# pierluigiferrari/differential_equations_resnet

Hardware: AMD Instinct MI355X
Metric: CIFAR-10 images/sec (fwd+bwd) antisym-ResNet-32 @ batch 512; 1/2/4/8 GPUs (higher is better)
Workload: dtype bf16; 1 GPU; antisym-ResNet-32 (C=64, 30 Euler blocks) batch 512/GPU bf16; train step = fwd + bwd + Adam; global_batch=512, per_gpu_batch=512, channels=64, blocks=30, integrator=euler, parallelism=dp1, degraded_handoffs=0

## Files before the change

### differential_equations_resnet_amd/csrc/asr_api.hip

```cpp
#include <math.h>

#include <vector>

#include "asr_common.h"
#include "asr_internal.h"

namespace asr {
static bool mfma_supported(int C, int W) { return (C == 16 || C == 32 || C == 64) && W == 32; }

static int check_shape(int N, int H, int W, int C) {
  if (N < 1 || H < 1 || W < 1 || C < 1) return fail(ASR_E_ARG, "bad shape N=%d H=%d W=%d C=%d", N, H, W, C);
  if ((long)N * H * W * C > (1L << 40)) return fail(ASR_E_ARG, "shape too large");
  return ASR_OK;
}

static int check_bf16_conv(int C, int W) {
  if (!mfma_supported(C, W) && !convb_supported(W, C))
    return fail(ASR_E_UNSUPPORTED, "bf16 conv needs C in {16,32,64} and W == 8 or W %% 16 == 0 (C=%d W=%d)", C, W);
  return ASR_OK;
}

static int check_kernel_size(const char* fn, int kernel_size) {
  if (kernel_size < 1 || kernel_size > 15 || !(kernel_size & 1))
    return fail(ASR_E_ARG, "%s: kernel_size %d (odd, 1..15)", fn, kernel_size);
  return ASR_OK;
}

struct BwdWs {
  size_t dz, slabs, red, g, total;
};

static BwdWs bwd_ws_layout(int N, int H, int W, int C, int dtype, int stages = 1, int K = 3, int slab_rows = -1) {
  BwdWs b{};
  const long E = (long)K * K * C * C;
  const long P = (long)N * H * W * C;
  const int nsl = slab_rows >= 0 ? slab_rows : kMaxBlockSlabs * stages;
  WsCursor c;
  b.dz = c.take(dtype == ASR_F32 ? (size_t)P * 4 : 0);
  b.slabs = c.take((size_t)nsl * (E + C) * 4);
  b.red = c.take(reduce_ws_bytes(nsl, E + C));
  b.g = c.take(stages > 1 ? (size_t)P * (dtype == ASR_BF16 ? 2 : 4) : 0);
  b.total = c.off;
  return b;
}

struct StemWs {
  size_t dz, slabs, red, total;
};

static StemWs stem_ws_layout(long P, int Cin, int C, int K = 3) {
  StemWs w{};
  const long ES1 = (long)K * K * Cin * C + C;
  WsCursor c;
  w.dz = c.take((size_t)P * 4);
  w.slabs = c.take((size_t)kMaxBlockSlabs * ES1 * 4);
  w.red = c.take(reduce_ws_bytes(kMaxBlockSlabs, ES1));
  w.total = c.off;
  return w;
}

static int block_backward(int mode, const void* dy, const void* x, const uint8_t* mask, const void* w, float h,
                          float gamma, int N, int H, int W, int C, int dtype, void* dx, bool need_w, const void* extra,
                          bool skip_dy, float* slabs, float* dz_scratch, int* nsl, hipStream_t s, bool relu_dx = false,
                          int* relu_done = nullptr, const float* fold_slabs = nullptr, int fold_P = 0,
                          float* fold_grp = nullptr, int* fold_done = nullptr, bool accum_slabs = false) {
  *nsl = 0;
  if (relu_done) *relu_done = 0;
  if (fold_done) *fold_done = 0;
  if (dtype == ASR_BF16) {
    if (!dx && !need_w) return ASR_OK;
    if (!mfma_supported(C, W)) {
      if (extra || skip_dy || relu_dx || fold_slabs || accum_slabs || !convb_supported(W, C))
        return fail(ASR_E_UNSUPPORTED, "bf16 backward at C=%d W=%d: plain Euler blocks and convs only", C, W);
      return convb_backward(dy, mask, x, w, h, 2.f * gamma, N, H, W, C, dx, need_w, slabs, nsl, s,
                            mode == ASR_MODE_CONV);
    }
    const int cm = (mode == ASR_MODE_EULER) ? 2 : 3;
    return block_bwd_mfma(cm, dy, x, mask, w, h, 2.f * gamma, N, H, W, C, dx, slabs, nsl, extra, skip_dy ? 1 : 0, s,
                          relu_dx ? 1 : 0, relu_done, fold_slabs, fold_P, fold_grp, fold_done, accum_slabs ? 1 : 0);
  }
  if (accum_slabs) return fail(ASR_E_UNSUPPORTED, "slab accumulation: bf16 path only");
  const bool euler = mode == ASR_MODE_EULER;
  if (euler && conv32_fused_bwd_supported(W, C))
    return conv32_bwd_fused((const float*)dy, mask, h, (const float*)x, (const float*)w, 2.f * gamma,
                            (const float*)extra, skip_dy, N, H, W, C, (float*)dx, need_w, slabs, nsl, s);
  ASR_TRY(make_dz(euler ? F_EULER : F_CONV, dy, mask, nullptr, h, N, H, W, C, 0, dz_scratch, s));
  if (dx)
    ASR_TRY(conv_f32((euler && !skip_dy) ? B_EULER : B_CONV, dz_scratch, dx, nullptr, (const float*)w, nullptr, h,
                     2.f * gamma, (const float*)dy, N, H, W, C, C, 0, s, (const float*)extra));
  if (need_w) ASR_TRY(wgrad_f32(x, 0, dz_scratch, N, H, W, C, C, slabs, nsl, s));
  return ASR_OK;
}

int conv_backward_keep_slabs(const void* dy, const void* x, const uint8_t* mask, const void* w, float h, float gamma,
                             int N, int H, int W, int C, void* dx, void* ws, float* slabs, int* nsl, hipStream_t s) {
  const BwdWs L = bwd_ws_layout(N, H, W, C, ASR_F32);
  return block_backward(ASR_MODE_EULER, dy, x, mask, w, h, gamma, N, H, W, C, ASR_F32, dx, true, nullptr, false, slabs,
                        (float*)((unsigned char*)ws + L.dz), nsl, s);
}

static int rk2_forward_impl(const void* x, void* xmid, void* y, uint8_t* mask1, uint8_t* mask2, const void* w,
                            const float* bias, float h, int N, int H, int W, int C, int dtype, hipStream_t s) {
  if (dtype == ASR_BF16) {
    ASR_TRY(block_fwd_mfma(0, x, nullptr, xmid, mask1, w, bias, 0.5f * h, N, H, W, C, s));
    return block_fwd_mfma(0, xmid, x, y, mask2, w, bias, h, N, H, W, C, s);
  }
  ASR_TRY(conv_f32(F_EULER, x, xmid, mask1, (const float*)w, bias, 0.5f * h, 0.f, nullptr, N, H, W, C, C, 0, s));
  return conv_f32(F_EULER, xmid, y, mask2, (const float*)w, bias, h, 0.f, nullptr, N, H, W, C, C, 0, s,
                  (const float*)x);
}

static int rk2_backward_slabs(const void* dy, const void* x, const void* xmid, const uint8_t* mask1,
                              const uint8_t* mask2, const void* w, float h, float gamma, int N, int H, int W, int C,
                              int dtype, void* dx, void* g, bool need_w, float* slabs, float* dz_scratch, int* nsl,
                              hipStream_t s, const float* fold_slabs = nullptr, int fold_P = 0,
                              float* fold_grp = nullptr, int* fold_done = nullptr) {
  int n2 = 0, n1 = 0;
  const bool one_set = dtype == ASR_BF16;
  ASR_TRY(block_backward(ASR_MODE_EULER, dy, xmid, mask2, w, h, gamma, N, H, W, C, dtype, g, need_w, nullptr, true,
                         slabs, dz_scratch, &n2, s, false, nullptr, fold_slabs, fold_P, fold_grp, fold_done));
  ASR_TRY(block_backward(ASR_MODE_EULER, g, x, mask1, w, 0.5f * h, gamma, N, H, W, C, dtype, dx, need_w, dy, false,
                         one_set ? slabs : slabs + (long)n2 * (9L * C * C + C), dz_scratch, &n1, s, false, nullptr,
                         nullptr, 0, nullptr, nullptr, one_set));
  *nsl = one_set ? n2 : n1 + n2;
  return ASR_OK;
}

__global__ void k_adam(float* __restrict__ p, const float* __restrict__ g, float* __restrict__ m,
                       float* __restrict__ v, long n, float lr_t, float b1, float b2, float eps, float gscale) {
  for (long i = blockIdx.x * (long)blockDim.x + threadIdx.x; i < n; i += (long)gridDim.x * blockDim.x) {
    const float gi = g[i] * gscale;
    const float mi = b1 * m[i] + (1.f - b1) * gi;
    const float vi = b2 * v[i] + (1.f - b2) * gi * gi;
    m[i] = mi;
    v[i] = vi;
    p[i] -= lr_t * mi / (sqrtf(vi) + eps);
  }
}

__global__ __launch_bounds__(256) void k_relu_grad_bf16(bf16* __restrict__ d, const bf16* __restrict__ x, long n8) {
  for (long i = blockIdx.x * (long)blockDim.x + threadIdx.x; i < n8; i += (long)gridDim.x * blockDim.x) {
    bf16x8 dv = ((const bf16x8*)d)[i];
    const bf16x8 xv = ((const bf16x8*)x)[i];
#pragma unroll
    for (int e = 0; e < 8; ++e) dv[e] = (float)xv[e] > 0.f ? dv[e] : (bf16)0.f;
    ((bf16x8*)d)[i] = dv;
  }
}

int relu_grad_bf16(void* d, const void* x, long n, hipStream_t s) {
  if (n % 8) return fail(ASR_E_ARG, "relu_grad_bf16: n %% 8 != 0");
  const long n8 = n / 8;
  hipLaunchKernelGGL(k_relu_grad_bf16, dim3((unsigned)std::max<long>(1, std::min<long>((n8 + 255) / 256, 4096))),
                     dim3(256), 0, s, (bf16*)d, (const bf16*)x, n8);
  ASR_LAUNCH_CHECK("k_relu_grad_bf16");
  return ASR_OK;
}

__global__ __launch_bounds__(256) void k_segment_sq_norms(const float* __restrict__ x, const long* __restrict__ off,
                                                          float* __restrict__ out) {
  const long b = off[blockIdx.x], e = off[blockIdx.x + 1];
  float acc = 0.f;
  for (long i = b + threadIdx.x; i < e; i += blockDim.x) acc = fmaf(x[i], x[i], acc);
  for (int d = 32; d >= 1; d >>= 1) acc += __shfl_xor(acc, d, 64);
  __shared__ float part[4];
  if ((threadIdx.x & 63) == 0) part[threadIdx.x >> 6] = acc;
  __syncthreads();
  if (threadIdx.x == 0) out[blockIdx.x] = (part[0] + part[1]) + (part[2] + part[3]);
}

__global__ __launch_bounds__(256) void k_batch_metrics(const float* __restrict__ probs, const float* __restrict__ tgt,
                                                       const float* __restrict__ loss, int N, int K,
                                                       float* __restrict__ accum) {
  __shared__ int correct;
  __shared__ float lsum[4];
  if (threadIdx.x == 0) correct = 0;
  __syncthreads();
  float l = 0.f;
  for (int n = threadIdx.x; n < N; n += blockDim.x) {
    const float* p = probs + (long)n * K;
    const float* t = tgt + (long)n * K;
    int ap = 0, at = 0;
    float bp = p[0], bt = t[0], s = 0.f;
    for (int k = 0; k < K; ++k) {
      if (p[k] > bp) bp = p[k], ap = k;
      if (t[k] > bt) bt = t[k], at = k;
      s += p[k];
    }
    if (ap == at) atomicAdd(&correct, 1);
    if (!loss)
      for (int k = 0; k < K; ++k) {
        const float q = p[k] / s;
        l -= t[k] * (q > 1.f - 1e-7f ? -1e-7f : logf(fmaxf(q, 1e-7f)));
      }
  }
  for (int d = 32; d >= 1; d >>= 1) l += __shfl_xor(l, d, 64);
  if ((threadIdx.x & 63) == 0) lsum[threadIdx.x >> 6] = l;
  __syncthreads();
  if (threadIdx.x == 0) {
    accum[0] += loss ? *loss : ((lsum[0] + lsum[1]) + (lsum[2] + lsum[3])) / (float)N;
    accum[1] += (float)correct;
    accum[2] += (float)N;
    accum[3] += 1.f;
  }
}

template <typename Tin>
__global__ void k_normalize(const Tin* __restrict__ img, long n, float mean, float inv_std, int use_norm,
                            float* __restrict__ out) {
  for (long i = blockIdx.x * (long)blockDim.x + threadIdx.x; i < n; i += (long)gridDim.x * blockDim.x) {
    float v = (float)img[i];
    if (use_norm) v = (v - mean) * inv_std;
    out[i] = v;
  }
}

struct NetLayout {
  long ntheta, P, E, wstride;
  long off_c1k, off_c1b, off_blk, blk_stride, off_fck, off_fcb, nparams;
  bool sep_bwd;
  bool rk2;
  int stages;
  long grp_stride;
  size_t grp;
  size_t slabs_all;
  long slab_stride;
  size_t w_src, w_src_bwd, theta_dst, wbuf, wbuf_bwd, x0, acts, xmids, masks, dxa, dxb, dxg, bwdws, slabs2, slabs, red, probs,
      loss_per, dlogits, gap, total;
  long mask_bytes;
  int act_bytes;
  bool fast_stem;
  bool deep;
  size_t deep_slabs;
  bool inference;
  bool stack_bwd;
  bool stack_pair;
  int stack_grid;
  size_t theta_dst_tm, stack_slabs, stack_done;
  size_t theta_dst_pr;
  int f32_rows;
  size_t grow;
  BwdWs bw;
  StemWs stem;
  int k1, kb;
  bool stem_kxk;
  bool kxk;
  int kxk_rows;
};

static int net_k1(const asr_net_config* c) { return c->conv1_kernel_size ? c->conv1_kernel_size : 3; }
static int net_kb(const asr_net_config* c) { return c->kernel_size ? c->kernel_size : 3; }

static const char kNetKernelSizes[] =
    "kernel_size and conv1_kernel_size in {0 (= 3), 3, 5, 7}; kernel_size 5 / 7: ASR_PARAM_GENERAL or "
    "ASR_PARAM_REGULAR blocks, Euler integrator, float32 at any shape, bfloat16 at C in {16, 32, 64} and "
    "W in {8, 16, 32}; kernel_size 3 in bfloat16: C in {16, 32, 64} and W == 8 or W % 16 == 0 (RK2: W == 32)";

static int check_net_kernel_size(const char* field, int k) {
  if (k == 3 || k == 5 || k == 7) return ASR_OK;
  return fail((k < 1 || !(k & 1)) ? ASR_E_ARG : ASR_E_UNSUPPORTED, "%s %d: the network takes %s", field, k,
              kNetKernelSizes);
}

static int net_check(const asr_net_config* c) {
  if (!c) return fail(ASR_E_ARG, "null config");
  ASR_TRY(check_shape(c->N, c->H, c->W, c->C));
  if (c->L < 1 || c->Cin < 1 || c->num_classes < 1)
    return fail(ASR_E_ARG, "bad net config (L=%d Cin=%d K=%d C=%d)", c->L, c->Cin, c->num_classes, c->C);
  if (c->num_classes > 256 || c->C > 256)
    return fail(ASR_E_UNSUPPORTED, "the head takes C and num_classes <= 256 (C=%d K=%d)", c->C, c->num_classes);
  if (c->dtype != ASR_F32 && c->dtype != ASR_BF16) return fail(ASR_E_ARG, "bad dtype");
  if (param_is_antisymmetric(c->param_kind, c->antisymmetric) < 0) return ASR_E_ARG;
  if (c->param_kind == ASR_PARAM_3BY3 && !c->antisymmetric)
    return fail(ASR_E_ARG, "the 3by3 parametrisation is always antisymmetric");
  if (c->integrator != ASR_INTEGRATOR_EULER && c->integrator != ASR_INTEGRATOR_RK2)
    return fail(ASR_E_ARG, "bad integrator %d", c->integrator);
  if (c->variant & ~(ASR_VARIANT_NO_FOLD | ASR_VARIANT_STEM_FWD_VALU | ASR_VARIANT_STEM_WGRAD_VALU | ASR_VARIANT_PER_BLOCK_FWD |
                    ASR_VARIANT_PER_BLOCK_BWD | ASR_VARIANT_INFERENCE | ASR_VARIANT_TIMED | ASR_VARIANT_FULL_DXL |
                    ASR_VARIANT_FULL_SLABS | ASR_VARIANT_W_BF16))
    return fail(ASR_E_ARG, "bad variant bits 0x%x", c->variant);
  const int kb = net_kb(c);
  ASR_TRY(check_net_kernel_size("conv1_kernel_size", net_k1(c)));
  ASR_TRY(check_net_kernel_size("kernel_size", kb));
  if (kb != 3) {
    if (c->param_kind == ASR_PARAM_3BY3)
      return fail(ASR_E_ARG, "the 3by3 parametrisation has kernel_size 3 (kernel_size=%d): the network takes %s", kb,
                  kNetKernelSizes);
    if (c->integrator == ASR_INTEGRATOR_RK2)
      return fail(ASR_E_UNSUPPORTED, "RK2 blocks with kernel_size %d: the network takes %s", kb, kNetKernelSizes);
    if (c->dtype == ASR_BF16 && !convk_bf16_supported(kb, c->W, c->C))
      return fail(ASR_E_UNSUPPORTED, "bf16 network with kernel_size %d at C=%d W=%d: the network takes %s", kb, c->C,
                  c->W, kNetKernelSizes);
    return ASR_OK;
  }
  if (c->dtype == ASR_BF16 && !mfma_supported(c->C, c->W)) {
    if (!convb_supported(c->W, c->C))
      return fail(ASR_E_UNSUPPORTED, "bf16 network needs C in {16,32,64} and W == 8 or W %% 16 == 0 (C=%d W=%d)", c->C,
                  c->W);
    if (c->integrator == ASR_INTEGRATOR_RK2)
      return fail(ASR_E_UNSUPPORTED, "bf16 network with RK2 blocks needs W == 32 (C=%d W=%d)", c->C, c->W);
  }
  return ASR_OK;
}

static NetLayout net_layout(const asr_net_config* c) {
  NetLayout L{};
  const int C = c->C, K = c->num_classes;
  L.k1 = net_k1(c);
  L.kb = net_kb(c);
  L.kxk = L.kb != 3;
  L.ntheta = theta_count_k(C, L.kb, c->param_kind, c->antisymmetric);
  L.sep_bwd = param_is_antisymmetric(c->param_kind, c->antisymmetric) == 0;
  L.rk2 = c->integrator == ASR_INTEGRATOR_RK2;
  L.stages = L.rk2 ? 2 : 1;
  L.P = (long)c->N * c->H * c->W * C;
  L.E = (long)L.kb * L.kb * C * C;
  L.act_bytes = c->dtype == ASR_BF16 ? 2 : 4;
  L.wstride = c->dtype == ASR_BF16 ? (long)(C / 16) * ((L.kb * L.kb * C + 31) / 32) * 512 : L.E;
  L.off_c1k = 0;
  L.off_c1b = (long)L.k1 * L.k1 * c->Cin * C;
  L.off_blk = L.off_c1b + C;
  L.blk_stride = L.ntheta + C;
  L.off_fck = L.off_blk + (long)c->L * L.blk_stride;
  L.off_fcb = L.off_fck + (long)C * K;
  L.nparams = L.off_fcb + K;
  L.mask_bytes = asr_mask_bytes(c->N, c->H, c->W, C);
  L.fast_stem = L.k1 == 3 && stem_supported(c->Cin, c->H, c->W, C);
  L.stem_kxk = c->dtype == ASR_BF16 && L.k1 != 3 && stem_kxk_supported(L.k1, c->Cin, c->W, C);
  L.inference = (c->variant & ASR_VARIANT_INFERENCE) != 0;
  const bool tr = !L.inference;
  L.deep = !L.kxk && c->dtype == ASR_BF16 && !L.rk2 && deep16_supported(c->H, c->W, C);
  L.stack_bwd = !L.kxk && tr && c->dtype == ASR_BF16 && block_stack_bwd_supported(c->N, c->H, c->W, C);
  L.stack_grid = L.stack_bwd ? block_stack_bwd_grid(c->N) : 0;
  L.stack_pair = L.stack_bwd && !L.sep_bwd;
  WsCursor ws;
  L.w_src = ws.take((size_t)L.E * 4);
  L.w_src_bwd = ws.take(L.sep_bwd && tr ? (size_t)L.E * 4 : 0);
  L.theta_dst = ws.take((size_t)L.ntheta * 2 * 4);
  L.wbuf = ws.take((size_t)c->L * L.wstride * L.act_bytes);
  L.wbuf_bwd = ws.take(L.sep_bwd && tr ? (size_t)c->L * L.wstride * L.act_bytes : 0);
  L.x0 = ws.take(L.fast_stem ? 0 : (size_t)c->N * c->H * c->W * c->Cin * 4);
  L.acts = ws.take((size_t)(tr ? c->L + 1 : 3) * L.P * L.act_bytes);
  L.xmids = ws.take(L.rk2 ? (size_t)(tr ? c->L : 1) * L.P * L.act_bytes : 0);
  L.masks = ws.take(tr ? (size_t)L.stages * c->L * L.mask_bytes : 0);
  L.dxa = ws.take(tr ? (size_t)L.P * L.act_bytes : 0);
  L.dxb = ws.take(tr ? (size_t)L.P * L.act_bytes : 0);
  L.dxg = ws.take(L.rk2 && tr ? (size_t)L.P * L.act_bytes : 0);
  const bool f32 = c->dtype == ASR_F32;
  L.kxk_rows = !L.kxk ? 0 : f32 ? wgrad_f32_chunks(c->N, c->H) : wgradk_bf16_slab_rows(L.kb, c->N, c->H, c->W, C);
  L.f32_rows = f32 && !L.kxk ? f32_block_slab_rows(c->N, c->H, c->W, C) : 0;
  L.bw = bwd_ws_layout(c->N, c->H, c->W, C, c->dtype, L.stages, L.kb, L.kxk ? L.kxk_rows : f32 ? 0 : -1);
  L.stem = stem_ws_layout(L.P, c->Cin, C, L.k1);
  L.bwdws = ws.take(tr ? std::max(L.bw.total, L.stem.total) : 0);
  L.slabs2 = ws.take(tr && !f32 && !L.kxk ? (size_t)L.stages * kMaxBlockSlabs * (L.E + C) * 4 : 0);
  const int rows = L.kxk ? L.kxk_rows : f32 ? L.stages * L.f32_rows : L.stages * kMaxBlockSlabs;
  L.grp_stride = (long)reduce_groups(rows) * (L.E + C);
  L.grp = ws.take(tr ? (size_t)c->L * L.grp_stride * 4 : 0);
  L.slab_stride = (long)rows * (L.E + C);
  L.slabs_all = ws.take(tr && f32 && !L.kxk ? (size_t)c->L * L.slab_stride * 4 : 0);
  L.deep_slabs = ws.take(L.deep && tr ? deep16_slab_bytes(c->N, c->L) : 0);
  L.theta_dst_tm = ws.take(L.stack_bwd ? (size_t)L.ntheta * 2 * 4 : 0);
  L.theta_dst_pr = ws.take(L.stack_pair ? (size_t)L.ntheta * 2 * 4 : 0);
  L.stack_slabs = ws.take(L.stack_bwd ? (size_t)c->L * L.stack_grid * (L.E + C) * 4 : 0);
  L.stack_done = ws.take(L.stack_bwd ? (size_t)stack_done_words(c->L) * 4 : 0);
  L.grow = ws.take(L.stack_bwd && !L.rk2 ? (size_t)c->N * C * 2 : 0);
  L.probs = ws.take((size_t)c->N * K * 4);
  L.loss_per = ws.take(tr ? (size_t)c->N * 4 : 0);
  L.dlogits = ws.take(tr ? (size_t)c->N * K * 4 : 0);
  L.gap = ws.take(tr ? (size_t)c->N * C * 4 : 0);
  L.total = ws.off;
  return L;
}

constexpr int kMaxTimedDevices = 64;
struct TimedEvents {
  hipEvent_t ev[5];
  bool made;
  unsigned rec;
};
static TimedEvents g_tev[kMaxTimedDevices];

static TimedEvents* timed_events_here() {
  int dev = 0;
  if (hipGetDevice(&dev) != hipSuccess || dev < 0 || dev >= kMaxTimedDevices) return nullptr;
  return &g_tev[dev];
}

static int timed_event(const asr_net_config* c, int i, hipStream_t s) {
  if (!(c->variant & ASR_VARIANT_TIMED)) return ASR_OK;
  TimedEvents* t = timed_events_here();
  if (!t) return fail(ASR_E_HIP, "ASR_VARIANT_TIMED: no current device (or device id >= %d)", kMaxTimedDevices);
  if (!t->made) {
    for (auto& e : t->ev) ASR_TRY(hip_check(hipEventCreate(&e), "hipEventCreate"));
    t->made = true;
  }
  if (i == 0) t->rec = 0;
  ASR_TRY(hip_check(hipEventRecord(t->ev[i], s), "hipEventRecord"));
  t->rec |= 1u << i;
  return ASR_OK;
}

static unsigned char* net_xL(const asr_net_config* c, const NetLayout& L, unsigned char* ws, bool training,
                             bool stack_fwd) {
  const size_t a = (size_t)L.P * L.act_bytes;
  if (training) return ws + L.acts + (size_t)c->L * a;
  if (stack_fwd) return ws + L.acts + (size_t)(1 + (c->L - 1) % 2) * a;
  return ws + L.acts + (size_t)(c->L & 1) * a;
}

static int net_normalize(const asr_net_config* c, const NetLayout& L, const void* images, unsigned char* ws,
                         hipStream_t s) {
  const float inv_std = c->use_norm ? 1.f / c->divide_by_stddev : 1.f;
  const long nin = (long)c->N * c->H * c->W * c->Cin;
  float* x0 = (float*)(ws + L.x0);
  const unsigned gn = (unsigned)std::min<long>((nin + 255) / 256, 4096);
  if (c->input_u8)
    hipLaunchKernelGGL(k_normalize<uint8_t>, dim3(gn), dim3(256), 0, s, (const uint8_t*)images, nin, c->subtract_mean,
                       inv_std, c->use_norm, x0);
  else
    hipLaunchKernelGGL(k_normalize<float>, dim3(gn), dim3(256), 0, s, (const float*)images, nin, c->subtract_mean,
                       inv_std, c->use_norm, x0);
  ASR_LAUNCH_CHECK("k_normalize");
  return ASR_OK;
}

static int net_forward_impl(const asr_net_config* c, const NetLayout& L, const float* params, const void* images,
                            bool training, unsigned char* ws, hipStream_t s, unsigned char** xL_out = nullptr) {
  const int C = c->C, N = c->N, H = c->H, W = c->W;
  const bool bf = c->dtype == ASR_BF16;
  const float inv_std = c->use_norm ? 1.f / c->divide_by_stddev : 1.f;
  if (training && L.inference) return fail(ASR_E_ARG, "an ASR_VARIANT_INFERENCE workspace has no training buffers");
  const bool bal = !(c->variant & ASR_VARIANT_W_BF16);
  if (L.kxk) {
    const float* th = params + L.off_blk;
    const int32_t* src = (const int32_t*)(ws + L.w_src);
    const int32_t* src_bwd = (const int32_t*)(ws + L.w_src_bwd);
    if (bf) {
      ASR_TRY(asr_theta_to_w_k_bf16(th, L.blk_stride, c->L, C, L.kb, src, c->gamma, ws + L.wbuf, L.wstride, s));
      if (training && L.sep_bwd)
        ASR_TRY(asr_theta_to_w_k_bf16(th, L.blk_stride, c->L, C, L.kb, src_bwd, 0.f, ws + L.wbuf_bwd, L.wstride, s));
    } else {
      ASR_TRY(asr_theta_to_w_k(th, L.blk_stride, c->L, C, L.kb, src, c->gamma, (float*)(ws + L.wbuf), L.wstride, s));
      if (training && L.sep_bwd)
        ASR_TRY(asr_theta_to_w_k(th, L.blk_stride, c->L, C, L.kb, src_bwd, 0.f, (float*)(ws + L.wbuf_bwd), L.wstride,
                                 s));
    }
  } else if (bf)
    ASR_TRY(theta_to_w_bf16(params + L.off_blk, L.blk_stride, c->L, C, (const int32_t*)(ws + L.w_src), c->gamma,
                            ws + L.wbuf, L.wstride, bal, s,
                            c->param_kind != ASR_PARAM_REGULAR ? (const int32_t*)(ws + L.theta_dst) : nullptr,
                            L.ntheta));
  else
    ASR_TRY(asr_theta_to_w(params + L.off_blk, L.blk_stride, c->L, C, (const int32_t*)(ws + L.w_src), c->gamma,
                           ws + L.wbuf, L.wstride, c->dtype, s));
  if (training && L.sep_bwd && !L.kxk) {
    if (bf)
      ASR_TRY(theta_to_w_bf16(params + L.off_blk, L.blk_stride, c->L, C, (const int32_t*)(ws + L.w_src_bwd), 0.f,
                              ws + L.wbuf_bwd, L.wstride, bal, s));
    else
      ASR_TRY(asr_theta_to_w(params + L.off_blk, L.blk_stride, c->L, C, (const int32_t*)(ws + L.w_src_bwd), 0.f,
                             ws + L.wbuf_bwd, L.wstride, c->dtype, s));
  }
  unsigned char* acts = ws + L.acts;
  auto act = [&](int i) -> unsigned char* {
    const int slot = training ? i : (i & 1);
    return acts + (size_t)slot * L.P * L.act_bytes;
  };
  if (xL_out) *xL_out = net_xL(c, L, ws, training, false);
  if (L.fast_stem && bf && stem_fwd_mfma_supported(c->Cin, H, W, C) && !(c->variant & ASR_VARIANT_STEM_FWD_VALU)) {
    ASR_TRY(stem_fwd_mfma(images, c->input_u8, params + L.off_c1k, params + L.off_c1b, N, H, W, c->Cin, C,
                          c->subtract_mean, inv_std, c->use_norm, act(0), s));
  } else if (L.stem_kxk && !(c->variant & ASR_VARIANT_STEM_FWD_VALU)) {
    ASR_TRY(stem_fwd_kxk(L.k1, images, c->input_u8, params + L.off_c1k, params + L.off_c1b, N, H, W, c->Cin, C,
                         c->subtract_mean, inv_std, c->use_norm, act(0), s));
  } else if (L.fast_stem) {
    ASR_TRY(stem_forward(images, c->input_u8, params + L.off_c1k, params + L.off_c1b, N, H, W, c->Cin, C,
                         c->subtract_mean, inv_std, c->use_norm, act(0), bf ? 1 : 0, s));
  } else {
    float* x0 = (float*)(ws + L.x0);
    ASR_TRY(net_normalize(c, L, images, ws, s));
    ASR_TRY(conv_f32(F_RELU, x0, act(0), nullptr, params + L.off_c1k, params + L.off_c1b, 1.f, 0.f, nullptr, N, H,
                     W, c->Cin, C, bf ? 1 : 0, s, nullptr, L.k1));
  }
  ASR_TRY(timed_event(c, 0, s));
  if (L.deep) {
    ASR_TRY(deep16_forward(act(0), act(training ? 1 : c->L), L.P, training ? (uint8_t*)(ws + L.masks) : nullptr,
                           L.mask_bytes, ws + L.wbuf, params + L.off_blk + L.ntheta, L.blk_stride, c->h, N, c->L,
                           training, s));
    return timed_event(c, 1, s);
  }
  if (bf && training && L.rk2 && block_stack_fwd_supported(N, H, W, C) && !(c->variant & ASR_VARIANT_PER_BLOCK_FWD)) {
    uint8_t* m1 = (uint8_t*)(ws + L.masks);
    ASR_TRY(block_stack_fwd_rk2_mfma(act(0), act(1), ws + L.xmids, (long)L.P, m1, m1 + (size_t)c->L * L.mask_bytes,
                                     (long)L.mask_bytes, ws + L.wbuf, (long)L.wstride, params + L.off_blk + L.ntheta,
                                     L.blk_stride, c->h, N, H, W, C, c->L, s));
    return timed_event(c, 1, s);
  }
  if (bf && !L.rk2 && !L.kxk && (training || L.inference) && block_stack_fwd_supported(N, H, W, C) &&
      !(c->variant & ASR_VARIANT_PER_BLOCK_FWD)) {
    if (training) {
      ASR_TRY(block_stack_fwd_mfma(act(0), act(1), (long)L.P, (uint8_t*)(ws + L.masks), (long)L.mask_bytes,
                                   ws + L.wbuf, (long)L.wstride, params + L.off_blk + L.ntheta, L.blk_stride, c->h, N,
                                   H, W, C, c->L, s));
    } else {
      ASR_TRY(block_stack_fwd_mfma(acts, acts + (size_t)L.P * L.act_bytes, (long)L.P, nullptr, 0, ws + L.wbuf,
                                   (long)L.wstride, params + L.off_blk + L.ntheta, L.blk_stride, c->h, N, H, W, C,
                                   c->L, s, 2));
      if (xL_out) *xL_out = net_xL(c, L, ws, false, true);
    }
    return timed_event(c, 1, s);
  }
  for (int l = 0; l < c->L; ++l) {
    const float* bias = params + L.off_blk + (long)l * L.blk_stride + L.ntheta;
    const unsigned char* wl = ws + L.wbuf + (size_t)l * L.wstride * L.act_bytes;
    uint8_t* mask = training ? (uint8_t*)(ws + L.masks) + (size_t)l * L.mask_bytes : nullptr;
    if (L.rk2) {
      unsigned char* xm = ws + L.xmids + (training ? (size_t)l * L.P * L.act_bytes : 0);
      uint8_t* mask2 = training ? mask + (size_t)c->L * L.mask_bytes : nullptr;
      ASR_TRY(rk2_forward_impl(act(l), xm, act(l + 1), mask, mask2, wl, bias, c->h, N, H, W, C, c->dtype, s));
    } else if (L.kxk && bf) {
      ASR_TRY(convk_bf16(F_EULER, L.kb, act(l), act(l + 1), mask, wl, bias, c->h, 0.f, nullptr, N, H, W, C, s));
    } else if (L.kxk) {
      ASR_TRY(conv_f32_k(F_EULER, L.kb, act(l), act(l + 1), mask, (const float*)wl, bias, c->h, 0.f, nullptr, N, H, W,
                         C, s, nullptr));
    } else if (bf && !mfma_supported(C, W)) {
      ASR_TRY(convb_forward(act(l), act(l + 1), mask, wl, bias, c->h, N, H, W, C, s));
    } else if (bf) {
      ASR_TRY(block_fwd_mfma(0, act(l), nullptr, act(l + 1), mask, wl, bias, c->h, N, H, W, C, s));
    } else {
      ASR_TRY(conv_f32(F_EULER, act(l), act(l + 1), mask, (const float*)wl, bias, c->h, 0.f, nullptr, N, H, W, C, C,
                       0, s));
    }
  }
  return timed_event(c, 1, s);
}

int fused_stage_kind(int H, int W, int C, int dtype) {
  if (dtype == ASR_BF16 && deep16_supported(H, W, C)) return kFusedDeep16;
  return stage_img_supported(H, W, C, dtype) ? kFusedImg : kFusedNone;
}

int fused_stage_forward(int kind, int dtype, const void* x0, void* ys, long y_stride, uint8_t* masks, long mask_stride,
                        const void* w, long w_stride, const float* bias, long bias_stride, float h, int N, int H, int W,
                        int C, int L, bool store_all, hipStream_t s) {
  if (kind == kFusedDeep16)
    return deep16_forward(x0, ys, y_stride, masks, mask_stride, w, bias, bias_stride, h, N, L, store_all, s);
  if (kind != kFusedImg || !store_all)
    return fail(ASR_E_ARG, "fused_stage_forward: kind %d, store_all %d", kind, store_all);
  return stage_img_forward(dtype, x0, ys, y_stride, masks, mask_stride, w, w_stride, bias, bias_stride, h, N, H, W, C,
                           L, s);
}

int fused_stage_backward(const char* who, int kind, int dtype, void* d, void* e, int* in_e, void* dx0_copy, void* dys,
                         const void* xs, long x_stride, const uint8_t* masks, long mask_stride, const void* w,
                         long w_stride, float h, float two_gamma, int N, int H, int W, int C, int L, float* slabs,
                         long slab_stride, int slab_rows, float* grp, long grp_stride, const int32_t* theta_dst,
                         long n_theta, float* dparams, long dp_stride, hipStream_t s) {
  const long E = 9L * C * C, P = (long)N * H * W * C;
  int rows = 0;
  if (kind == kFusedDeep16) {
    ASR_TRY(deep16_backward(d, e, xs, x_stride, masks, mask_stride, w, h, two_gamma, N, L, slabs, &rows, in_e, s));
    if (dx0_copy)
      ASR_TRY(hip_check(hipMemcpyAsync(dx0_copy, *in_e ? e : d, (size_t)P * 2, hipMemcpyDeviceToDevice, s),
                        "hipMemcpyAsync"));
    if (!dparams) return ASR_OK;
    if (rows != slab_rows) return fail(ASR_E_WORKSPACE, "%s: deep16 slab rows %d != %d", who, rows, slab_rows);
    ASR_TRY(reduce_slabs_to_groups(slabs, L * rows, E + C, grp, s));
    return project_layers(grp, grp_stride, reduce_groups(rows), E, C, theta_dst, n_theta, L, dparams, dp_stride, s);
  }
  if (kind != kFusedImg) return fail(ASR_E_ARG, "%s: not a fused stage", who);
  *in_e = 1;
  ASR_TRY(stage_img_backward(dtype, d, dys, P, e, masks, mask_stride, w, w_stride, h, two_gamma, N, H, W, C, L, s));
  if (!dparams) return ASR_OK;
  ASR_TRY(wgrad_layers(dtype, xs, x_stride, dys, P, masks, mask_stride, h, N, H, W, C, L, slabs, slab_stride, &rows, s));
  if (rows > slab_rows) return fail(ASR_E_WORKSPACE, "%s: %d slab rows > the workspace's %d", who, rows, slab_rows);
  ASR_TRY(reduce_slab_layers(slabs, slab_stride, rows, E + C, grp, grp_stride, L, s));
  return project_layers(grp, grp_stride, reduce_groups(rows), E, C, theta_dst, n_theta, L, dparams, dp_stride, s);
}

}

using namespace asr;

extern "C" {

long asr_mask_bytes(int N, int H, int W, int C) {
  if (N < 1 || H < 1 || W < 1 || C < 1) return -1;
  return ((long)N * H * W * C + 31) / 32 * 4;
}

int asr_conv_forward(int mode, const void* x, void* y, uint8_t* mask, const void* w, const float* bias, float h,
                     int N, int H, int W, int C, int dtype, asr_stream_t stream) {
  ASR_TRY(check_shape(N, H, W, C));
  if (!x || !y || !w) return fail(ASR_E_ARG, "asr_conv_forward: null pointer");
  if (mode != ASR_MODE_EULER && mode != ASR_MODE_CONV) return fail(ASR_E_ARG, "asr_conv_forward: bad mode %d", mode);
  hipStream_t s = (hipStream_t)stream;
  if (dtype == ASR_BF16) {
    ASR_TRY(check_bf16_conv(C, W));
    if (!mfma_supported(C, W))
      return convb_forward(x, y, mask, w, bias, h, N, H, W, C, s, mode == ASR_MODE_CONV);
    if (mode == ASR_MODE_EULER && deep16_supported(H, W, C))
      return deep16_forward(x, y, 0, mask, 0, w, bias, 0, h, N, 1, true, s);
    return block_fwd_mfma(mode == ASR_MODE_EULER ? 0 : 1, x, nullptr, y, mask, w, bias, h, N, H, W, C, s);
  }
  if (dtype == ASR_F32)
    return conv_f32(mode == ASR_MODE_EULER ? F_EULER : F_CONV, x, y, mask, (const float*)w, bias, h, 0.f, nullptr, N,
                    H, W, C, C, 0, s);
  return fail(ASR_E_ARG, "asr_conv_forward: bad dtype %d", dtype);
}

static int stack_img_check_strides(const char* who, int dtype, long y_stride, long mask_stride, long w_stride,
                                   long bias_stride, long x_stride) {
  const bool bf = dtype == ASR_BF16;
  if (y_stride % 4) return fail(ASR_E_ARG, "%s: y_stride %% 4 != 0 on the image-resident path", who);
  if (mask_stride % 2) return fail(ASR_E_ARG, "%s: mask_stride %% 2 != 0 on the image-resident path", who);
  if (bf && w_stride % 8) return fail(ASR_E_ARG, "%s: w_stride %% 8 != 0 on the image-resident path", who);
  if (bias_stride % 4) return fail(ASR_E_ARG, "%s: bias_stride %% 4 != 0 on the image-resident path", who);
  if (x_stride % (bf ? 8 : 4))
    return fail(ASR_E_ARG, "%s: x_stride %% %d != 0 on the image-resident path", who, bf ? 8 : 4);
  return ASR_OK;
}

int asr_block_stack_forward(const void* x0, void* ys, long y_stride, uint8_t* masks, long mask_stride, const void* w,
                            long w_stride, const float* bias, long bias_stride, float h, int N, int H, int W, int C,
                            int L, int dtype, int store_all, asr_stream_t stream) {
  ASR_TRY(check_shape(N, H, W, C));
  if (!x0 || !ys || !w || L < 1) return fail(ASR_E_ARG, "asr_block_stack_forward: null pointer or L < 1");
  if (store_all && L > 1 && y_stride < (long)N * H * W * C)
    return fail(ASR_E_ARG, "asr_block_stack_forward: y_stride smaller than one activation");
  hipStream_t s = (hipStream_t)stream;
  const int fused = fused_stage_kind(H, W, C, dtype);
  if (fused == kFusedDeep16) {
    if (L > 1 && w_stride != (long)asr_wpack_elems(C))
      return fail(ASR_E_ARG, "asr_block_stack_forward: w_stride must be asr_wpack_elems(C) on the fused path");
    return fused_stage_forward(fused, dtype, x0, ys, y_stride, masks, mask_stride, w, w_stride, bias, bias_stride, h, N,
                               H, W, C, L, store_all != 0, s);
  }
  if (dtype == ASR_BF16) ASR_TRY(check_bf16_conv(C, W));
  if (dtype != ASR_F32 && dtype != ASR_BF16) return fail(ASR_E_ARG, "asr_block_stack_forward: bad dtype");
  const size_t es = dtype == ASR_BF16 ? 2 : 4;
  if (!store_all && L > 1) return fail(ASR_E_UNSUPPORTED, "asr_block_stack_forward: store_all=0 needs the fused path");
  if (fused == kFusedImg && store_all && bias && masks) {
    ASR_TRY(stack_img_check_strides("asr_block_stack_forward", dtype, y_stride, mask_stride, w_stride, bias_stride, 0));
    return fused_stage_forward(fused, dtype, x0, ys, y_stride, masks, mask_stride, w, w_stride, bias, bias_stride, h, N,
                               H, W, C, L, true, s);
  }
  if (dtype == ASR_BF16 && block_stack_fwd_supported(N, H, W, C))
    return block_stack_fwd_mfma(x0, ys, L > 1 ? y_stride : (long)N * H * W * C, masks, mask_stride, w, w_stride, bias,
                                bias_stride, h, N, H, W, C, L, s);
  for (int l = 0; l < L; ++l) {
    const void* xi = l == 0 ? x0 : (const unsigned char*)ys + (size_t)(l - 1) * y_stride * es;
    void* yo = (unsigned char*)ys + (size_t)l * y_stride * es;
    ASR_TRY(asr_conv_forward(ASR_MODE_EULER, xi, yo, masks ? masks + (size_t)l * mask_stride : nullptr,
                             (const unsigned char*)w + (size_t)l * w_stride * es, bias ? bias + l * bias_stride : nullptr,
                             h, N, H, W, C, dtype, stream));
  }
  return ASR_OK;
}

struct StackWs {
  size_t da, db, slabs, grp, blk, done, tdst, g, dys, total;
  int fused;
  bool stack64;
  int grid;
  int rows;
};
static StackWs stack_ws_layout(int N, int H, int W, int C, int L, int dtype, bool rk2 = false) {
  StackWs w{};
  const size_t act = (size_t)N * H * W * C * (dtype == ASR_BF16 ? 2 : 4);
  const long ES = 9L * C * C + C;
  w.fused = rk2 ? kFusedNone : fused_stage_kind(H, W, C, dtype);
  w.stack64 = dtype == ASR_BF16 && w.fused == kFusedNone && block_stack_bwd_supported(N, H, W, C);
  w.grid = w.stack64 ? block_stack_bwd_grid(N) : 0;
  WsCursor c;
  w.da = c.take(act);
  w.db = c.take(act);
  if (w.fused == kFusedImg) {
    w.rows = f32_block_slab_rows(N, H, W, C);
    w.dys = c.take(L * act);
    w.slabs = c.take((size_t)L * w.rows * ES * 4);
    w.grp = c.take((size_t)L * reduce_groups(w.rows) * ES * 4);
  } else if (w.fused == kFusedDeep16) {
    w.rows = (int)(deep16_slab_bytes(N, 1) / ((size_t)ES * 4));
    w.slabs = c.take(deep16_slab_bytes(N, L));
    w.grp = c.take((size_t)L * reduce_groups(kMaxBlockSlabs) * ES * 4);
  } else if (w.stack64) {
    w.slabs = c.take((size_t)L * w.grid * ES * 4);
    w.grp = c.take((size_t)L * reduce_groups(w.grid) * ES * 4);
    w.done = c.take((size_t)stack_done_words(L) * 4);
    w.tdst = c.take((size_t)2 * 9 * C * C * 4);
    if (rk2) w.g = c.take(act);
  } else {
    w.blk = c.take(bwd_ws_layout(N, H, W, C, dtype).total);
  }
  w.total = c.off;
  return w;
}

static int stack64_backward(const char* who, const StackWs& Lw, const void* dyL, const void* xs, const void* xmids,
                            long x_stride, const uint8_t* masks, const uint8_t* masks2, long mask_stride,
                            const void* w, long w_stride, const int32_t* theta_dst, long n_theta, float h, float gamma,
                            int N, int H, int W, int C, int L, void* dx0, float* dparams, unsigned char* base,
                            hipStream_t s) {
  if (n_theta > 9L * C * C) return fail(ASR_E_ARG, "%s: n_theta > 9*C*C", who);
  const size_t act = (size_t)N * H * W * C * 2;
  ASR_TRY(hip_check(hipMemcpyAsync(base + Lw.da, dyL, act, hipMemcpyDeviceToDevice, s), "hipMemcpyAsync"));
  float* slabs = (float*)(base + Lw.slabs);
  float* grp = (float*)(base + Lw.grp);
  const long ES = stack_slab_floats(C, 1), sst = (long)Lw.grid * ES, gst = (long)reduce_groups(Lw.grid) * ES;
  int lfold = L;
  ASR_TRY(block_stack_bwd_mfma(base + Lw.da, base + Lw.db, xs, x_stride, masks, mask_stride, w, w_stride, h,
                               2.f * gamma, N, H, W, C, L, 0, slabs, sst, grp, gst, (unsigned*)(base + Lw.done),
                               &lfold, s, xmids, masks2, xmids ? base + Lw.g : nullptr, nullptr, 1, 1));
  ASR_TRY(hip_check(hipMemcpyAsync(dx0, base + ((L & 1) ? Lw.db : Lw.da), act, hipMemcpyDeviceToDevice, s),
                    "hipMemcpyAsync"));
  if (!dparams) return ASR_OK;
  ASR_TRY(stack_bwd_reduce_rest(slabs, sst, Lw.grid, ES, grp, gst, L, lfold, (const unsigned*)(base + Lw.done), s));
  int32_t* tm = (int32_t*)(base + Lw.tdst);
  ASR_TRY(theta_dst_pair(theta_dst, n_theta, C, tm, s));
  return project_layers(grp, gst, reduce_groups(Lw.grid), ES - C, C, tm, n_theta, L, dparams, n_theta + C, s);
}

size_t asr_block_stack_backward_workspace_bytes(int N, int H, int W, int C, int L, int dtype) {
  if (check_shape(N, H, W, C) != ASR_OK || L < 1) return 0;
  return stack_ws_layout(N, H, W, C, L, dtype).total;
}

int asr_block_stack_backward(const void* dyL, const void* xs, long x_stride, const uint8_t* masks, long mask_stride,
                             const void* w, long w_stride, const int32_t* theta_dst, long n_theta, float h,
                             float gamma, int N, int H, int W, int C, int L, int dtype, void* dx0, float* dparams,
                             void* ws, size_t ws_bytes, asr_stream_t stream) {
  ASR_TRY(check_shape(N, H, W, C));
  if (!dyL || !xs || !masks || !w || !dx0 || L < 1) return fail(ASR_E_ARG, "asr_block_stack_backward: null pointer");
  if (dparams && !theta_dst) return fail(ASR_E_ARG, "asr_block_stack_backward: theta_dst needed for dparams");
  if (dtype != ASR_F32 && dtype != ASR_BF16) return fail(ASR_E_ARG, "asr_block_stack_backward: bad dtype");
  if (dtype == ASR_BF16) ASR_TRY(check_bf16_conv(C, W));
  const StackWs Lw = stack_ws_layout(N, H, W, C, L, dtype);
  if (Lw.fused == kFusedImg)
    ASR_TRY(stack_img_check_strides("asr_block_stack_backward", dtype, 0, 0, w_stride, 0, x_stride));
  if (!ws || ws_bytes < Lw.total) return fail(ASR_E_WORKSPACE, "asr_block_stack_backward: workspace too small");
  if (Lw.fused == kFusedDeep16 && w_stride != (long)asr_wpack_elems(C))
    return fail(ASR_E_ARG, "asr_block_stack_backward: w_stride must be asr_wpack_elems(C) on the fused path");
  hipStream_t s = (hipStream_t)stream;
  unsigned char* base = (unsigned char*)ws;
  const size_t es = dtype == ASR_BF16 ? 2 : 4, act = (size_t)N * H * W * C * es;
  if (Lw.fused != kFusedNone) {
    const bool deep = Lw.fused == kFusedDeep16;
    const long ES = 9L * C * C + C;
    if (deep) ASR_TRY(hip_check(hipMemcpyAsync(base + Lw.da, dyL, act, hipMemcpyDeviceToDevice, s), "hipMemcpyAsync"));
    int in_e = 0;
    return fused_stage_backward("asr_block_stack_backward", Lw.fused, dtype, deep ? base + Lw.da : (void*)dyL,
                                deep ? base + Lw.db : dx0, &in_e, deep ? dx0 : nullptr, base + Lw.dys, xs, x_stride,
                                masks, mask_stride, w, w_stride, h, 2.f * gamma, N, H, W, C, L,
                                (float*)(base + Lw.slabs), (long)Lw.rows * ES, Lw.rows, (float*)(base + Lw.grp),
                                (long)reduce_groups(Lw.rows) * ES, theta_dst, n_theta, dparams, n_theta + C, s);
  }
  if (Lw.stack64)
    return stack64_backward("asr_block_stack_backward", Lw, dyL, xs, nullptr, x_stride, masks, nullptr, mask_stride, w,
                            w_stride, theta_dst, n_theta, h, gamma, N, H, W, C, L, dx0, dparams, base, s);
  const void* dcur = dyL;
  for (int l = L - 1; l >= 0; --l) {
    void* dnext = l == 0 ? dx0 : base + ((l & 1) ? Lw.db : Lw.da);
    float* dp = dparams ? dparams + (long)l * (n_theta + C) : nullptr;
    ASR_TRY(asr_conv_backward(ASR_MODE_EULER, dcur, (const unsigned char*)xs + (size_t)l * x_stride * es,
                              masks + (size_t)l * mask_stride, (const unsigned char*)w + (size_t)l * w_stride * es,
                              theta_dst, n_theta, h, gamma, N, H, W, C, dtype, dnext, dp, dp ? dp + n_theta : nullptr,
                              nullptr, base + Lw.blk, ws_bytes - Lw.blk, stream));
    dcur = dnext;
  }
  return ASR_OK;
}

int asr_rk2_stack_forward(const void* x0, void* ys, void* xmids, long y_stride, uint8_t* masks1, uint8_t* masks2,
                          long mask_stride, const void* w, long w_stride, const float* bias, long bias_stride, float h,
                          int N, int H, int W, int C, int L, int dtype, asr_stream_t stream) {
  ASR_TRY(check_shape(N, H, W, C));
  if (!x0 || !ys || !xmids || !w || L < 1) return fail(ASR_E_ARG, "asr_rk2_stack_forward: null pointer or L < 1");
  if (dtype != ASR_BF16 || !block_stack_fwd_supported(N, H, W, C))
    return fail(ASR_E_UNSUPPORTED, "asr_rk2_stack_forward: bf16, C=64, W=32 only (C=%d W=%d)", C, W);
  if ((masks1 == nullptr) != (masks2 == nullptr)) return fail(ASR_E_ARG, "asr_rk2_stack_forward: masks1/masks2");
  return block_stack_fwd_rk2_mfma(x0, ys, xmids, y_stride, masks1, masks2, mask_stride, w, w_stride, bias,
                                  bias_stride, h, N, H, W, C, L, (hipStream_t)stream);
}

size_t asr_rk2_stack_backward_workspace_bytes(int N, int H, int W, int C, int L, int dtype) {
  if (check_shape(N, H, W, C) != ASR_OK || L < 1) return 0;
  const StackWs w = stack_ws_layout(N, H, W, C, L, dtype, true);
  return w.stack64 ? w.total : 0;
}

int asr_rk2_stack_backward(const void* dyL, const void* xs, const void* xmids, long x_stride, const uint8_t* masks1,
                           const uint8_t* masks2, long mask_stride, const void* w, long w_stride,
                           const int32_t* theta_dst, long n_theta, float h, float gamma, int N, int H, int W, int C,
                           int L, int dtype, void* dx0, float* dparams, void* ws, size_t ws_bytes,
                           asr_stream_t stream) {
  ASR_TRY(check_shape(N, H, W, C));
  if (!dyL || !xs || !xmids || !masks1 || !masks2 || !w || !dx0 || L < 1)
    return fail(ASR_E_ARG, "asr_rk2_stack_backward: null pointer");
  if (dparams && !theta_dst) return fail(ASR_E_ARG, "asr_rk2_stack_backward: theta_dst needed for dparams");
  const StackWs Lw = stack_ws_layout(N, H, W, C, L, dtype, true);
  if (!Lw.stack64) return fail(ASR_E_UNSUPPORTED, "asr_rk2_stack_backward: bf16, C=64, W=32 only (C=%d W=%d)", C, W);
  if (!ws || ws_bytes < Lw.total) return fail(ASR_E_WORKSPACE, "asr_rk2_stack_backward: workspace too small");
  return stack64_backward("asr_rk2_stack_backward", Lw, dyL, xs, xmids, x_stride, masks1, masks2, mask_stride, w,
                          w_stride, theta_dst, n_theta, h, gamma, N, H, W, C, L, dx0, dparams, (unsigned char*)ws,
                          (hipStream_t)stream);
}

size_t asr_conv_backward_workspace_bytes_k(int N, int H, int W, int C, int kernel_size) {
  if (check_shape(N, H, W, C) != ASR_OK || kernel_size < 1 || !(kernel_size & 1)) return 0;
  return bwd_ws_layout(N, H, W, C, ASR_F32, 1, kernel_size).total;
}

int asr_conv_forward_k(int mode, int kernel_size, const float* x, float* y, uint8_t* mask, const float* w,
                       const float* bias, float h, int N, int H, int W, int C, asr_stream_t stream) {
  ASR_TRY(check_shape(N, H, W, C));
  if (!x || !y || !w) return fail(ASR_E_ARG, "asr_conv_forward_k: null pointer");
  if (mode != ASR_MODE_EULER && mode != ASR_MODE_CONV) return fail(ASR_E_ARG, "asr_conv_forward_k: bad mode %d", mode);
  ASR_TRY(check_kernel_size("asr_conv_forward_k", kernel_size));
  return conv_f32_k(mode == ASR_MODE_EULER ? F_EULER : F_CONV, kernel_size, x, y, mask, w, bias, h, 0.f, nullptr, N, H, W,
                    C, (hipStream_t)stream, nullptr);
}

int asr_conv_backward_k(int mode, int kernel_size, const float* dy, const float* x, const uint8_t* mask,
                        const float* w, const int32_t* theta_dst, long n_theta, float h, float gamma, int N, int H,
                        int W, int C, float* dx, float* dtheta, float* dbias, float* dw, void* ws, size_t ws_bytes,
                        asr_stream_t stream) {
  ASR_TRY(check_shape(N, H, W, C));
  if (mode != ASR_MODE_EULER && mode != ASR_MODE_CONV) return fail(ASR_E_ARG, "asr_conv_backward_k: bad mode %d", mode);
  ASR_TRY(check_kernel_size("asr_conv_backward_k", kernel_size));
  if (!dy || !w || (mode == ASR_MODE_EULER && !mask)) return fail(ASR_E_ARG, "asr_conv_backward_k: null pointer");
  if ((dtheta || dbias || dw) && !x) return fail(ASR_E_ARG, "asr_conv_backward_k: x needed for weight gradients");
  if (dtheta && !theta_dst) return fail(ASR_E_ARG, "asr_conv_backward_k: theta_dst needed for dtheta");
  const BwdWs Lw = bwd_ws_layout(N, H, W, C, ASR_F32, 1, kernel_size);
  if (!ws || ws_bytes < Lw.total) return fail(ASR_E_WORKSPACE, "asr_conv_backward_k: workspace too small");
  hipStream_t s = (hipStream_t)stream;
  unsigned char* base = (unsigned char*)ws;
  float* dz = (float*)(base + Lw.dz);
  float* slabs = (float*)(base + Lw.slabs);
  const bool euler = mode == ASR_MODE_EULER;
  ASR_TRY(make_dz(euler ? F_EULER : F_CONV, dy, mask, nullptr, h, N, H, W, C, 0, dz, s));
  if (dx) ASR_TRY(conv_f32_k(euler ? B_EULER : B_CONV, kernel_size, dz, dx, nullptr, w, nullptr, h, 2.f * gamma, dy, N, H,
                             W, C, s, nullptr));
  if (dtheta || dbias || dw) {
    int nsl = 0;
    ASR_TRY(wgrad_f32(x, 0, dz, N, H, W, C, C, slabs, &nsl, s, kernel_size));
    ASR_TRY(reduce_and_project(slabs, nsl, (long)kernel_size * kernel_size * C * C, C, dtheta ? theta_dst : nullptr,
                               n_theta, dtheta, dbias, dw, (float*)(base + Lw.red), s));
  }
  return ASR_OK;
}

static int check_k_bf16(const char* fn, int kernel_size, int W, int C) {
  ASR_TRY(check_kernel_size(fn, kernel_size));
  if (!convk_bf16_supported(kernel_size, W, C))
    return fail(ASR_E_UNSUPPORTED,
                "%s: the bf16 k x k kernels take kernel_size in {5, 7}, C in {16, 32, 64}, W in {8, 16, 32} "
                "(kernel_size=%d C=%d W=%d)", fn, kernel_size, C, W);
  return ASR_OK;
}

struct BwdWsK {
  size_t slabs, red, total;
  int rows;
};
static BwdWsK bwd_ws_layout_k_bf16(int N, int H, int W, int C, int K) {
  BwdWsK b{};
  const long ES = (long)K * K * C * C + C;
  b.rows = wgradk_bf16_slab_rows(K, N, H, W, C);
  WsCursor c;
  b.slabs = c.take((size_t)b.rows * ES * 4);
  b.red = c.take(reduce_ws_bytes(b.rows, ES));
  b.total = c.off;
  return b;
}

int asr_conv_forward_k_bf16(int mode, int kernel_size, const void* x, void* y, uint8_t* mask, const void* w,
                            const float* bias, float h, int N, int H, int W, int C, asr_stream_t stream) {
  ASR_TRY(check_shape(N, H, W, C));
  if (!x || !y || !w) return fail(ASR_E_ARG, "asr_conv_forward_k_bf16: null pointer");
  if (mode != ASR_MODE_EULER && mode != ASR_MODE_CONV)
    return fail(ASR_E_ARG, "asr_conv_forward_k_bf16: bad mode %d", mode);
  ASR_TRY(check_k_bf16("asr_conv_forward_k_bf16", kernel_size, W, C));
  return convk_bf16(mode == ASR_MODE_EULER ? F_EULER : F_CONV, kernel_size, x, y, mask, w, bias, h, 0.f, nullptr, N, H,
                    W, C, (hipStream_t)stream);
}

size_t asr_conv_backward_workspace_bytes_k_bf16(int N, int H, int W, int C, int kernel_size) {
  if (check_shape(N, H, W, C) != ASR_OK || !convk_bf16_supported(kernel_size, W, C)) return 0;
  return bwd_ws_layout_k_bf16(N, H, W, C, kernel_size).total;
}

int asr_conv_backward_k_bf16(int mode, int kernel_size, const void* dy, const void* x, const uint8_t* mask,
                             const void* w, const int32_t* theta_dst, long n_theta, float h, float gamma, int N, int H,
                             int W, int C, void* dx, float* dtheta, float* dbias, float* dw, void* ws, size_t ws_bytes,
                             asr_stream_t stream) {
  ASR_TRY(check_shape(N, H, W, C));
  if (mode != ASR_MODE_EULER && mode != ASR_MODE_CONV)
    return fail(ASR_E_ARG, "asr_conv_backward_k_bf16: bad mode %d", mode);
  ASR_TRY(check_k_bf16("asr_conv_backward_k_bf16", kernel_size, W, C));
  if (!dy || !w || (mode == ASR_MODE_EULER && !mask)) return fail(ASR_E_ARG, "asr_conv_backward_k_bf16: null pointer");
  if ((dtheta || dbias || dw) && !x) return fail(ASR_E_ARG, "asr_conv_backward_k_bf16: x needed for weight gradients");
  if (dtheta && !theta_dst) return fail(ASR_E_ARG, "asr_conv_backward_k_bf16: theta_dst needed for dtheta");
  const BwdWsK Lw = bwd_ws_layout_k_bf16(N, H, W, C, kernel_size);
  if (!ws || ws_bytes < Lw.total) return fail(ASR_E_WORKSPACE, "asr_conv_backward_k_bf16: workspace too small");
  hipStream_t s = (hipStream_t)stream;
  unsigned char* base = (unsigned char*)ws;
  const bool euler = mode == ASR_MODE_EULER;
  if (dx) ASR_TRY(convk_bf16(euler ? B_EULER : B_CONV, kernel_size, dy, dx, nullptr, w, nullptr, h, 2.f * gamma,
                             euler ? mask : nullptr, N, H, W, C, s));
  if (dtheta || dbias || dw) {
    float* slabs = (float*)(base + Lw.slabs);
    int nsl = 0;
    ASR_TRY(wgradk_bf16(kernel_size, x, dy, euler ? mask : nullptr, euler ? h : 1.f, N, H, W, C, slabs, &nsl, s));
    ASR_TRY(reduce_and_project(slabs, nsl, (long)kernel_size * kernel_size * C * C, C, dtheta ? theta_dst : nullptr,
                               n_theta, dtheta, dbias, dw, (float*)(base + Lw.red), s));
  }
  return ASR_OK;
}

size_t asr_conv_backward_workspace_bytes(int N, int H, int W, int C, int dtype) {
  if (check_shape(N, H, W, C) != ASR_OK) return 0;
  return bwd_ws_layout(N, H, W, C, dtype).total;
}

int asr_conv_backward(int mode, const void* dy, const void* x, const uint8_t* mask, const void* w,
                      const int32_t* theta_dst, long n_theta, float h, float gamma, int N, int H, int W, int C,
                      int dtype, void* dx, float* dtheta, float* dbias, float* dw_hwio, void* ws, size_t ws_bytes,
                      asr_stream_t stream) {
  ASR_TRY(check_shape(N, H, W, C));
  if (mode != ASR_MODE_EULER && mode != ASR_MODE_CONV) return fail(ASR_E_ARG, "asr_conv_backward: bad mode %d", mode);
  if (!dy || !w || (mode == ASR_MODE_EULER && !mask)) return fail(ASR_E_ARG, "asr_conv_backward: null pointer");
  if ((dtheta || dbias || dw_hwio) && !x) return fail(ASR_E_ARG, "asr_conv_backward: x needed for weight gradients");
  if (dtheta && !theta_dst) return fail(ASR_E_ARG, "asr_conv_backward: theta_dst needed for dtheta");
  if (dtype != ASR_F32 && dtype != ASR_BF16) return fail(ASR_E_ARG, "asr_conv_backward: bad dtype");
  if (dtype == ASR_BF16) ASR_TRY(check_bf16_conv(C, W));
  const BwdWs L = bwd_ws_layout(N, H, W, C, dtype);
  if (!ws || ws_bytes < L.total) return fail(ASR_E_WORKSPACE, "asr_conv_backward: workspace too small");
  hipStream_t s = (hipStream_t)stream;
  unsigned char* base = (unsigned char*)ws;
  float* slabs = (float*)(base + L.slabs);
  const bool need_w = dtheta || dbias || dw_hwio;
  int nsl = 0;
  ASR_TRY(block_backward(mode, dy, x, mask, w, h, gamma, N, H, W, C, dtype, dx, need_w, nullptr, false, slabs,
                         (float*)(base + L.dz), &nsl, s));
  if (need_w)
    ASR_TRY(reduce_and_project(slabs, nsl, 9L * C * C, C, dtheta ? theta_dst : nullptr, n_theta, dtheta, dbias,
                               dw_hwio, (float*)(base + L.red), s));
  return ASR_OK;
}

static int check_block_args(const char* fn, int N, int H, int W, int C, int dtype) {
  ASR_TRY(check_shape(N, H, W, C));
  if (dtype != ASR_F32 && dtype != ASR_BF16) return fail(ASR_E_ARG, "%s: bad dtype %d", fn, dtype);
  if (dtype == ASR_BF16 && !mfma_supported(C, W))
    return fail(ASR_E_UNSUPPORTED, "%s: bf16 needs C in {16,32,64} and W == 32 (C=%d W=%d)", fn, C, W);
  return ASR_OK;
}

int asr_rk2_forward(const void* x, void* xmid, void* y, uint8_t* mask1, uint8_t* mask2, const void* w,
                    const float* bias, float h, int N, int H, int W, int C, int dtype, asr_stream_t stream) {
  ASR_TRY(check_block_args("asr_rk2_forward", N, H, W, C, dtype));
  if (!x || !xmid || !y || !w) return fail(ASR_E_ARG, "asr_rk2_forward: null pointer");
  if (x == xmid || x == y || xmid == y) return fail(ASR_E_ARG, "asr_rk2_forward: x, xmid and y must not alias");
  return rk2_forward_impl(x, xmid, y, mask1, mask2, w, bias, h, N, H, W, C, dtype, (hipStream_t)stream);
}

size_t asr_rk2_backward_workspace_bytes(int N, int H, int W, int C, int dtype) {
  if (check_shape(N, H, W, C) != ASR_OK) return 0;
  return bwd_ws_layout(N, H, W, C, dtype, 2).total;
}

int asr_rk2_backward(const void* dy, const void* x, const void* xmid, const uint8_t* mask1, const uint8_t* mask2,
                     const void* w, const int32_t* theta_dst, long n_theta, float h, float gamma, int N, int H, int W,
                     int C, int dtype, void* dx, float* dtheta, float* dbias, float* dw_hwio, void* ws,
                     size_t ws_bytes, asr_stream_t stream) {
  ASR_TRY(check_block_args("asr_rk2_backward", N, H, W, C, dtype));
  if (!dy || !x || !xmid || !mask1 || !mask2 || !w) return fail(ASR_E_ARG, "asr_rk2_backward: null pointer");
  if (dtheta && !theta_dst) return fail(ASR_E_ARG, "asr_rk2_backward: theta_dst needed for dtheta");
  const BwdWs L = bwd_ws_layout(N, H, W, C, dtype, 2);
  if (!ws || ws_bytes < L.total) return fail(ASR_E_WORKSPACE, "asr_rk2_backward: workspace too small");
  hipStream_t s = (hipStream_t)stream;
  unsigned char* base = (unsigned char*)ws;
  float* slabs = (float*)(base + L.slabs);
  const bool need_w = dtheta || dbias || dw_hwio;
  int nsl = 0;
  ASR_TRY(rk2_backward_slabs(dy, x, xmid, mask1, mask2, w, h, gamma, N, H, W, C, dtype, dx, base + L.g, need_w, slabs,
                             (float*)(base + L.dz), &nsl, s));
  if (need_w)
    ASR_TRY(reduce_and_project(slabs, nsl, 9L * C * C, C, dtheta ? theta_dst : nullptr, n_theta, dtheta, dbias,
                               dw_hwio, (float*)(base + L.red), s));
  return ASR_OK;
}

long asr_net_param_count(const asr_net_config* cfg) {
  if (net_check(cfg) != ASR_OK) return -1;
  return net_layout(cfg).nparams;
}

size_t asr_net_workspace_bytes(const asr_net_config* cfg) {
  if (net_check(cfg) != ASR_OK) return 0;
  return net_layout(cfg).total;
}

int asr_net_prepare(const asr_net_config* cfg, void* ws, size_t ws_bytes) {
  ASR_TRY(net_check(cfg));
  const NetLayout L = net_layout(cfg);
  if (!ws || ws_bytes < L.total) return fail(ASR_E_WORKSPACE, "asr_net_prepare: workspace too small");
  ASR_TRY(check_ws_device(ws, "asr_net_prepare"));
  std::vector<int32_t> w_src((size_t)L.E), theta_dst((size_t)L.ntheta * 2);
  ASR_TRY(param_map_k(cfg->C, L.kb, cfg->param_kind, cfg->antisymmetric, w_src.data(), theta_dst.data()));
  unsigned char* b = (unsigned char*)ws;
  if (L.sep_bwd && !L.inference) {
    std::vector<int32_t> w_bwd((size_t)L.E);
    ASR_TRY(param_map_transpose_k(cfg->C, L.kb, w_src.data(), w_bwd.data()));
    ASR_TRY(hip_check(hipMemcpy(b + L.w_src_bwd, w_bwd.data(), w_bwd.size() * 4, hipMemcpyHostToDevice), "hipMemcpy"));
  }
  ASR_TRY(hip_check(hipMemcpy(b + L.w_src, w_src.data(), w_src.size() * 4, hipMemcpyHostToDevice), "hipMemcpy"));
  ASR_TRY(hip_check(hipMemcpy(b + L.theta_dst, theta_dst.data(), theta_dst.size() * 4, hipMemcpyHostToDevice),
                    "hipMemcpy"));
  if (L.stack_pair) {
    std::vector<int32_t> pr(theta_dst.size());
    ASR_TRY(theta_dst_pair_host(theta_dst.data(), L.ntheta, cfg->C, pr.data()));
    ASR_TRY(hip_check(hipMemcpy(b + L.theta_dst_pr, pr.data(), pr.size() * 4, hipMemcpyHostToDevice), "hipMemcpy"));
  }
  if (L.stack_bwd) {
    const int C = cfg->C;
    std::vector<int32_t> tm(theta_dst);
    for (auto& v : tm) {
      if (v < 0) continue;
      const long e = v >> 1, m = e / C, o = e % C;
      const long et = (((m / 16) * (C / 16) + o / 16) * 64 + 16 * ((m % 16) / 4) + o % 16) * 4 + m % 4;
      v = (int32_t)((et << 1) | (v & 1));
    }
    ASR_TRY(hip_check(hipMemcpy(b + L.theta_dst_tm, tm.data(), tm.size() * 4, hipMemcpyHostToDevice), "hipMemcpy"));
  }
  return ASR_OK;
}

int asr_net_forward(const asr_net_config* cfg, const float* params, const void* images, float* probs, void* ws,
                    size_t ws_bytes, asr_stream_t stream) {
  ASR_TRY(net_check(cfg));
  const NetLayout L = net_layout(cfg);
  if (!params || !images || !probs) return fail(ASR_E_ARG, "asr_net_forward: null pointer");
  if (!ws || ws_bytes < L.total) return fail(ASR_E_WORKSPACE, "asr_net_forward: workspace too small");
  ASR_TRY(check_ws_device(ws, "asr_net_forward"));
  hipStream_t s = (hipStream_t)stream;
  unsigned char* b = (unsigned char*)ws;
  unsigned char* xL = nullptr;
  ASR_TRY(net_forward_impl(cfg, L, params, images, false, b, s, &xL));
  ASR_TRY(head(xL, cfg->dtype == ASR_BF16, params + L.off_fck, params + L.off_fcb, nullptr, cfg->N, cfg->H * cfg->W,
               cfg->C, cfg->num_classes, probs, nullptr, nullptr, nullptr, nullptr, s));
  return ASR_OK;
}

int asr_net_check_status(const asr_net_config* cfg, const void* ws, size_t ws_bytes, asr_stream_t stream) {
  ASR_TRY(net_check(cfg));
  const NetLayout L = net_layout(cfg);
  if (!ws || ws_bytes < L.total) return fail(ASR_E_WORKSPACE, "asr_net_check_status: workspace too small");
  ASR_TRY(check_ws_device(ws, "asr_net_check_status"));
  return hip_check(hipStreamSynchronize((hipStream_t)stream), "hipStreamSynchronize");
}

int asr_net_kernel_times(float* us) {
  if (!us) return fail(ASR_E_ARG, "asr_net_kernel_times: null output");
  const TimedEvents* t = timed_events_here();
  if (!t || !t->made || !(t->rec & 3u))
    return fail(ASR_E_ARG, "asr_net_kernel_times: no ASR_VARIANT_TIMED call recorded on the current device");
  for (int i = 0; i < 3; ++i) us[i] = -1.f;
  for (int i = 0; i < 3; ++i) {
    const int a = i == 0 ? 0 : i + 1, e = a + 1;
    if ((t->rec >> a & 1u) && (t->rec >> e & 1u)) {
      ASR_TRY(hip_check(hipEventSynchronize(t->ev[e]), "hipEventSynchronize"));
      float ms = 0.f;
      ASR_TRY(hip_check(hipEventElapsedTime(&ms, t->ev[a], t->ev[e]), "hipEventElapsedTime"));
      us[i] = ms * 1e3f;
    }
  }
  return ASR_OK;
}

int asr_net_forward_backward(const asr_net_config* cfg, const float* params, const void* images, const float* targets,
                             float* grads, float* loss, float* probs, void* ws, size_t ws_bytes,
                             asr_stream_t stream) {
  ASR_TRY(net_check(cfg));
  const NetLayout L = net_layout(cfg);
  if (!params || !images || !targets || !grads || !loss) return fail(ASR_E_ARG, "asr_net_forward_backward: null");
  if (!ws || ws_bytes < L.total) return fail(ASR_E_WORKSPACE, "asr_net_forward_backward: workspace too small");
  if (L.inference)
    return fail(ASR_E_ARG, "asr_net_forward_backward: an ASR_VARIANT_INFERENCE workspace has no training buffers");
  ASR_TRY(check_ws_device(ws, "asr_net_forward_backward"));
  hipStream_t s = (hipStream_t)stream;
  unsigned char* b = (unsigned char*)ws;
  const int C = cfg->C, N = cfg->N, H = cfg->H, W = cfg->W, K = cfg->num_classes;
  const bool bf = cfg->dtype == ASR_BF16;
  const bool stacked = L.stack_bwd && !(cfg->variant & ASR_VARIANT_PER_BLOCK_BWD);
  ASR_TRY(net_forward_impl(cfg, L, params, images, true, b, s));
  auto act = [&](int i) { return b + L.acts + (size_t)i * L.P * L.act_bytes; };
  unsigned char* dcur = b + L.dxa;
  unsigned char* dnext = b + L.dxb;
  float* probs_ws = probs ? probs : (float*)(b + L.probs);
  const bool grow = stacked && !L.rk2 && !(cfg->variant & ASR_VARIANT_FULL_DXL);
  ASR_TRY(head(act(cfg->L), bf, params + L.off_fck, params + L.off_fcb, targets, N, H * W, C, K, probs_ws,
               (float*)(b + L.loss_per), (float*)(b + L.dlogits), (float*)(b + L.gap), grow ? nullptr : dcur, s,
               grow ? b + L.grow : nullptr));
  ASR_TRY(head_param_grads((const float*)(b + L.gap), (const float*)(b + L.dlogits), N, C, K, grads + L.off_fck,
                           grads + L.off_fcb, (const float*)(b + L.loss_per), loss, s));
  const int32_t* theta_dst = (const int32_t*)(b + L.theta_dst);
  int nsl_blk = 0;
  int dz1_fused = 0;
  const float* pend_slabs = nullptr;
  int pend_P = 0;
  float* pend_grp = nullptr;
  const bool fold_on = !(cfg->variant & ASR_VARIANT_NO_FOLD);
  const bool stem_v1 = (cfg->variant & ASR_VARIANT_STEM_WGRAD_VALU) != 0;
  ASR_TRY(timed_event(cfg, 2, s));
  if (L.deep) {
    int rows = 0, in_b = 0;
    float* slabs = (float*)(b + L.deep_slabs);
    ASR_TRY(deep16_backward(dcur, dnext, act(0), L.P, (const uint8_t*)(b + L.masks), L.mask_bytes,
                            b + (L.sep_bwd ? L.wbuf_bwd : L.wbuf), cfg->h, L.sep_bwd ? 0.f : 2.f * cfg->gamma, N,
                            cfg->L, slabs, &rows, &in_b, s));
    ASR_TRY(timed_event(cfg, 3, s));
    if (in_b) std::swap(dcur, dnext);
    const int G = reduce_groups(rows);
    ASR_TRY(reduce_slabs_to_groups(slabs, cfg->L * rows, L.E + C, (float*)(b + L.grp), s));
    ASR_TRY(project_layers((float*)(b + L.grp), (long)G * (L.E + C), G, L.E, C, theta_dst, L.ntheta, cfg->L,
                           grads + L.off_blk, L.blk_stride, s));
    ASR_TRY(timed_event(cfg, 4, s));
  }
  if (stacked) {
    const int grid = L.stack_grid;
    const bool pair = L.stack_pair && !(cfg->variant & ASR_VARIANT_FULL_SLABS);
    const long ES = stack_slab_floats(C, pair ? 1 : 0), sst = (long)grid * ES;
    float* slabs = (float*)(b + L.stack_slabs);
    float* grp = (float*)(b + L.grp);
    const int ro0 = (L.fast_stem || L.stem_kxk) && !stem_v1 && !L.rk2;
    int lfold = cfg->L;
    const uint8_t* m1 = (const uint8_t*)(b + L.masks);
    ASR_TRY(block_stack_bwd_mfma(dcur, dnext, act(0), L.P, m1, L.mask_bytes, b + (L.sep_bwd ? L.wbuf_bwd : L.wbuf),
                                 L.wstride, cfg->h, L.sep_bwd ? 0.f : 2.f * cfg->gamma, N, H, W, C, cfg->L, ro0, slabs,
                                 sst, grp, L.grp_stride, (unsigned*)(b + L.stack_done), &lfold, s,
                                 L.rk2 ? b + L.xmids : nullptr, L.rk2 ? m1 + (size_t)cfg->L * L.mask_bytes : nullptr,
                                 L.rk2 ? b + L.dxg : nullptr, grow ? b + L.grow : nullptr, fold_on ? 1 : 0,
                                 pair ? 1 : 0));
    ASR_TRY(timed_event(cfg, 3, s));
    ASR_TRY(stack_bwd_reduce_rest(slabs, sst, grid, ES, grp, L.grp_stride, cfg->L, lfold,
                                  (const unsigned*)(b + L.stack_done), s));
    if (cfg->L & 1) std::swap(dcur, dnext);
    dz1_fused = ro0;
    ASR_TRY(project_layers(grp, L.grp_stride, reduce_groups(grid), ES - C, C,
                           (const int32_t*)(b + (pair ? L.theta_dst_pr : L.theta_dst_tm)), L.ntheta, cfg->L,
                           grads + L.off_blk, L.blk_stride, s));
    ASR_TRY(timed_event(cfg, 4, s));
  }
  if (L.kxk) {
    float* slabs_k = (float*)(b + L.bwdws + L.bw.slabs);
    float* dz_k = (float*)(b + L.bwdws + L.bw.dz);
    for (int l = cfg->L - 1; l >= 0; --l) {
      const unsigned char* wl = b + (L.sep_bwd ? L.wbuf_bwd : L.wbuf) + (size_t)l * L.wstride * L.act_bytes;
      const uint8_t* mask = (const uint8_t*)(b + L.masks) + (size_t)l * L.mask_bytes;
      const float two_gamma = L.sep_bwd ? 0.f : 2.f * cfg->gamma;
      int nsl = 0;
      if (bf) {
        ASR_TRY(convk_bf16(B_EULER, L.kb, dcur, dnext, nullptr, wl, nullptr, cfg->h, two_gamma, mask, N, H, W, C, s));
        ASR_TRY(wgradk_bf16(L.kb, act(l), dcur, mask, cfg->h, N, H, W, C, slabs_k, &nsl, s));
      } else {
        ASR_TRY(make_dz(F_EULER, dcur, mask, nullptr, cfg->h, N, H, W, C, 0, dz_k, s));
        ASR_TRY(conv_f32_k(B_EULER, L.kb, dz_k, dnext, nullptr, (const float*)wl, nullptr, cfg->h, two_gamma,
                           (const float*)dcur, N, H, W, C, s, nullptr));
        ASR_TRY(wgrad_f32(act(l), 0, dz_k, N, H, W, C, C, slabs_k, &nsl, s, L.kb));
      }
      if (nsl < 1 || nsl > L.kxk_rows)
        return fail(ASR_E_WORKSPACE, "k x k block %d wrote %d slab rows, the workspace holds %d", l, nsl, L.kxk_rows);
      ASR_TRY(reduce_slabs_to_groups(slabs_k, nsl, L.E + C, (float*)(b + L.grp) + (size_t)l * L.grp_stride, s));
      nsl_blk = nsl;
      std::swap(dcur, dnext);
    }
  }
  const bool blk_fuses = !bf || mfma_supported(C, W);
  for (int l = (L.deep || stacked || L.kxk) ? -1 : cfg->L - 1; l >= 0; --l) {
    const unsigned char* wl = b + (L.sep_bwd ? L.wbuf_bwd : L.wbuf) + (size_t)l * L.wstride * L.act_bytes;
    const uint8_t* mask = (const uint8_t*)(b + L.masks) + (size_t)l * L.mask_bytes;
    const float gam = L.sep_bwd ? 0.f : cfg->gamma;
    float* grp_l = (float*)(b + L.grp) + (size_t)l * L.grp_stride;
    float* slabs_l = !bf ? (float*)(b + L.slabs_all) + (size_t)l * L.slab_stride
                         : (float*)(b + ((l & 1) ? L.slabs2 : L.bwdws + L.bw.slabs));
    int nsl = 0, folded = 0;
    if (L.rk2) {
      const unsigned char* xm = b + L.xmids + (size_t)l * L.P * L.act_bytes;
      ASR_TRY(rk2_backward_slabs(dcur, act(l), xm, mask, mask + (size_t)cfg->L * L.mask_bytes, wl, cfg->h, gam, N, H,
                                 W, C, cfg->dtype, dnext, b + L.dxg, true, slabs_l, (float*)(b + L.bwdws + L.bw.dz),
                                 &nsl, s, fold_on ? pend_slabs : nullptr, fold_on ? pend_P : 0, pend_grp, &folded));
    } else {
      ASR_TRY(block_backward(ASR_MODE_EULER, dcur, act(l), mask, wl, cfg->h, gam, N, H, W, C, cfg->dtype, dnext, true,
                             nullptr, false, slabs_l, (float*)(b + L.bwdws + L.bw.dz), &nsl, s,
                             l == 0 && (L.fast_stem || L.stem_kxk) && bf && !stem_v1 && blk_fuses,
                             l == 0 ? &dz1_fused : nullptr, fold_on && blk_fuses ? pend_slabs : nullptr,
                             fold_on && blk_fuses ? pend_P : 0, pend_grp, &folded));
    }
    nsl_blk = nsl;
    std::swap(dcur, dnext);
    if (!bf) {
      if (nsl > L.stages * L.f32_rows)
        return fail(ASR_E_WORKSPACE, "fp32 block %d wrote %d slab rows, the workspace holds %d (sized on another device?)",
                    l, nsl, L.stages * L.f32_rows);
      continue;
    }
    if (pend_P > 0 && !folded) ASR_TRY(reduce_slabs_to_groups(pend_slabs, pend_P, L.E + C, pend_grp, s));
    pend_slabs = slabs_l;
    pend_P = nsl;
    pend_grp = grp_l;
  }
  if (pend_P > 0) ASR_TRY(reduce_slabs_to_groups(pend_slabs, pend_P, L.E + C, pend_grp, s));
  if (!bf && !L.deep && !stacked && !L.kxk && nsl_blk > 0)
    ASR_TRY(reduce_slab_layers((const float*)(b + L.slabs_all), L.slab_stride, nsl_blk, L.E + C,
                               (float*)(b + L.grp), L.grp_stride, cfg->L, s));
  if (!L.deep && !stacked) {
    ASR_TRY(timed_event(cfg, 3, s));
    ASR_TRY(project_layers((float*)(b + L.grp), L.grp_stride, reduce_groups(nsl_blk), L.E, C, theta_dst, L.ntheta,
                           cfg->L, grads + L.off_blk, L.blk_stride, s));
    ASR_TRY(timed_event(cfg, 4, s));
  }
  const long E1 = (long)L.k1 * L.k1 * cfg->Cin * C;
  float* dz = (float*)(b + L.bwdws + L.stem.dz);
  float* slabs = (float*)(b + L.bwdws + L.stem.slabs);
  float* red = (float*)(b + L.bwdws + L.stem.red);
  int nsl = 0;
  const float inv_std = cfg->use_norm ? 1.f / cfg->divide_by_stddev : 1.f;
  if (L.fast_stem && bf && !dz1_fused && !stem_v1 && stem_wgrad_mfma_supported(cfg->Cin, H, W, C) && L.P % 8 == 0) {
    ASR_TRY(relu_grad_bf16(dcur, act(0), L.P, s));
    dz1_fused = 1;
  }
  if (L.stem_kxk && !stem_v1) {
    if (!dz1_fused) ASR_TRY(relu_grad_bf16(dcur, act(0), L.P, s));
    ASR_TRY(stem_wgrad_kxk(L.k1, images, cfg->input_u8, dcur, N, H, W, cfg->Cin, C, cfg->subtract_mean, inv_std,
                           cfg->use_norm, slabs, &nsl, s));
  } else if (L.fast_stem && dz1_fused && stem_wgrad_mfma_supported(cfg->Cin, H, W, C)) {
    ASR_TRY(stem_wgrad_mfma(images, cfg->input_u8, dcur, N, H, W, cfg->Cin, C, cfg->subtract_mean, inv_std,
                            cfg->use_norm, slabs, &nsl, s));
  } else if (L.fast_stem) {
    ASR_TRY(stem_wgrad(images, cfg->input_u8, dcur, act(0), bf, N, H, W, cfg->Cin, C, cfg->subtract_mean, inv_std,
                       cfg->use_norm, slabs, &nsl, s));
  } else {
    if (L.stem_kxk && !(cfg->variant & ASR_VARIANT_STEM_FWD_VALU)) ASR_TRY(net_normalize(cfg, L, images, b, s));
    ASR_TRY(make_dz(F_RELU, dcur, nullptr, act(0), 1.f, N, H, W, C, bf ? 1 : 0, dz, s));
    ASR_TRY(wgrad_f32(b + L.x0, 0, dz, N, H, W, cfg->Cin, C, slabs, &nsl, s, L.k1));
  }
  ASR_TRY(reduce_and_project(slabs, nsl, E1, C, nullptr, 0, nullptr, grads + L.off_c1b, grads + L.off_c1k, red, s));
  return ASR_OK;
}

int asr_segment_sq_norms(const float* x, const long* offsets, int n_segments, float* out, asr_stream_t stream) {
  if (!x || !offsets || !out || n_segments < 0) return fail(ASR_E_ARG, "asr_segment_sq_norms: bad arguments");
  if (n_segments == 0) return ASR_OK;
  hipLaunchKernelGGL(k_segment_sq_norms, dim3(n_segments), dim3(256), 0, (hipStream_t)stream, x, offsets, out);
  ASR_LAUNCH_CHECK("k_segment_sq_norms");
  return ASR_OK;
}

int asr_batch_metrics(const float* probs, const float* targets, const float* loss, int N, int K, float* accum,
                      asr_stream_t stream) {
  if (!probs || !targets || !accum || N < 1 || K < 1) return fail(ASR_E_ARG, "asr_batch_metrics: bad args");
  hipLaunchKernelGGL(k_batch_metrics, dim3(1), dim3(256), 0, (hipStream_t)stream, probs, targets, loss, N, K, accum);
  ASR_LAUNCH_CHECK("k_batch_metrics");
  return ASR_OK;
}

int asr_adam_update(float* params, const float* grads, float* m, float* v, long n, float lr, float beta1, float beta2,
                    float eps, long step, float grad_scale, asr_stream_t stream) {
  if (!params || !grads || !m || !v || n < 0 || step < 1) return fail(ASR_E_ARG, "asr_adam_update: bad arguments");
  const double lr_t = (double)lr * sqrt(1.0 - pow((double)beta2, (double)step)) / (1.0 - pow((double)beta1, (double)step));
  const unsigned grid = (unsigned)std::max<long>(1, std::min<long>((n + 255) / 256, 4096));
  hipLaunchKernelGGL(k_adam, dim3(grid), dim3(256), 0, (hipStream_t)stream, params, grads, m, v, n, (float)lr_t,
                     beta1, beta2, eps, grad_scale);
  ASR_LAUNCH_CHECK("k_adam");
  return ASR_OK;
}

}
```

### differential_equations_resnet_amd/csrc/asr_blk_stem.h

```cpp
#pragma once
#include <type_traits>

#include "asr_blk_common.h"
#include "asr_common.h"
#include "asr_device.h"

namespace asr {
namespace blk {

template <int C, typename Tin>
__global__ __launch_bounds__(256) void k_stem_wgrad_mfma(const Tin* __restrict__ img, const bf16* __restrict__ dz1,
                                                         int N, int H, float mean, float inv_std,
                                                         float* __restrict__ slabs) {
  constexpr int W = 32, CIN = 3, TW = W + 2, BRS = 8, KC = 9 * CIN, NT = C / 16;
  constexpr int IMROW = TW * 4 * 16, DZROW = TW * (C / 8) * 16, DZT = BRS * DZROW;
  extern __shared__ __attribute__((aligned(16))) unsigned char lds[];
  const int IM = 0, DZ0 = H * IMROW, FT = DZ0 + 2 * DZT;
  float* ft = (float*)(lds + FT);
  const int tid = threadIdx.x, lane = tid & 63, wave = tid >> 6;
  const int g = lane >> 4, lx = lane & 15, tq = lx >> 2, tp = lx & 3;
  const int nbands = H / BRS;
  for (int i = tid; i < (H + 2) * TW * CIN; i += 256) ft[i] = 0.f;
  f32x4 acc[2][NT];
#pragma unroll
  for (int mt = 0; mt < 2; ++mt)
#pragma unroll
    for (int nt = 0; nt < NT; ++nt) acc[mt][nt] = f32x4{0.f, 0.f, 0.f, 0.f};
  const int n0 = blockIdx.x, items = ((N - n0 + (int)gridDim.x - 1) / (int)gridDim.x) * nbands;
  auto band_n = [&](int it) { return n0 + (it / nbands) * (int)gridDim.x; };
  auto dma_band = [&](int it, int buf) {
    dma_rows<C, W>(dz1, lds + DZ0 + buf * DZT, band_n(it), (it % nbands) * BRS, BRS, H, wave, 4, lane);
  };
  if (items > 0) dma_band(0, 0);
  for (int it = 0; it < items; ++it) {
    const int buf = it & 1, b = it % nbands;
    if (b == 0) {
      const int n = band_n(it);
      __syncthreads();
      const Tin* src = img + (long)n * H * W * CIN;
      for (int i = tid; i < H * W * CIN; i += 256) {
        const int ci = i % CIN, p = i / CIN;
        ft[((p / W + 1) * TW + p % W + 1) * CIN + ci] = (float)src[i] - mean;
      }
      __syncthreads();
      for (int p = tid; p < H * W; p += 256) {
        const int y = p / W, x = p % W;
#pragma unroll
        for (int q = 0; q < 4; ++q) {
          bf16x8 v;
#pragma unroll
          for (int j = 0; j < 8; ++j) {
            const int kap = 8 * q + j;
            float f = 0.f;
            if (kap < KC) {
              const int tap = kap / CIN, ci = kap % CIN;
              f = ft[((y + tap / 3) * TW + x + tap % 3) * CIN + ci];
            } else if (kap == KC) {
              f = 1.f;
            }
            v[j] = (bf16)f;
          }
          *(bf16x8*)(lds + IM + toff<32>(y, x + 1, q, TW)) = v;
        }
      }
    }
    barrier_vm(0);
    if (it + 1 < items) dma_band(it + 1, buf ^ 1);
    const unsigned char* dzt = lds + DZ0 + buf * DZT;
#pragma unroll
    for (int k = 0; k < BRS / 4; ++k) {
      const int r = wave + 4 * k, y = b * BRS + r;
      const int pb = 8 * g + tq;
      bf16x8 A[2], B[NT];
#pragma unroll
      for (int mt = 0; mt < 2; ++mt) {
        const int q = 2 * mt + (tp >> 1);
        A[mt] = tr_pair(lds + IM + toff<32>(y, pb + 1, q, TW) + 8 * (tp & 1),
                        lds + IM + toff<32>(y, pb + 5, q, TW) + 8 * (tp & 1));
      }
#pragma unroll
      for (int nt = 0; nt < NT; ++nt) {
        const int q = 2 * nt + (tp >> 1);
        B[nt] = tr_pair(dzt + toff<C>(r, pb + 1, q, TW) + 8 * (tp & 1), dzt + toff<C>(r, pb + 5, q, TW) + 8 * (tp & 1));
      }
#pragma unroll
      for (int mt = 0; mt < 2; ++mt)
#pragma unroll
        for (int nt = 0; nt < NT; ++nt)
          acc[mt][nt] = __builtin_amdgcn_mfma_f32_16x16x32_bf16(A[mt], B[nt], acc[mt][nt], 0, 0, 0);
    }
  }
  barrier_vm(0);
  float* red = (float*)lds;
#pragma unroll
  for (int mt = 0; mt < 2; ++mt)
#pragma unroll
    for (int nt = 0; nt < NT; ++nt)
#pragma unroll
      for (int e = 0; e < 4; ++e) red[(wave * 32 + 16 * mt + 4 * g + e) * C + 16 * nt + lx] = acc[mt][nt][e];
  __syncthreads();
  float* slab = slabs + (long)blockIdx.x * (KC * C + C);
  for (int i = tid; i < (KC + 1) * C; i += 256) {
    const float v = (red[i] + red[32 * C + i]) + (red[2 * 32 * C + i] + red[3 * 32 * C + i]);
    slab[i] = i < KC * C ? v * inv_std : v;
  }
}

template <int C, typename Tin>
__global__ __launch_bounds__(256) void k_stem_fwd_mfma(const Tin* __restrict__ img, const float* __restrict__ w1,
                                                       const float* __restrict__ b1, int N, int H, float mean,
                                                       float inv_std, bf16* __restrict__ out) {
  constexpr int W = 32, CIN = 3, TW = W + 2, KC = 9 * CIN, MT = C / 16;
  extern __shared__ __attribute__((aligned(16))) unsigned char lds[];
  float* ft = (float*)lds;
  const int tid = threadIdx.x, lane = tid & 63, wave = tid >> 6;
  const int g = lane >> 4, lx = lane & 15;
  for (int i = tid; i < (H + 2) * TW * CIN; i += 256) ft[i] = 0.f;
  bf16x8 Ah[MT], Al[MT];
#pragma unroll
  for (int mt = 0; mt < MT; ++mt)
#pragma unroll
    for (int j = 0; j < 8; ++j) {
      const int kap = 8 * g + j;
      const float wv = kap < KC ? w1[kap * C + 16 * mt + lx] * inv_std : 0.f;
      const bf16 hi = (bf16)wv;
      Ah[mt][j] = hi;
      Al[mt][j] = (bf16)(wv - (float)hi);
    }
  float bz[MT][4];
#pragma unroll
  for (int mt = 0; mt < MT; ++mt)
#pragma unroll
    for (int e = 0; e < 4; ++e) bz[mt][e] = b1 ? b1[16 * mt + 4 * g + e] : 0.f;
  int koff[8];
#pragma unroll
  for (int j = 0; j < 8; ++j) {
    const int kap = min(8 * g + j, KC - 1), tap = kap / CIN, ci = kap % CIN;
    koff[j] = ((tap / 3) * TW + tap % 3) * CIN + ci;
  }
  for (int n = blockIdx.x; n < N; n += gridDim.x) {
    __syncthreads();
    const Tin* src = img + (long)n * H * W * CIN;
    for (int i = tid; i < H * W * CIN; i += 256) {
      const int ci = i % CIN, p = i / CIN;
      ft[((p / W + 1) * TW + p % W + 1) * CIN + ci] = (float)src[i] - mean;
    }
    __syncthreads();
    for (int pt = wave; pt < H * W / 16; pt += 4) {
      const int y = pt / (W / 16), x0 = (pt % (W / 16)) * 16;
      const float* pb = ft + (y * TW + x0 + lx) * CIN;
      bf16x8 B;
#pragma unroll
      for (int j = 0; j < 8; ++j) B[j] = (bf16)((8 * g + j < KC) ? pb[koff[j]] : 0.f);
      f32x4 acc[MT];
#pragma unroll
      for (int mt = 0; mt < MT; ++mt) {
        acc[mt] = f32x4{bz[mt][0], bz[mt][1], bz[mt][2], bz[mt][3]};
        acc[mt] = __builtin_amdgcn_mfma_f32_16x16x32_bf16(Ah[mt], B, acc[mt], 0, 0, 0);
        acc[mt] = __builtin_amdgcn_mfma_f32_16x16x32_bf16(Al[mt], B, acc[mt], 0, 0, 0);
      }
      u32x2 ov[MT];
#pragma unroll
      for (int mt = 0; mt < MT; ++mt) {
        bf16x4 o4;
#pragma unroll
        for (int e = 0; e < 4; ++e) o4[e] = (bf16)fmaxf(acc[mt][e], 0.f);
        ov[mt] = *(const u32x2*)&o4;
      }
      bf16* orow = out + (((long)n * H + y) * W + x0 + lx) * C;
      if constexpr (MT == 1) {
        *(u32x2*)(orow + 4 * g) = ov[0];
      } else {
#pragma unroll
        for (int mp = 0; mp < MT / 2; ++mp) {
          const auto s0 = __builtin_amdgcn_permlane16_swap(ov[2 * mp][0], ov[2 * mp + 1][0], false, false);
          const auto s1 = __builtin_amdgcn_permlane16_swap(ov[2 * mp][1], ov[2 * mp + 1][1], false, false);
          *(u32x4*)(orow + 16 * (2 * mp + (g & 1)) + 8 * (g >> 1)) = u32x4{s0[0], s1[0], s0[1], s1[1]};
        }
      }
    }
  }
}

template <int W_, int K>
struct StemK {
  static constexpr int W = W_, CIN = 3, KC = K * K * CIN, TW = W + K - 1;
  static constexpr int KS = (KC + 31) / 32;
  static constexpr int BRF = 512 / W;
  static constexpr int BRW = 256 / W;
  static constexpr int MT = (KC + 1 + 15) / 16;
  static constexpr int MTW = (MT + 3) / 4;
};

template <int W, int K, int ROWS, typename Tin>
__device__ __forceinline__ void stemk_stage(const Tin* __restrict__ img, int n, int y0, int H, float mean,
                                            float* __restrict__ ft, int tid) {
  constexpr int CIN = 3, TW = W + K - 1, R = K / 2;
  for (int i = tid; i < ROWS * TW * CIN; i += 256) {
    const int ci = i % CIN, c = (i / CIN) % TW, r = i / (CIN * TW);
    const int gy = y0 + r - R, gx = c - R;
    float v = 0.f;
    if ((unsigned)gy < (unsigned)H && (unsigned)gx < (unsigned)W)
      v = (float)img[(((long)n * H + gy) * W + gx) * CIN + ci] - mean;
    ft[i] = v;
  }
}

template <int C, int W, int K, typename Tin>
__global__ __launch_bounds__(256) void k_stem_fwd_kxk(const Tin* __restrict__ img, const float* __restrict__ w1,
                                                      const float* __restrict__ b1, int N, int H, float mean,
                                                      float inv_std, bf16* __restrict__ out) {
  using G = StemK<W, K>;
  constexpr int CIN = 3, TW = G::TW, KC = G::KC, KS = G::KS, MT = C / 16, BR = G::BRF, ROWS = BR + K - 1;
  __shared__ float ft[ROWS * TW * CIN];
  const int tid = threadIdx.x, lane = tid & 63, wave = tid >> 6;
  const int g = lane >> 4, lx = lane & 15;
  bf16x8 Ah[MT][KS], Al[MT][KS];
#pragma unroll
  for (int mt = 0; mt < MT; ++mt)
#pragma unroll
    for (int ks = 0; ks < KS; ++ks)
#pragma unroll
      for (int j = 0; j < 8; ++j) {
        const int kap = 32 * ks + 8 * g + j;
        const float wv = kap < KC ? w1[kap * C + 16 * mt + lx] * inv_std : 0.f;
        const bf16 hi = (bf16)wv;
        Ah[mt][ks][j] = hi;
        Al[mt][ks][j] = (bf16)(wv - (float)hi);
      }
  float bz[MT][4];
#pragma unroll
  for (int mt = 0; mt < MT; ++mt)
#pragma unroll
    for (int e = 0; e < 4; ++e) bz[mt][e] = b1 ? b1[16 * mt + 4 * g + e] : 0.f;
  int koff[KS][8];
#pragma unroll
  for (int ks = 0; ks < KS; ++ks)
#pragma unroll
    for (int j = 0; j < 8; ++j) {
      const int kap = min(32 * ks + 8 * g + j, KC - 1), tap = kap / CIN, ci = kap % CIN;
      koff[ks][j] = ((tap / K) * TW + tap % K) * CIN + ci;
    }
  const int nb = (H + BR - 1) / BR;
  const long items = (long)N * nb;
  for (long item = blockIdx.x; item < items; item += gridDim.x) {
    const int n = (int)(item / nb), y0 = (int)(item % nb) * BR;
    __syncthreads();
    stemk_stage<W, K, ROWS>(img, n, y0, H, mean, ft, tid);
    __syncthreads();
    const int rows = min(BR, H - y0), ntiles = (rows * W + 15) / 16;
    for (int pt = wave; pt < ntiles; pt += 4) {
      const int p = 16 * pt + lx, yl = p / W, x = p % W;
      const float* pb = ft + (yl * TW + x) * CIN;
      bf16x8 B[KS];
#pragma unroll
      for (int ks = 0; ks < KS; ++ks)
#pragma unroll
        for (int j = 0; j < 8; ++j) B[ks][j] = (bf16)((32 * ks + 8 * g + j < KC) ? pb[koff[ks][j]] : 0.f);
      f32x4 acc[MT];
#pragma unroll
      for (int mt = 0; mt < MT; ++mt) {
        acc[mt] = f32x4{bz[mt][0], bz[mt][1], bz[mt][2], bz[mt][3]};
#pragma unroll
        for (int ks = 0; ks < KS; ++ks) {
          acc[mt] = __builtin_amdgcn_mfma_f32_16x16x32_bf16(Ah[mt][ks], B[ks], acc[mt], 0, 0, 0);
          acc[mt] = __builtin_amdgcn_mfma_f32_16x16x32_bf16(Al[mt][ks], B[ks], acc[mt], 0, 0, 0);
        }
      }
      u32x2 ov[MT];
#pragma unroll
      for (int mt = 0; mt < MT; ++mt) {
        bf16x4 o4;
#pragma unroll
        for (int e = 0; e < 4; ++e) o4[e] = (bf16)fmaxf(acc[mt][e], 0.f);
        ov[mt] = *(const u32x2*)&o4;
      }
      const bool live = y0 + yl < H;
      bf16* orow = out + (((long)n * H + y0 + yl) * W + x) * C;
      if constexpr (MT == 1) {
        if (live) *(u32x2*)(orow + 4 * g) = ov[0];
      } else {
#pragma unroll
        for (int mp = 0; mp < MT / 2; ++mp) {
          const auto s0 = __builtin_amdgcn_permlane16_swap(ov[2 * mp][0], ov[2 * mp + 1][0], false, false);
          const auto s1 = __builtin_amdgcn_permlane16_swap(ov[2 * mp][1], ov[2 * mp + 1][1], false, false);
          if (live) *(u32x4*)(orow + 16 * (2 * mp + (g & 1)) + 8 * (g >> 1)) = u32x4{s0[0], s1[0], s0[1], s1[1]};
        }
      }
    }
  }
}

template <int C, int W, int K, typename Tin>
__global__ __launch_bounds__(256) void k_stem_wgrad_kxk(const Tin* __restrict__ img, const bf16* __restrict__ dz1,
                                                        int N, int H, float mean, float inv_std,
                                                        float* __restrict__ slabs) {
  using G = StemK<W, K>;
  constexpr int CIN = 3, TW = G::TW, KC = G::KC, MT = G::MT, MTW = G::MTW, NT = C / 16, BR = G::BRW;
  constexpr int ROWS = BR + K - 1, PS = C + 8, C8 = C / 8, NPX = BR * W;
  __shared__ float ft[ROWS * TW * CIN];
  __shared__ __attribute__((aligned(16))) bf16 dzt[NPX * PS];
  const int tid = threadIdx.x, lane = tid & 63, wave = tid >> 6;
  const int g = lane >> 4, lx = lane & 15, q = lx >> 2, pq = lx & 3;
  int koff[MTW], kind[MTW];
#pragma unroll
  for (int i = 0; i < MTW; ++i) {
    const int mt = wave + 4 * i, kap = 16 * mt + lx;
    const int kc = min(kap, KC - 1), tap = kc / CIN, ci = kc % CIN;
    koff[i] = ((tap / K) * TW + tap % K) * CIN + ci;
    kind[i] = (mt < MT && kap < KC) ? 0 : (mt < MT && kap == KC) ? 1 : 2;
  }
  f32x4 acc[MTW][NT];
#pragma unroll
  for (int i = 0; i < MTW; ++i)
#pragma unroll
    for (int nt = 0; nt < NT; ++nt) acc[i][nt] = f32x4{0.f, 0.f, 0.f, 0.f};
  typedef short s16x8 __attribute__((ext_vector_type(8)));
  const int nb = (H + BR - 1) / BR;
  const long items = (long)N * nb;
  const long i0 = (long)blockIdx.x * items / gridDim.x, i1 = (long)(blockIdx.x + 1) * items / gridDim.x;
  for (long item = i0; item < i1; ++item) {
    const int n = (int)(item / nb), y0 = (int)(item % nb) * BR;
    __syncthreads();
    stemk_stage<W, K, ROWS>(img, n, y0, H, mean, ft, tid);
    const bf16* src = dz1 + ((long)n * H + y0) * W * C;
    for (int i = tid; i < NPX * C8; i += 256) {
      const int P = i / C8, c8 = i % C8;
      uint4 v = make_uint4(0u, 0u, 0u, 0u);
      if (y0 + P / W < H) v = *(const uint4*)(src + 8L * i);
      *(uint4*)(dzt + P * PS + 8 * c8) = v;
    }
    __syncthreads();
    const int rows = min(BR, H - y0), nch = (rows * W + 31) / 32;
    for (int ch = 0; ch < nch; ++ch) {
      const int k1 = 32 * ch + 4 * g + q;
      bf16x8 B[NT];
#pragma unroll
      for (int nt = 0; nt < NT; ++nt) {
        const s16x4 a = __builtin_amdgcn_ds_read_tr16_b64_v4i16((ASR_LDS s16x4*)(dzt + k1 * PS + 16 * nt + 4 * pq));
        const s16x4 b =
            __builtin_amdgcn_ds_read_tr16_b64_v4i16((ASR_LDS s16x4*)(dzt + (k1 + 16) * PS + 16 * nt + 4 * pq));
        const s16x8 c = {a[0], a[1], a[2], a[3], b[0], b[1], b[2], b[3]};
        B[nt] = __builtin_bit_cast(bf16x8, c);
      }
      const int pa = 32 * ch + 4 * g, pb = pa + 16;
      const float* fa = ft + ((pa / W) * TW + pa % W) * CIN;
      const float* fb = ft + ((pb / W) * TW + pb % W) * CIN;
#pragma unroll
      for (int i = 0; i < MTW; ++i) {
        if (wave + 4 * i < MT) {
          bf16x8 A;
#pragma unroll
          for (int j = 0; j < 4; ++j) {
            A[j] = (bf16)(kind[i] == 0 ? fa[CIN * j + koff[i]] : kind[i] == 1 ? 1.f : 0.f);
            A[4 + j] = (bf16)(kind[i] == 0 ? fb[CIN * j + koff[i]] : kind[i] == 1 ? 1.f : 0.f);
          }
#pragma unroll
          for (int nt = 0; nt < NT; ++nt)
            acc[i][nt] = __builtin_amdgcn_mfma_f32_16x16x32_bf16(A, B[nt], acc[i][nt], 0, 0, 0);
        }
      }
    }
  }
  mfma_bf16_settle();
  float* slab = slabs + (long)blockIdx.x * (KC * C + C);
#pragma unroll
  for (int i = 0; i < MTW; ++i)
#pragma unroll
    for (int nt = 0; nt < NT; ++nt)
#pragma unroll
      for (int e = 0; e < 4; ++e) {
        const int m = 16 * (wave + 4 * i) + 4 * g + e;
        if (m <= KC) slab[m * C + 16 * nt + lx] = m < KC ? acc[i][nt][e] * inv_std : acc[i][nt][e];
      }
}

}
}
```

### differential_equations_resnet_amd/csrc/asr_block_mfma.hip

```cpp
#include <stdlib.h>

#include "asr_common.h"
#include "asr_internal.h"
#include "asr_blk_common.h"
#include "asr_blk_fwd.h"
#include "asr_blk_bwd.h"
#include "asr_blk_stack.h"
#include "asr_blk_stem.h"

namespace asr {

constexpr int kBwdBR = 4;
constexpr int kFwdBR = 4;

#if ASR_BLK_TRACE
}
extern "C" int asr_debug_blk_trace(void* trace, size_t tbytes, void* clock, size_t cbytes) {
  if (hipMemcpyFromSymbol(trace, HIP_SYMBOL(asr::blk::g_btrace), tbytes) != hipSuccess) return -1;
  return hipMemcpyFromSymbol(clock, HIP_SYMBOL(asr::blk::g_bclock), cbytes) == hipSuccess ? 0 : -1;
}
extern "C" int asr_debug_blk_switch(void* dst, size_t bytes) {
  if (bytes > sizeof(asr::blk::g_bswitch)) bytes = sizeof(asr::blk::g_bswitch);
  return hipMemcpyFromSymbol(dst, HIP_SYMBOL(asr::blk::g_bswitch), bytes) == hipSuccess ? 0 : -1;
}
namespace asr {
#endif

static int persistent_grid(long items) {
  const int cus = launch_cus();
  return (int)std::max<long>(1, std::min<long>({items, (long)cus, (long)kMaxBlockSlabs}));
}

template <int C, int W, int BR, int NW>
static int launch_fwd_v(int mode, const void* x, const void* resid, void* y, uint8_t* mask, const void* w,
                        const float* bias, float h, int N, int H, hipStream_t s) {
  static_assert(NW % blk::Geo<C>::OSPLIT == 0, "waves must cover the o-split");
  const long items = (long)N * ((H + BR - 1) / BR);
  if (items > 0x7fffffffL) return fail(ASR_E_UNSUPPORTED, "bf16 block: too many row bands (%ld)", items);
  const int cus = launch_cus();
  const int grid = (int)std::max<long>(1, std::min<long>(items, (long)cus * (8 / NW)));
  const size_t lds = 2 * (size_t)(BR + 2) * (W + 2) * C * 2;
  if constexpr (C == 64 && W == 32 && BR == 4 && NW == 4) {
    if (!resid || mode == blk::FWD_EULER) {
      const int grid3 = (int)std::max<long>(1, std::min<long>(items, (long)cus * kFwd3Wgs));
      if (mode == blk::FWD_EULER && resid)
        hipLaunchKernelGGL((blk::k_fwd3<C, W, BR, blk::FWD_EULER, 3, true>), dim3(grid3), dim3(256), lds, s,
                           (const bf16*)x, (const bf16*)resid, (bf16*)y, mask, (const bf16*)w, bias, h, N, H);
      else if (mode == blk::FWD_EULER)
        hipLaunchKernelGGL((blk::k_fwd3<C, W, BR, blk::FWD_EULER, 3>), dim3(grid3), dim3(256), lds, s, (const bf16*)x,
                           nullptr, (bf16*)y, mask, (const bf16*)w, bias, h, N, H);
      else
        hipLaunchKernelGGL((blk::k_fwd3<C, W, BR, blk::FWD_CONV, 3>), dim3(grid3), dim3(256), lds, s, (const bf16*)x,
                           nullptr, (bf16*)y, mask, (const bf16*)w, bias, h, N, H);
      ASR_LAUNCH_CHECK("k_fwd3");
      return ASR_OK;
    }
  }
  if constexpr (C >= 32) {
    if (mode == blk::FWD_EULER && resid) {
      hipLaunchKernelGGL((blk::k_fwd_pipe<C, W, BR, blk::FWD_EULER, NW, true>), dim3(grid), dim3(64 * NW), lds, s,
                         (const bf16*)x, (const bf16*)resid, (bf16*)y, mask, (const bf16*)w, bias, h, N, H);
    } else if (mode == blk::FWD_EULER) {
      hipLaunchKernelGGL((blk::k_fwd_pipe<C, W, BR, blk::FWD_EULER, NW>), dim3(grid), dim3(64 * NW), lds, s,
                         (const bf16*)x, nullptr, (bf16*)y, mask, (const bf16*)w, bias, h, N, H);
    } else {
      hipLaunchKernelGGL((blk::k_fwd_pipe<C, W, BR, blk::FWD_CONV, NW>), dim3(grid), dim3(64 * NW), lds, s,
                         (const bf16*)x, nullptr, (bf16*)y, mask, (const bf16*)w, bias, h, N, H);
    }
  } else {
    if (mode == blk::FWD_EULER)
      hipLaunchKernelGGL((blk::k_fwd<C, W, BR, blk::FWD_EULER, NW>), dim3(grid), dim3(64 * NW), lds, s,
                         (const bf16*)x, (const bf16*)resid, (bf16*)y, mask, (const bf16*)w, bias, h, N, H);
    else
      hipLaunchKernelGGL((blk::k_fwd<C, W, BR, blk::FWD_CONV, NW>), dim3(grid), dim3(64 * NW), lds, s,
                         (const bf16*)x, (const bf16*)resid, (bf16*)y, mask, (const bf16*)w, bias, h, N, H);
  }
  ASR_LAUNCH_CHECK("k_fwd");
  return ASR_OK;
}

template <int C, int W>
static int launch_fwd(int mode, const void* x, const void* resid, void* y, uint8_t* mask, const void* w,
                      const float* bias, float h, int N, int H, hipStream_t s) {
  return launch_fwd_v<C, W, 4, 4>(mode, x, resid, y, mask, w, bias, h, N, H, s);
}

template <int C, int W>
static int launch_bwd(int mode, const void* dy, const void* x, const uint8_t* mask, const void* w, float h,
                      float two_gamma, int N, int H, void* dx, float* slabs, int* nslabs, const void* extra,
                      int skip_dy, int relu_dx, int* relu_done, const float* fold_slabs, int fold_P, float* fold_grp,
                      int* fold_done, int accum, hipStream_t s) {
  const long items = (long)N * ((H + kBwdBR - 1) / kBwdBR);
  if (items > 0x7fffffffL) return fail(ASR_E_UNSUPPORTED, "bf16 block: too many row bands (%ld)", items);
  const int grid = persistent_grid(items);
  *nslabs = grid;
  using L = blk::BwdLds<C, W, kBwdBR>;
  const size_t red = (size_t)(12288 + 4 * 64) * 4;
  const size_t lds = std::max((size_t)(extra ? L::TOTAL_XT : L::TOTAL), red);
#define ASR_LAUNCH_BWD(M, XT)                                                                                    \
  hipLaunchKernelGGL((blk::k_bwd<C, W, kBwdBR, M, XT>), dim3(grid), dim3(512), lds, s, (const bf16*)dy, (const bf16*)x, \
                     mask, (const bf16*)w, h, two_gamma, N, H, (bf16*)dx, slabs, (const bf16*)extra, skip_dy, accum)
  const bool xt = extra != nullptr || skip_dy != 0 || accum != 0;
  if constexpr (C == 64) {
    const bool xt2 = extra && accum && !skip_dy && mode == blk::BWD_EULER && !relu_dx;
    if (xt2 || (!extra && !accum && (mode == blk::BWD_EULER || !skip_dy))) {
      using L2 = blk::Bwd2Lds<C, W, kBwdBR>;
      const size_t lds2 = std::max((size_t)L2::TOTAL, red);
      const long fchunks = (long)((fold_P + 31) / 32) * ((9 * C * C + C) / 4);
      if ((fchunks + grid - 1) / grid > 512) fold_P = 0;
#define ASR_LAUNCH_BWD3(M, RO, XT)                                                                            \
  hipLaunchKernelGGL((blk::k_bwd3<C, W, kBwdBR, M, RO, XT>), dim3(grid), dim3(768), lds2, s, (const bf16*)dy,    \
                     (const bf16*)x, mask, (const bf16*)w, h, two_gamma, N, H, (bf16*)dx, slabs, fold_slabs, fold_P, \
                     fold_grp, skip_dy, (const bf16*)extra)
      if (xt2) ASR_LAUNCH_BWD3(blk::BWD_EULER, false, true);
      else if (mode == blk::BWD_EULER && relu_dx) {
        ASR_LAUNCH_BWD3(blk::BWD_EULER, true, false);
        if (relu_done) *relu_done = 1;
      } else if (mode == blk::BWD_EULER) ASR_LAUNCH_BWD3(blk::BWD_EULER, false, false);
      else ASR_LAUNCH_BWD3(blk::BWD_CONV, false, false);
#undef ASR_LAUNCH_BWD3
      ASR_LAUNCH_CHECK("k_bwd3");
      if (fold_done) *fold_done = fold_P > 0;
      return ASR_OK;
    }
  }
  if (mode == blk::BWD_EULER) {
    if (xt) ASR_LAUNCH_BWD(blk::BWD_EULER, true);
    else ASR_LAUNCH_BWD(blk::BWD_EULER, false);
  } else {
    if (xt) ASR_LAUNCH_BWD(blk::BWD_CONV, true);
    else ASR_LAUNCH_BWD(blk::BWD_CONV, false);
  }
#undef ASR_LAUNCH_BWD
  ASR_LAUNCH_CHECK("k_bwd");
  return ASR_OK;
}

static size_t stem_wgrad_mfma_lds(int H, int C) {
  return (size_t)H * 34 * 64 + 2 * 8 * 34 * (C / 8) * 16 + (size_t)(H + 2) * 34 * 3 * 4;
}

bool stem_wgrad_mfma_supported(int Cin, int H, int W, int C) {
  return Cin == 3 && W == 32 && (C == 64 || C == 16) && H % 8 == 0 && H >= 8 &&
         stem_wgrad_mfma_lds(H, C) <= 160 * 1024;
}

int stem_wgrad_mfma(const void* img, int input_u8, const void* dz1, int N, int H, int W, int Cin, int C, float mean,
                    float inv_std, int use_norm, float* slabs, int* nslabs, hipStream_t s) {
  if (!stem_wgrad_mfma_supported(Cin, H, W, C)) return fail(ASR_E_UNSUPPORTED, "stem wgrad (MFMA): unsupported shape");
  const int cus = launch_cus();
  const int grid = std::max(1, std::min(N, std::min(cus, kMaxBlockSlabs)));
  *nslabs = grid;
  const size_t lds = std::max(stem_wgrad_mfma_lds(H, C), (size_t)4 * 32 * C * 4);
  const float m = use_norm ? mean : 0.f, is = use_norm ? inv_std : 1.f;
#define ASR_STEMW(CC, TI)                                                                                   \
  hipLaunchKernelGGL((blk::k_stem_wgrad_mfma<CC, TI>), dim3(grid), dim3(256), lds, s, (const TI*)img, \
                     (const bf16*)dz1, N, H, m, is, slabs)
  if (C == 64) {
    if (input_u8) ASR_STEMW(64, uint8_t);
    else ASR_STEMW(64, float);
  } else {
    if (input_u8) ASR_STEMW(16, uint8_t);
    else ASR_STEMW(16, float);
  }
#undef ASR_STEMW
  ASR_LAUNCH_CHECK("k_stem_wgrad_mfma");
  return ASR_OK;
}

bool stem_fwd_mfma_supported(int Cin, int H, int W, int C) {
  const size_t lds = (size_t)(H + 2) * 34 * 3 * 4;
  return Cin == 3 && W == 32 && (C == 64 || C == 16) && H >= 1 && lds <= 160 * 1024;
}

int stem_fwd_mfma(const void* img, int input_u8, const float* w1, const float* b1, int N, int H, int W, int Cin, int C,
                  float mean, float inv_std, int use_norm, void* out, hipStream_t s) {
  if (!stem_fwd_mfma_supported(Cin, H, W, C)) return fail(ASR_E_UNSUPPORTED, "stem fwd (MFMA): unsupported shape");
  const int cus = launch_cus();
  const int grid = std::max(1, std::min(N, 4 * cus));
  const size_t lds = (size_t)(H + 2) * 34 * 3 * 4;
  const float m = use_norm ? mean : 0.f, is = use_norm ? inv_std : 1.f;
#define ASR_STEMF(CC, TI)                                                                                     \
  hipLaunchKernelGGL((blk::k_stem_fwd_mfma<CC, TI>), dim3(grid), dim3(256), lds, s, (const TI*)img, w1, b1, N, H, m, \
                     is, (bf16*)out)
  if (C == 64) {
    if (input_u8) ASR_STEMF(64, uint8_t);
    else ASR_STEMF(64, float);
  } else {
    if (input_u8) ASR_STEMF(16, uint8_t);
    else ASR_STEMF(16, float);
  }
#undef ASR_STEMF
  ASR_LAUNCH_CHECK("k_stem_fwd_mfma");
  return ASR_OK;
}

bool stem_kxk_supported(int K, int Cin, int W, int C) {
  return (K == 5 || K == 7) && Cin == 3 && (W == 32 || W == 16 || W == 8) && (C == 16 || C == 32 || C == 64);
}

#define ASR_STEMK_CASES(K_)                                                                                     \
  ASR_STEMK(K_, 16, 8) ASR_STEMK(K_, 16, 16) ASR_STEMK(K_, 16, 32) ASR_STEMK(K_, 32, 8) ASR_STEMK(K_, 32, 16)   \
  ASR_STEMK(K_, 32, 32) ASR_STEMK(K_, 64, 8) ASR_STEMK(K_, 64, 16) ASR_STEMK(K_, 64, 32)

template <int C, int W, int K, typename TI>
static int launch_stem_fwd_kxk(const void* img, const float* w1, const float* b1, int N, int H, float m, float is,
                               void* out, hipStream_t s) {
  const long items = (long)N * ((H + blk::StemK<W, K>::BRF - 1) / blk::StemK<W, K>::BRF);
  const int grid = (int)std::max<long>(1, std::min<long>(items, 2L * launch_cus()));
  hipLaunchKernelGGL((blk::k_stem_fwd_kxk<C, W, K, TI>), dim3(grid), dim3(256), 0, s, (const TI*)img, w1, b1, N, H, m,
                     is, (bf16*)out);
  ASR_LAUNCH_CHECK("k_stem_fwd_kxk");
  return ASR_OK;
}

int stem_fwd_kxk(int K, const void* img, int input_u8, const float* w1, const float* b1, int N, int H, int W, int Cin,
                 int C, float mean, float inv_std, int use_norm, void* out, hipStream_t s) {
  if (!stem_kxk_supported(K, Cin, W, C) || N < 1 || H < 1)
    return fail(ASR_E_UNSUPPORTED, "stem fwd (MFMA, K=%d): unsupported shape", K);
  const float m = use_norm ? mean : 0.f, is = use_norm ? inv_std : 1.f;
#define ASR_STEMK(K_, C_, W_)                                                                                  \
  if (K == K_ && C == C_ && W == W_)                                                                           \
    return input_u8 ? launch_stem_fwd_kxk<C_, W_, K_, uint8_t>(img, w1, b1, N, H, m, is, out, s)               \
                    : launch_stem_fwd_kxk<C_, W_, K_, float>(img, w1, b1, N, H, m, is, out, s);
  ASR_STEMK_CASES(5)
  ASR_STEMK_CASES(7)
#undef ASR_STEMK
  return fail(ASR_E_UNSUPPORTED, "stem fwd (MFMA, K=%d): unsupported shape", K);
}

template <int C, int W, int K, typename TI>
static int launch_stem_wgrad_kxk(const void* img, const void* dz1, int N, int H, float m, float is, float* slabs,
                                 int* nslabs, hipStream_t s) {
  const long items = (long)N * ((H + blk::StemK<W, K>::BRW - 1) / blk::StemK<W, K>::BRW);
  const int grid = persistent_grid(items);
  *nslabs = grid;
  hipLaunchKernelGGL((blk::k_stem_wgrad_kxk<C, W, K, TI>), dim3(grid), dim3(256), 0, s, (const TI*)img,
                     (const bf16*)dz1, N, H, m, is, slabs);
  ASR_LAUNCH_CHECK("k_stem_wgrad_kxk");
  return ASR_OK;
}

int stem_wgrad_kxk(int K, const void* img, int input_u8, const void* dz1, int N, int H, int W, int Cin, int C,
                   float mean, float inv_std, int use_norm, float* slabs, int* nslabs, hipStream_t s) {
  *nslabs = 0;
  if (!stem_kxk_supported(K, Cin, W, C) || N < 1 || H < 1)
    return fail(ASR_E_UNSUPPORTED, "stem wgrad (MFMA, K=%d): unsupported shape", K);
  const float m = use_norm ? mean : 0.f, is = use_norm ? inv_std : 1.f;
#define ASR_STEMK(K_, C_, W_)                                                                                  \
  if (K == K_ && C == C_ && W == W_)                                                                           \
    return input_u8 ? launch_stem_wgrad_kxk<C_, W_, K_, uint8_t>(img, dz1, N, H, m, is, slabs, nslabs, s)      \
                    : launch_stem_wgrad_kxk<C_, W_, K_, float>(img, dz1, N, H, m, is, slabs, nslabs, s);
  ASR_STEMK_CASES(5)
  ASR_STEMK_CASES(7)
#undef ASR_STEMK
  return fail(ASR_E_UNSUPPORTED, "stem wgrad (MFMA, K=%d): unsupported shape", K);
}
#undef ASR_STEMK_CASES

int block_fwd_mfma(int mode, const void* x, const void* resid, void* y, uint8_t* mask, const void* w,
                   const float* bias, float h, int N, int H, int W, int C, hipStream_t s) {
  if (W != 32) return fail(ASR_E_UNSUPPORTED, "bf16 block: W=%d not supported (W must be 32)", W);
  switch (C) {
    case 16: return launch_fwd<16, 32>(mode, x, resid, y, mask, w, bias, h, N, H, s);
    case 32: return launch_fwd<32, 32>(mode, x, resid, y, mask, w, bias, h, N, H, s);
    case 64: return launch_fwd<64, 32>(mode, x, resid, y, mask, w, bias, h, N, H, s);
  }
  return fail(ASR_E_UNSUPPORTED, "bf16 block: C=%d not supported (16, 32, 64)", C);
}

bool block_stack_fwd_supported(int N, int H, int W, int C) {
  return C == 64 && W == 32 && N >= 1 && (H + kFwdBR - 1) / kFwdBR >= 4;
}

static int stack_fwd_grid(int N) { return std::max(1, std::min(N, 2 * launch_cus())); }
static size_t stack_fwd_lds(int W, int C) { return 3 * (size_t)(kFwdBR + 2) * (W + 2) * C * 2; }

int block_stack_fwd_mfma(const void* x0, void* ys, long y_stride, uint8_t* masks, long mask_stride, const void* w,
                         long w_stride, const float* bias, long bias_stride, float h, int N, int H, int W, int C, int L,
                         hipStream_t s, int slots) {
  if (!block_stack_fwd_supported(N, H, W, C) || L < 1)
    return fail(ASR_E_UNSUPPORTED, "stack forward: needs C=64, W=32, >= 4 row bands per image (C=%d W=%d H=%d)", C, W, H);
  if (y_stride < (long)N * H * W * C) return fail(ASR_E_ARG, "stack forward: y_stride smaller than one activation");
  if (slots != 0 && slots != 2) return fail(ASR_E_ARG, "stack forward: slots must be 0 or 2");
  const int grid = stack_fwd_grid(N);
  const size_t lds = stack_fwd_lds(W, C);
  hipLaunchKernelGGL((blk::k_fwd3_stack<64, 32, kFwdBR>), dim3(grid), dim3(256), lds, s, (const bf16*)x0,
                     (bf16*)ys, y_stride, masks, mask_stride, (const bf16*)w, w_stride, bias, bias_stride, h, N, H, L,
                     slots);
  ASR_LAUNCH_CHECK("k_fwd3_stack");
  return ASR_OK;
}

static int g_stack_grid_override = 0;

static size_t stack_bwd_lds() { return (size_t)blk::Bwd2Lds<64, 32, kBwdBR>::TOTAL + 16; }

static int stack_bwd_resident_per_cu() {
  static int dev_cached = -1, per = 0;
  int dev = 0;
  if (hipGetDevice(&dev) != hipSuccess) return 0;
  if (dev != dev_cached) {
    int a = 0, b = 0, c = 0, d = 0;
    if (hipOccupancyMaxActiveBlocksPerMultiprocessor(&a, blk::k_bwd3_stack<64, 32, kBwdBR, false, false>, 768,
                                                     stack_bwd_lds()) != hipSuccess ||
        hipOccupancyMaxActiveBlocksPerMultiprocessor(&b, blk::k_bwd3_stack<64, 32, kBwdBR, true, false>, 768,
                                                     stack_bwd_lds()) != hipSuccess ||
        hipOccupancyMaxActiveBlocksPerMultiprocessor(&c, blk::k_bwd3_stack<64, 32, kBwdBR, false, true>, 768,
                                                     stack_bwd_lds()) != hipSuccess ||
        hipOccupancyMaxActiveBlocksPerMultiprocessor(&d, blk::k_bwd3_stack<64, 32, kBwdBR, true, true>, 768,
                                                     stack_bwd_lds()) != hipSuccess)
      return 0;
    per = std::min(std::min(a, b), std::min(c, d));
    dev_cached = dev;
  }
  return per;
}

bool block_stack_bwd_supported(int N, int H, int W, int C) {
  return C == 64 && W == 32 && N >= 1 && (H + kBwdBR - 1) / kBwdBR >= 4 && stack_bwd_resident_per_cu() >= 1;
}

int block_stack_bwd_grid(int N) {
  const int cus = launch_cus();
  const int cap = g_stack_grid_override > 0 ? g_stack_grid_override : cus;
  return std::max(1, std::min(N, std::min(cap, kMaxBlockSlabs)));
}

int stack_done_words(int L) { return 2 * L + 4; }

long stack_slab_floats(int C, int pair) { return pair ? (long)PairSlabLayout::ES : 9L * C * C + C; }

int block_stack_bwd_mfma(void* dbuf0, void* dbuf1, const void* xs, long x_stride, const uint8_t* masks,
                         long mask_stride, const void* w, long w_stride, float h, float two_gamma, int N, int H, int W,
                         int C, int L, int ro0, float* slabs, long slab_stride, float* grp, long grp_stride,
                         unsigned* done, int* lfold_out, hipStream_t s, const void* xm, const uint8_t* masks2,
                         void* gbuf, const void* gtop, int fold, int pair) {
  if (!block_stack_bwd_supported(N, H, W, C) || L < 1)
    return fail(ASR_E_UNSUPPORTED, "stack backward: needs C=64, W=32, >= 4 row bands per image (C=%d W=%d H=%d)", C, W, H);
  const int grid = block_stack_bwd_grid(N);
  const long ES = stack_slab_floats(C, pair);
  if (slab_stride < (long)grid * ES) return fail(ASR_E_ARG, "stack backward: slab_stride too small");
  const long fchunks = (long)((grid + 31) / 32) * (ES / 4);
  const int lfold = fold && (fchunks + grid - 1) / grid <= 512 ? 2 : L;
  if (lfold_out) *lfold_out = lfold;
  ASR_TRY(hip_check(hipMemsetAsync(done, 0, (size_t)stack_done_words(L) * 4, s), "hipMemsetAsync"));
  unsigned* skipf = done + L + 4;
  const size_t lds = stack_bwd_lds();
#define ASR_STACK_BWD(RK, PR)                                                                                   \
  hipLaunchKernelGGL((blk::k_bwd3_stack<64, 32, kBwdBR, RK, PR>), dim3(grid), dim3(768), lds, s, (bf16*)dbuf0,         \
                     (bf16*)dbuf1, (const bf16*)xs, x_stride, masks, mask_stride, (const bf16*)w, w_stride, h,         \
                     two_gamma, N, H, L, RK ? 0 : ro0, slabs, slab_stride, grp, grp_stride, done, skipf, lfold,        \
                     RK ? (const bf16*)xm : nullptr, RK ? masks2 : nullptr, RK ? (bf16*)gbuf : nullptr,                \
                     RK ? nullptr : (const bf16*)gtop)
  if (xm) {
    if (!masks2 || !gbuf) return fail(ASR_E_ARG, "stack backward (RK2): masks2 and the g buffer are required");
    if (pair) ASR_STACK_BWD(true, true);
    else ASR_STACK_BWD(true, false);
  } else {
    if (pair) ASR_STACK_BWD(false, true);
    else ASR_STACK_BWD(false, false);
  }
#undef ASR_STACK_BWD
  ASR_LAUNCH_CHECK("k_bwd3_stack");
  return ASR_OK;
}

__global__ __launch_bounds__(256) void k_reduce_slabs_flagged(const float* __restrict__ slabs, long slab_stride, long ES,
                                                              int P, float* __restrict__ grp, long grp_stride, int L,
                                                              int lfold, const unsigned* __restrict__ flags) {
  const long e = blockIdx.x * (long)blockDim.x + threadIdx.x;
  const int g = blockIdx.y;
  const int p0 = 32 * g, p1 = min(P, p0 + 32);
  for (int l = 0; l < L; ++l) {
    if (l >= lfold && flags[l] == 0u) continue;
    if (e >= ES) continue;
    const float* in = slabs + (long)l * slab_stride;
    float acc0 = 0.f, acc1 = 0.f, acc2 = 0.f, acc3 = 0.f;
    int p = p0;
    for (; p + 3 < p1; p += 4) {
      acc0 += in[(long)p * ES + e];
      acc1 += in[(long)(p + 1) * ES + e];
      acc2 += in[(long)(p + 2) * ES + e];
      acc3 += in[(long)(p + 3) * ES + e];
    }
    for (; p < p1; ++p) acc0 += in[(long)p * ES + e];
    grp[(long)l * grp_stride + (long)g * ES + e] = (acc0 + acc1) + (acc2 + acc3);
  }
}

int stack_bwd_reduce_rest(const float* slabs, long slab_stride, int grid, long ES, float* grp, long grp_stride, int L,
                          int lfold, const unsigned* done, hipStream_t s) {
  const int G = (grid + 31) / 32;
  hipLaunchKernelGGL(k_reduce_slabs_flagged, dim3((unsigned)((ES + 255) / 256), G), dim3(256), 0, s, slabs,
                     slab_stride, ES, grid, grp, grp_stride, L, lfold, done + L + 4);
  ASR_LAUNCH_CHECK("k_reduce_slabs_flagged");
  return ASR_OK;
}

int block_stack_fwd_rk2_mfma(const void* x0, void* ys, void* xm, long y_stride, uint8_t* masks, uint8_t* masks2,
                             long mask_stride, const void* w, long w_stride, const float* bias, long bias_stride,
                             float h, int N, int H, int W, int C, int L, hipStream_t s) {
  if (!block_stack_fwd_supported(N, H, W, C) || L < 1 || !xm)
    return fail(ASR_E_UNSUPPORTED, "RK2 stack forward: needs C=64, W=32, >= 4 row bands per image");
  if (y_stride < (long)N * H * W * C) return fail(ASR_E_ARG, "RK2 stack forward: y_stride smaller than one activation");
  const int grid = stack_fwd_grid(N);
  const size_t lds = stack_fwd_lds(W, C);
  hipLaunchKernelGGL((blk::k_fwd3_stack<64, 32, kFwdBR, true>), dim3(grid), dim3(256), lds, s, (const bf16*)x0,
                     (bf16*)ys, y_stride, masks, mask_stride, (const bf16*)w, w_stride, bias, bias_stride, h, N, H, L, 0,
                     (bf16*)xm, masks2);
  ASR_LAUNCH_CHECK("k_fwd3_stack<RK2>");
  return ASR_OK;
}

int block_bwd_mfma(int mode, const void* dy, const void* x, const uint8_t* mask, const void* w, float h,
                   float two_gamma, int N, int H, int W, int C, void* dx, float* slabs, int* nslabs, const void* extra,
                   int skip_dy, hipStream_t s, int relu_dx, int* relu_done, const float* fold_slabs, int fold_P,
                   float* fold_grp, int* fold_done, int accum) {
  if (relu_done) *relu_done = 0;
  if (fold_done) *fold_done = 0;
  if (fold_P > kMaxBlockSlabs) fold_P = 0;
  if (W != 32) return fail(ASR_E_UNSUPPORTED, "bf16 block: W=%d not supported (W must be 32)", W);
  switch (C) {
    case 16:
      return launch_bwd<16, 32>(mode, dy, x, mask, w, h, two_gamma, N, H, dx, slabs, nslabs, extra, skip_dy, relu_dx,
                                relu_done, fold_slabs, fold_P, fold_grp, fold_done, accum, s);
    case 32:
      return launch_bwd<32, 32>(mode, dy, x, mask, w, h, two_gamma, N, H, dx, slabs, nslabs, extra, skip_dy, relu_dx,
                                relu_done, fold_slabs, fold_P, fold_grp, fold_done, accum, s);
    case 64:
      return launch_bwd<64, 32>(mode, dy, x, mask, w, h, two_gamma, N, H, dx, slabs, nslabs, extra, skip_dy, relu_dx,
                                relu_done, fold_slabs, fold_P, fold_grp, fold_done, accum, s);
  }
  return fail(ASR_E_UNSUPPORTED, "bf16 block: C=%d not supported (16, 32, 64)", C);
}

}

extern "C" int asr_debug_stack_backward(int grid) {
  if (grid < 0 || grid > asr::kMaxBlockSlabs)
    return asr::fail(ASR_E_ARG, "asr_debug_stack_backward: grid must be in 0..%d", asr::kMaxBlockSlabs);
  asr::g_stack_grid_override = grid;
  return ASR_OK;
}

extern "C" int asr_stack_status(int reset) {
  unsigned* d = nullptr;
  if (hipMalloc(&d, sizeof(unsigned)) != hipSuccess) return asr::fail(ASR_E_HIP, "asr_stack_status: hipMalloc failed");
  int rs = reset ? 1 : 0;
  void* args[] = {&rs, &d};
  hipError_t e = hipLaunchKernel((const void*)asr::blk::k_stack_status_take, dim3(1), dim3(1), args, 0, (hipStream_t)0);
  unsigned n = 0;
  if (e == hipSuccess) e = hipMemcpy(&n, d, sizeof(n), hipMemcpyDeviceToHost);
  (void)hipFree(d);
  if (e != hipSuccess) return asr::fail(ASR_E_HIP, "asr_stack_status: %s", hipGetErrorString(e));
  return (int)std::min<unsigned>(n, 0x7fffffffu);
}

#if ASR_STAMP_BUILD
extern "C" int asr_debug_stamps(void* host, size_t bytes) {
  if (bytes > sizeof(asr::blk::g_stamps)) bytes = sizeof(asr::blk::g_stamps);
  return hipMemcpyFromSymbol(host, HIP_SYMBOL(asr::blk::g_stamps), bytes) == hipSuccess ? 0 : -4;
}
#endif
```

### differential_equations_resnet_amd/csrc/asr_internal.h

```cpp
#pragma once
#include "asr_common.h"

namespace asr {

enum { F_EULER = 0, F_CONV = 1, F_RELU = 2, B_EULER = 3, B_CONV = 4 };

constexpr int kMaxBlockSlabs = 512;
constexpr int kMaxStemSlabs = kMaxBlockSlabs;

int cu_count();
inline int launch_cus() { const int cus = cu_count(); return cus > 0 ? cus : 256; }
int check_ws_device(const void* ws, const char* who);
long theta_count(int C, int kind, int antisymmetric);
int param_map(int C, int kind, int antisymmetric, int32_t* w_src, int32_t* theta_dst);
int param_is_antisymmetric(int kind, int antisymmetric);
int param_map_transpose(int C, const int32_t* w_src, int32_t* w_bwd);
long theta_count_k(int C, int k, int kind, int antisymmetric);
int param_map_k(int C, int k, int kind, int antisymmetric, int32_t* w_src, int32_t* theta_dst);
int param_map_transpose_k(int C, int k, const int32_t* w_src, int32_t* w_bwd);
constexpr int kMaxPackJobs = 16;
int theta_to_w_bf16_jobs(const PackJob* jobs, int njobs, hipStream_t s);
int theta_to_w_bf16(const float* theta, long theta_stride, int L, int C, const int32_t* w_src, float gamma, void* w,
                    long w_stride, bool balance, hipStream_t s, const int32_t* theta_dst = nullptr,
                    long n_theta = 0);
int reduce_and_project(const float* slabs, int P, long E, int Cb, const int32_t* theta_dst, long n_theta,
                       float* dtheta, float* dbias, float* dw_out, float* ws, hipStream_t s);
size_t reduce_ws_bytes(int P, long ES);
int reduce_groups(int P);
int reduce_slabs_to_groups(const float* slabs, int P, long ES, float* grp, hipStream_t s);
int reduce_slab_layers(const float* slabs, long slab_stride, int P, long ES, float* grp, long grp_stride, int L,
                       hipStream_t s);
int project_layers(float* grp, long grp_stride, int G, long E, int Cb, const int32_t* theta_dst, long n_theta,
                   int L, float* out, long out_stride, hipStream_t s);
int theta_dst_pair(const int32_t* in, long n_theta, int C, int32_t* out, hipStream_t s);
int theta_dst_pair_host(const int32_t* in, long n_theta, int C, int32_t* out);

int block_fwd_mfma(int mode, const void* x, const void* resid, void* y, uint8_t* mask, const void* w,
                   const float* bias, float h, int N, int H, int W, int C, hipStream_t s);
int block_bwd_mfma(int mode, const void* dy, const void* x, const uint8_t* mask, const void* w, float h,
                   float two_gamma, int N, int H, int W, int C, void* dx, float* slabs, int* nslabs, const void* extra,
                   int skip_dy, hipStream_t s, int relu_dx = 0, int* relu_done = nullptr,
                   const float* fold_slabs = nullptr, int fold_P = 0, float* fold_grp = nullptr,
                   int* fold_done = nullptr, int accum = 0);
int stem_wgrad_mfma(const void* img, int input_u8, const void* dz1, int N, int H, int W, int Cin, int C, float mean,
                    float inv_std, int use_norm, float* slabs, int* nslabs, hipStream_t s);
bool stem_wgrad_mfma_supported(int Cin, int H, int W, int C);
int stem_fwd_mfma(const void* img, int input_u8, const float* w1, const float* b1, int N, int H, int W, int Cin, int C,
                  float mean, float inv_std, int use_norm, void* out, hipStream_t s);
bool stem_fwd_mfma_supported(int Cin, int H, int W, int C);
bool stem_kxk_supported(int K, int Cin, int W, int C);
int stem_fwd_kxk(int K, const void* img, int input_u8, const float* w1, const float* b1, int N, int H, int W, int Cin,
                 int C, float mean, float inv_std, int use_norm, void* out, hipStream_t s);
int stem_wgrad_kxk(int K, const void* img, int input_u8, const void* dz1, int N, int H, int W, int Cin, int C,
                   float mean, float inv_std, int use_norm, float* slabs, int* nslabs, hipStream_t s);
bool block_stack_fwd_supported(int N, int H, int W, int C);
int block_stack_fwd_mfma(const void* x0, void* ys, long y_stride, uint8_t* masks, long mask_stride, const void* w,
                         long w_stride, const float* bias, long bias_stride, float h, int N, int H, int W, int C, int L,
                         hipStream_t s, int slots = 0);
int block_stack_fwd_rk2_mfma(const void* x0, void* ys, void* xm, long y_stride, uint8_t* masks, uint8_t* masks2,
                             long mask_stride, const void* w, long w_stride, const float* bias, long bias_stride,
                             float h, int N, int H, int W, int C, int L, hipStream_t s);
bool block_stack_bwd_supported(int N, int H, int W, int C);
int block_stack_bwd_grid(int N);
int stack_done_words(int L);
long stack_slab_floats(int C, int pair);
int block_stack_bwd_mfma(void* dbuf0, void* dbuf1, const void* xs, long x_stride, const uint8_t* masks,
                         long mask_stride, const void* w, long w_stride, float h, float two_gamma, int N, int H, int W,
                         int C, int L, int ro0, float* slabs, long slab_stride, float* grp, long grp_stride,
                         unsigned* done, int* lfold_out, hipStream_t s, const void* xm = nullptr,
                         const uint8_t* masks2 = nullptr, void* gbuf = nullptr, const void* gtop = nullptr,
                         int fold = 1, int pair = 0);
int stack_bwd_reduce_rest(const float* slabs, long slab_stride, int grid, long ES, float* grp, long grp_stride, int L,
                          int lfold, const unsigned* done, hipStream_t s);

int conv_f32(int fmode, const void* xin, void* out, uint8_t* mask, const float* w, const float* bias, float h,
             float two_gamma, const float* dy, int N, int H, int W, int Ci, int Co, int out_bf16, hipStream_t s,
             const float* extra = nullptr, int K = 3);
int conv_f32_k(int fmode, int K, const void* xin, void* out, uint8_t* mask, const float* w, const float* bias, float h,
               float two_gamma, const float* dy, int N, int H, int W, int C, hipStream_t s, const float* extra);
int make_dz(int fmode, const void* dy, const uint8_t* mask, const void* relu_src, float h, int N, int H, int W, int C,
            int src_bf16, float* dz, hipStream_t s);
int wgrad_f32(const void* x, int x_bf16, const float* dz, int N, int H, int W, int Ci, int Co, float* slabs,
              int* nslabs, hipStream_t s, int K = 3);
int wgrad_f32_chunks(int N, int H);
int f32_block_slab_rows(int N, int H, int W, int C);
bool conv32_fused_bwd_supported(int W, int C);
int conv32_bwd_fused(const float* dy, const uint8_t* mask, float h, const float* x, const float* w, float two_gamma,
                     const float* extra, bool skip_dy, int N, int H, int W, int C, float* dx, bool need_w,
                     float* slabs, int* nslabs, hipStream_t s);
bool convb_supported(int W, int C);
int bf16_block_slab_rows(int N, int H, int W, int C);
int convb_forward(const void* x, void* y, uint8_t* mask, const void* w, const float* bias, float h, int N, int H, int W,
                  int C, hipStream_t s, bool conv_only = false);
int convb_backward(const void* dy, const uint8_t* mask, const void* x, const void* w, float h, float two_gamma, int N,
                   int H, int W, int C, void* dx, bool need_w, float* slabs, int* nslabs, hipStream_t s,
                   bool conv_only = false);
int convert_bf16_f32(const void* src, void* dst, long n, int to_f32, hipStream_t s);
bool stage_img_supported(int H, int W, int C, int dtype);
int stage_img_forward(int dtype, const void* x0, void* ys, long y_stride, uint8_t* masks, long mask_stride,
                      const void* w, long w_stride, const float* bias, long bias_stride, float h, int N, int H, int W,
                      int C, int L, hipStream_t s);
int stage_img_backward(int dtype, const void* dyL, void* dys, long d_stride, void* dx0, const uint8_t* masks,
                       long mask_stride, const void* w, long w_stride, float h, float two_gamma, int N, int H, int W,
                       int C, int L, hipStream_t s);
int wgrad_layers(int dtype, const void* x0, long x_stride, const void* dys, long d_stride, const uint8_t* masks,
                 long mask_stride, float h, int N, int H, int W, int C, int L, float* slabs, long slab_stride,
                 int* nslabs, hipStream_t s);

bool convk_bf16_supported(int K, int W, int C);
int convk_bf16(int fmode, int K, const void* xin, void* out, uint8_t* mask, const void* w, const float* bias, float h,
               float two_gamma, const uint8_t* dmask, int N, int H, int W, int C, hipStream_t s);
int wgradk_bf16_slab_rows(int K, int N, int H, int W, int C);
int wgradk_bf16(int K, const void* x, const void* dy, const uint8_t* mask, float h, int N, int H, int W, int C,
                float* slabs, int* nslabs, hipStream_t s);

bool deep16_supported(int H, int W, int C);
int deep16_forward(const void* x0, void* y0, long y_stride, uint8_t* mask0, long mask_stride, const void* wpack,
                   const float* bias, long bias_stride, float h, int N, int L, bool store_all, hipStream_t s);
size_t deep16_slab_bytes(int N, int L);
int deep16_backward(void* dbufA, void* dbufB, const void* xs, long x_stride, const uint8_t* masks, long mask_stride,
                    const void* wpack, float h, float two_gamma, int N, int L, float* slabs, int* slab_rows,
                    int* dx0_in_b, hipStream_t s);

bool stem_supported(int Cin, int H, int W, int C);
int stem_forward(const void* img, int input_u8, const float* w1, const float* b1, int N, int H, int W, int Cin, int C,
                 float mean, float inv_std, int use_norm, void* out, int out_bf16, hipStream_t s);
int stem_wgrad(const void* img, int input_u8, const void* dx1, const void* x1, int act_bf16, int N, int H, int W,
               int Cin, int C, float mean, float inv_std, int use_norm, float* slabs, int* nslabs, hipStream_t s);
int head(const void* xL, int act_bf16, const float* fck, const float* fcb, const float* targets, int N, int HW, int C,
         int K, float* probs, float* loss_per, float* dlogits, float* gap, void* dxL, hipStream_t s,
         void* growL = nullptr);
int head_param_grads(const float* gap, const float* dlogits, int N, int C, int K, float* dfck, float* dfcb,
                     const float* loss_per, float* loss_out, hipStream_t s);

int augment_batch(const void* src, long n_src, const asr_aug_plan* plan, const asr_aug_item* items, int N, void* dst,
                  hipStream_t s);

int conv_backward_keep_slabs(const void* dy, const void* x, const uint8_t* mask, const void* w, float h, float gamma,
                             int N, int H, int W, int C, void* dx, void* ws, float* slabs, int* nsl, hipStream_t s);
int relu_grad_bf16(void* d, const void* x, long n, hipStream_t s);
constexpr int kFusedNone = 0;
constexpr int kFusedDeep16 = 1;
constexpr int kFusedImg = 2;
int fused_stage_kind(int H, int W, int C, int dtype);
int fused_stage_forward(int kind, int dtype, const void* x0, void* ys, long y_stride, uint8_t* masks, long mask_stride,
                        const void* w, long w_stride, const float* bias, long bias_stride, float h, int N, int H, int W,
                        int C, int L, bool store_all, hipStream_t s);
int fused_stage_backward(const char* who, int kind, int dtype, void* d, void* e, int* in_e, void* dx0_copy, void* dys,
                         const void* xs, long x_stride, const uint8_t* masks, long mask_stride, const void* w,
                         long w_stride, float h, float two_gamma, int N, int H, int W, int C, int L, float* slabs,
                         long slab_stride, int slab_rows, float* grp, long grp_stride, const int32_t* theta_dst,
                         long n_theta, float* dparams, long dp_stride, hipStream_t s);

}
```

### differential_equations_resnet_amd/csrc/asr_stem_head.hip

```cpp
#include <math.h>

#include "asr_common.h"
#include "asr_internal.h"


namespace asr {

template <int CIN>
__device__ __forceinline__ void zero_tile(float* tile, int H, int W) {
  for (int i = threadIdx.x; i < (H + 2) * (W + 2) * CIN; i += blockDim.x) tile[i] = 0.f;
}

template <int CIN, typename Tin>
__device__ __forceinline__ void stage_image(const Tin* __restrict__ img, float* tile, int H, int W, float mean,
                                            float inv_std, int use_norm) {
  constexpr int EPV = 16 / sizeof(Tin);
  constexpr int KV = 4;
  const int TW = W + 2, nel = H * W * CIN;
  const bool vec_ok = ((uintptr_t)img % 16 == 0);
  const int nvec = vec_ok ? nel / EPV : 0;
  for (int v0 = threadIdx.x; v0 < nvec; v0 += KV * blockDim.x) {
    uint4 r[KV];
#pragma unroll
    for (int k = 0; k < KV; ++k) {
      const int vi = v0 + k * blockDim.x;
      r[k] = vi < nvec ? *(const uint4*)(img + (long)vi * EPV) : make_uint4(0, 0, 0, 0);
    }
#pragma unroll
    for (int k = 0; k < KV; ++k) {
      const int vi = v0 + k * blockDim.x;
      if (vi >= nvec) continue;
      const Tin* e = (const Tin*)&r[k];
#pragma unroll
      for (int j = 0; j < EPV; ++j) {
        const int o = vi * EPV + j, c = o % CIN, pix = o / CIN;
        float v = (float)e[j];
        if (use_norm) v = (v - mean) * inv_std;
        tile[((pix / W + 1) * TW + pix % W + 1) * CIN + c] = v;
      }
    }
  }
  for (int o = nvec * EPV + threadIdx.x; o < nel; o += blockDim.x) {
    const int c = o % CIN, pix = o / CIN;
    float v = (float)img[o];
    if (use_norm) v = (v - mean) * inv_std;
    tile[((pix / W + 1) * TW + pix % W + 1) * CIN + c] = v;
  }
}

typedef float f32x2 __attribute__((ext_vector_type(2)));

template <int CIN, typename Tin, typename Tout, int VEC>
__global__ __launch_bounds__(256) void k_stem_fwd(const Tin* __restrict__ img, const float* __restrict__ w1,
                                                  const float* __restrict__ b1, int N, int H, int W, int C,
                                                  float mean, float inv_std, int use_norm, Tout* __restrict__ out) {
  extern __shared__ __attribute__((aligned(16))) float sm[];
  float* tile = sm;
  constexpr int VP = (VEC + 1) / 2;
  const int NG = C / VEC, PLN = max(1, 256 / NG);
  const int cg = threadIdx.x % NG, pl = threadIdx.x / NG;
  const bool active = threadIdx.x < PLN * NG;
  f32x2 wr[9 * CIN][VP], bz[VP];
#pragma unroll
  for (int k = 0; k < 9 * CIN; ++k)
#pragma unroll
    for (int v = 0; v < VP; ++v)
      wr[k][v] = f32x2{active ? w1[k * C + cg * VEC + 2 * v] : 0.f,
                       (active && 2 * v + 1 < VEC) ? w1[k * C + cg * VEC + 2 * v + 1] : 0.f};
#pragma unroll
  for (int v = 0; v < VP; ++v)
    bz[v] = f32x2{(active && b1) ? b1[cg * VEC + 2 * v] : 0.f,
                  (active && b1 && 2 * v + 1 < VEC) ? b1[cg * VEC + 2 * v + 1] : 0.f};
  const int TW = W + 2;
  zero_tile<CIN>(tile, H, W);
  for (int n = blockIdx.x; n < N; n += gridDim.x) {
    __syncthreads();
    stage_image<CIN>(img + (long)n * H * W * CIN, tile, H, W, mean, inv_std, use_norm);
    __syncthreads();
    if (!active) continue;
    for (int p = pl; p < H * W; p += PLN) {
      const int x = p % W, y = p / W;
      f32x2 acc[VP];
#pragma unroll
      for (int v = 0; v < VP; ++v) acc[v] = bz[v];
#pragma unroll
      for (int tap = 0; tap < 9; ++tap) {
        const float* tp = tile + ((y + tap / 3) * TW + x + tap % 3) * CIN;
#pragma unroll
        for (int ci = 0; ci < CIN; ++ci) {
          const float xv = tp[ci];
#pragma unroll
          for (int v = 0; v < VP; ++v) acc[v] = __builtin_elementwise_fma(f32x2{xv, xv}, wr[tap * CIN + ci][v], acc[v]);
        }
      }
      Tout* o = out + ((long)n * H * W + p) * C + cg * VEC;
      if constexpr (VEC == 4 && sizeof(Tout) == 2) {
        bf16x4 r;
#pragma unroll
        for (int v = 0; v < 4; ++v) r[v] = (bf16)fmaxf(acc[v / 2][v % 2], 0.f);
        *(bf16x4*)o = r;
      } else {
#pragma unroll
        for (int v = 0; v < VEC; ++v) o[v] = from_f32<Tout>(fmaxf(acc[v / 2][v % 2], 0.f));
      }
    }
  }
}

template <int CIN, typename Tin, typename T>
__global__ __launch_bounds__(256) void k_stem_wgrad(const Tin* __restrict__ img, const T* __restrict__ dx1,
                                                    const T* __restrict__ x1, int N, int H, int W, int C, float mean,
                                                    float inv_std, int use_norm, float* __restrict__ slabs) {
  extern __shared__ __attribute__((aligned(16))) float sm[];
  constexpr int KC = 9 * CIN;
  const int tid = threadIdx.x, lane = tid & 63, wave = tid >> 6;
  const int NG = C / 4;
  int NGP = 1;
  while (NGP < NG) NGP <<= 1;
  const int PL = 256 / NGP;
  const int cg = tid % NGP, pl = tid / NGP;
  const int HWa = cg < NG ? H * W : 0;
  f32x2 acc[KC + 1][2];
#pragma unroll
  for (int k = 0; k <= KC; ++k) acc[k][0] = acc[k][1] = f32x2{0.f, 0.f};
  float* tile = sm;
  const int TW = W + 2;
  zero_tile<CIN>(tile, H, W);
  for (int n = blockIdx.x; n < N; n += gridDim.x) {
    __syncthreads();
    stage_image<CIN>(img + (long)n * H * W * CIN, tile, H, W, mean, inv_std, use_norm);
    __syncthreads();
    const T* d = dx1 + (long)n * H * W * C + cg * 4;
    const T* a = x1 + (long)n * H * W * C + cg * 4;
    constexpr int U = 4;
    for (int p0 = pl; p0 < HWa; p0 += U * PL) {
      f32x2 gv[U][2];
#pragma unroll
      for (int u = 0; u < U; ++u) {
        const int p = p0 + u * PL;
        const int pc = p < H * W ? p : 0;
        float dv[4], av[4];
        if constexpr (sizeof(T) == 2) {
          const bf16x4 d4 = *(const bf16x4*)(d + (long)pc * C), a4 = *(const bf16x4*)(a + (long)pc * C);
#pragma unroll
          for (int v = 0; v < 4; ++v) dv[v] = (float)d4[v], av[v] = (float)a4[v];
        } else {
          const float4 d4 = *(const float4*)(d + (long)pc * C), a4 = *(const float4*)(a + (long)pc * C);
          dv[0] = d4.x, dv[1] = d4.y, dv[2] = d4.z, dv[3] = d4.w;
          av[0] = a4.x, av[1] = a4.y, av[2] = a4.z, av[3] = a4.w;
        }
        float g4[4];
#pragma unroll
        for (int v = 0; v < 4; ++v) g4[v] = (p < H * W && av[v] > 0.f) ? dv[v] : 0.f;
        gv[u][0] = f32x2{g4[0], g4[1]};
        gv[u][1] = f32x2{g4[2], g4[3]};
      }
#pragma unroll
      for (int u = 0; u < U; ++u) {
        const int p = p0 + u * PL;
        const int pc = p < H * W ? p : 0;
        const int x = pc % W, y = pc / W;
#pragma unroll
        for (int tap = 0; tap < 9; ++tap) {
          const float* tp = tile + ((y + tap / 3) * TW + x + tap % 3) * CIN;
#pragma unroll
          for (int ci = 0; ci < CIN; ++ci) {
            const float xv = tp[ci];
#pragma unroll
            for (int h = 0; h < 2; ++h)
              acc[tap * CIN + ci][h] = __builtin_elementwise_fma(f32x2{xv, xv}, gv[u][h], acc[tap * CIN + ci][h]);
          }
        }
#pragma unroll
        for (int h = 0; h < 2; ++h) acc[KC][h] += gv[u][h];
      }
    }
  }
#pragma unroll
  for (int k = 0; k <= KC; ++k)
#pragma unroll
    for (int h = 0; h < 2; ++h)
#pragma unroll
      for (int e = 0; e < 2; ++e) {
        float v = acc[k][h][e];
        for (int off = NGP; off < 64; off <<= 1) v += __shfl_xor(v, off);
        acc[k][h][e] = v;
      }
  __syncthreads();
  float* red = sm;
  if (lane < NG)
#pragma unroll
    for (int k = 0; k <= KC; ++k)
#pragma unroll
      for (int v = 0; v < 4; ++v) red[((long)wave * (KC + 1) + k) * C + cg * 4 + v] = acc[k][v / 2][v % 2];
  __syncthreads();
  float* slab = slabs + (long)blockIdx.x * (KC * C + C);
  for (int i = tid; i < (KC + 1) * C; i += blockDim.x) {
    const long st = (long)(KC + 1) * C;
    slab[i] = (red[i] + red[st + i]) + (red[2 * st + i] + red[3 * st + i]);
  }
}

template <typename T, int VEC>
__global__ __launch_bounds__(256) void k_head(const T* __restrict__ xL, const float* __restrict__ fck,
                                              const float* __restrict__ fcb, const float* __restrict__ targets,
                                              int HW, int C, int K, float inv_n, float* __restrict__ probs,
                                              float* __restrict__ loss_per, float* __restrict__ dlogits,
                                              float* __restrict__ gap, T* __restrict__ dxL, T* __restrict__ growL) {
  __shared__ float red[256 * VEC];
  __shared__ float gs[256];
  __shared__ float lg[256];
  __shared__ float dl[256];
  const int n = blockIdx.x, tid = threadIdx.x;
  const int NQ = C / VEC;
  const int PL = max(1, 256 / NQ);
  const int q = tid % NQ, pl = tid / NQ;
  float s[VEC];
#pragma unroll
  for (int v = 0; v < VEC; ++v) s[v] = 0.f;
  if (pl < PL && tid < PL * NQ) {
    const T* base = xL + (long)n * HW * C + q * VEC;
#pragma unroll 8
    for (int p = pl; p < HW; p += PL) {
      if constexpr (VEC == 8 && sizeof(T) == 2) {
        const bf16x8 v8 = *(const bf16x8*)(base + (long)p * C);
#pragma unroll
        for (int v = 0; v < 8; ++v) s[v] += (float)v8[v];
      } else if constexpr (VEC == 4 && sizeof(T) == 4) {
        const float4 v4 = *(const float4*)(base + (long)p * C);
        s[0] += v4.x;
        s[1] += v4.y;
        s[2] += v4.z;
        s[3] += v4.w;
      } else {
#pragma unroll
        for (int v = 0; v < VEC; ++v) s[v] += to_f32(base[(long)p * C + v]);
      }
    }
  }
#pragma unroll
  for (int v = 0; v < VEC; ++v) red[tid * VEC + v] = s[v];
  __syncthreads();
  if (tid < C) {
    const int qq = tid / VEC, v = tid % VEC;
    float t = 0.f;
    for (int p = 0; p < PL; ++p) t += red[(p * NQ + qq) * VEC + v];
    t /= (float)HW;
    gs[tid] = t;
    if (gap) gap[(long)n * C + tid] = t;
  }
  __syncthreads();
  if (tid < K) {
    float a = fcb ? fcb[tid] : 0.f;
    for (int c = 0; c < C; ++c) a = fmaf(gs[c], fck[(long)c * K + tid], a);
    lg[tid] = a;
  }
  __syncthreads();
  if (tid == 0) {
    float m = -INFINITY;
    for (int k = 0; k < K; ++k) m = fmaxf(m, lg[k]);
    float S = 0.f;
    for (int k = 0; k < K; ++k) {
      const float e = expf(lg[k] - m);
      lg[k] = e;
      S += e;
    }
    float s2 = 0.f;
    for (int k = 0; k < K; ++k) {
      lg[k] /= S;
      s2 += lg[k];
      if (probs) probs[(long)n * K + k] = lg[k];
    }
    if (targets) {
      const float eps = 1e-7f;
      float loss = 0.f, sdq_p = 0.f;
      for (int k = 0; k < K; ++k) {
        const float qv = lg[k] / s2;
        const float qc = fminf(fmaxf(qv, eps), 1.f - eps);
        const float t = targets[(long)n * K + k];
        loss -= t * (qv > 1.f - eps ? -eps : logf(qc));
        const float dq = (qv >= eps && qv <= 1.f - eps) ? -t / qc * inv_n : 0.f;
        dl[k] = dq;
        sdq_p += dq * lg[k];
      }
      if (loss_per) loss_per[n] = loss;
      float sp_dp = 0.f;
      for (int k = 0; k < K; ++k) {
        const float dp = dl[k] / s2 - sdq_p / (s2 * s2);
        dl[k] = dp;
        sp_dp += lg[k] * dp;
      }
      for (int k = 0; k < K; ++k) {
        const float d = lg[k] * (dl[k] - sp_dp);
        dl[k] = d;
        if (dlogits) dlogits[(long)n * K + k] = d;
      }
    }
  }
  __syncthreads();
  if (targets && growL) {
    if (tid < C) {
      float a = 0.f;
      for (int k = 0; k < K; ++k) a = fmaf(dl[k], fck[(long)tid * K + k], a);
      growL[(long)n * C + tid] = from_f32<T>(a / (float)HW);
    }
  } else if (targets && dxL) {
    if (tid < C) {
      float a = 0.f;
      for (int k = 0; k < K; ++k) a = fmaf(dl[k], fck[(long)tid * K + k], a);
      gs[tid] = a / (float)HW;
    }
    __syncthreads();
    T* o = dxL + (long)n * HW * C;
    for (long i = tid; i < (long)HW * NQ; i += 256) {
      const int qq = (int)(i % NQ);
      T* dst = o + i * VEC;
      if constexpr (VEC == 8 && sizeof(T) == 2) {
        bf16x8 r;
#pragma unroll
        for (int v = 0; v < 8; ++v) r[v] = (bf16)gs[qq * 8 + v];
        *(bf16x8*)dst = r;
      } else {
#pragma unroll
        for (int v = 0; v < VEC; ++v) dst[v] = from_f32<T>(gs[qq * VEC + v]);
      }
    }
  }
}

__global__ __launch_bounds__(256) void k_head_param_grads(const float* __restrict__ gap,
                                                          const float* __restrict__ dlogits, int N, int C, int K,
                                                          float* __restrict__ dfck, float* __restrict__ dfcb,
                                                          const float* __restrict__ loss_per,
                                                          float* __restrict__ loss_out) {
  __shared__ float red[256];
  const int tid = threadIdx.x, c = blockIdx.x;
  const int NL = max(1, 256 / K);
  const int k = tid % K, nl = tid / K;
  float a = 0.f;
  if (nl < NL && tid < NL * K) {
    for (int n = nl; n < N; n += NL) {
      const float d = dlogits[(long)n * K + k];
      a = (c < C) ? fmaf(gap[(long)n * C + c], d, a) : a + d;
    }
  }
  red[tid] = a;
  __syncthreads();
  if (tid < K) {
    float s = 0.f;
    for (int g = 0; g < NL; ++g) s += red[g * K + tid];
    if (c < C)
      dfck[(long)c * K + tid] = s;
    else
      dfcb[tid] = s;
  }
  if (c == C) {
    __syncthreads();
    float l = 0.f;
    for (int n = tid; n < N; n += 256) l += loss_per[n];
    red[tid] = l;
    __syncthreads();
    for (int w = 128; w > 0; w >>= 1) {
      if (tid < w) red[tid] += red[tid + w];
      __syncthreads();
    }
    if (tid == 0) *loss_out = red[0] / (float)N;
  }
}

bool stem_supported(int Cin, int H, int W, int C) {
  const size_t lds = (size_t)(H + 2) * (W + 2) * Cin * 4;
  const size_t red = (size_t)4 * (9 * Cin + 1) * C * 4;
  return (Cin == 1 || Cin == 3) && C % 4 == 0 && C <= 64 && lds <= 64 * 1024 && red <= 64 * 1024;
}

static int stem_grid(int N) { return std::max(1, std::min(N, kMaxStemSlabs)); }

template <int CIN, typename Tin, typename Tout>
static void launch_stem_fwd(const void* img, const float* w1, const float* b1, int N, int H, int W, int C, float mean,
                            float inv_std, int use_norm, void* out, hipStream_t s) {
  const size_t lds = (size_t)(H + 2) * (W + 2) * CIN * 4;
  if (C % 4 == 0)
    hipLaunchKernelGGL((k_stem_fwd<CIN, Tin, Tout, 4>), dim3(stem_grid(N)), dim3(256), lds, s, (const Tin*)img, w1,
                       b1, N, H, W, C, mean, inv_std, use_norm, (Tout*)out);
  else
    hipLaunchKernelGGL((k_stem_fwd<CIN, Tin, Tout, 1>), dim3(stem_grid(N)), dim3(256), lds, s, (const Tin*)img, w1,
                       b1, N, H, W, C, mean, inv_std, use_norm, (Tout*)out);
}

int stem_forward(const void* img, int input_u8, const float* w1, const float* b1, int N, int H, int W, int Cin, int C,
                 float mean, float inv_std, int use_norm, void* out, int out_bf16, hipStream_t s) {
  if (!stem_supported(Cin, H, W, C)) return fail(ASR_E_UNSUPPORTED, "stem: unsupported shape");
#define ASR_STEM_F(CI, TI, TO) launch_stem_fwd<CI, TI, TO>(img, w1, b1, N, H, W, C, mean, inv_std, use_norm, out, s)
  if (Cin == 3) {
    if (input_u8) { if (out_bf16) ASR_STEM_F(3, uint8_t, bf16); else ASR_STEM_F(3, uint8_t, float); }
    else { if (out_bf16) ASR_STEM_F(3, float, bf16); else ASR_STEM_F(3, float, float); }
  } else {
    if (input_u8) { if (out_bf16) ASR_STEM_F(1, uint8_t, bf16); else ASR_STEM_F(1, uint8_t, float); }
    else { if (out_bf16) ASR_STEM_F(1, float, bf16); else ASR_STEM_F(1, float, float); }
  }
#undef ASR_STEM_F
  ASR_LAUNCH_CHECK("k_stem_fwd");
  return ASR_OK;
}

int stem_wgrad(const void* img, int input_u8, const void* dx1, const void* x1, int act_bf16, int N, int H, int W,
               int Cin, int C, float mean, float inv_std, int use_norm, float* slabs, int* nslabs, hipStream_t s) {
  if (!stem_supported(Cin, H, W, C)) return fail(ASR_E_UNSUPPORTED, "stem: unsupported shape");
  const int grid = stem_grid(N);
  *nslabs = grid;
  const size_t lds = std::max((size_t)(H + 2) * (W + 2) * Cin * 4, (size_t)4 * (9 * Cin + 1) * C * 4);
#define ASR_STEM_W(CI, TI, T)                                                                                   \
  hipLaunchKernelGGL((k_stem_wgrad<CI, TI, T>), dim3(grid), dim3(256), lds, s, (const TI*)img, (const T*)dx1, \
                     (const T*)x1, N, H, W, C, mean, inv_std, use_norm, slabs)
  if (Cin == 3) {
    if (input_u8) { if (act_bf16) ASR_STEM_W(3, uint8_t, bf16); else ASR_STEM_W(3, uint8_t, float); }
    else { if (act_bf16) ASR_STEM_W(3, float, bf16); else ASR_STEM_W(3, float, float); }
  } else {
    if (input_u8) { if (act_bf16) ASR_STEM_W(1, uint8_t, bf16); else ASR_STEM_W(1, uint8_t, float); }
    else { if (act_bf16) ASR_STEM_W(1, float, bf16); else ASR_STEM_W(1, float, float); }
  }
#undef ASR_STEM_W
  ASR_LAUNCH_CHECK("k_stem_wgrad");
  return ASR_OK;
}

int head(const void* xL, int act_bf16, const float* fck, const float* fcb, const float* targets, int N, int HW, int C,
         int K, float* probs, float* loss_per, float* dlogits, float* gap, void* dxL, hipStream_t s, void* growL) {
  if (C > 256 || K > 256) return fail(ASR_E_UNSUPPORTED, "head: C and num_classes must be <= 256");
  const float inv_n = 1.f / (float)N;
  if (act_bf16) {
    if (C % 8 == 0)
      hipLaunchKernelGGL((k_head<bf16, 8>), dim3(N), dim3(256), 0, s, (const bf16*)xL, fck, fcb, targets, HW, C, K,
                         inv_n, probs, loss_per, dlogits, gap, (bf16*)dxL, (bf16*)growL);
    else
      hipLaunchKernelGGL((k_head<bf16, 1>), dim3(N), dim3(256), 0, s, (const bf16*)xL, fck, fcb, targets, HW, C, K,
                         inv_n, probs, loss_per, dlogits, gap, (bf16*)dxL, (bf16*)growL);
  } else {
    if (C % 4 == 0)
      hipLaunchKernelGGL((k_head<float, 4>), dim3(N), dim3(256), 0, s, (const float*)xL, fck, fcb, targets, HW, C,
                         K, inv_n, probs, loss_per, dlogits, gap, (float*)dxL, (float*)growL);
    else
      hipLaunchKernelGGL((k_head<float, 1>), dim3(N), dim3(256), 0, s, (const float*)xL, fck, fcb, targets, HW, C,
                         K, inv_n, probs, loss_per, dlogits, gap, (float*)dxL, (float*)growL);
  }
  ASR_LAUNCH_CHECK("k_head");
  return ASR_OK;
}

int head_param_grads(const float* gap, const float* dlogits, int N, int C, int K, float* dfck, float* dfcb,
                     const float* loss_per, float* loss_out, hipStream_t s) {
  hipLaunchKernelGGL(k_head_param_grads, dim3(C + 1), dim3(256), 0, s, gap, dlogits, N, C, K, dfck, dfcb, loss_per,
                     loss_out);
  ASR_LAUNCH_CHECK("k_head_param_grads");
  return ASR_OK;
}

}
```

### differential_equations_resnet_amd/csrc/asr_theta.hip

```cpp
#include <stdarg.h>
#include <stdio.h>

#include <algorithm>
#include <type_traits>
#include <vector>

#include "asr_common.h"
#include "asr_internal.h"

namespace asr {

static thread_local char g_err[512] = "";

void set_error(const char* fmt, ...) {
  va_list ap;
  va_start(ap, fmt);
  vsnprintf(g_err, sizeof(g_err), fmt, ap);
  va_end(ap);
}

int fail(int code, const char* fmt, ...) {
  va_list ap;
  va_start(ap, fmt);
  vsnprintf(g_err, sizeof(g_err), fmt, ap);
// ... 480 lines not shown
  return (acc0 + acc1) + (acc2 + acc3);
}

__global__ void k_reduce_slabs(const float* __restrict__ in, long E, int P, int per, float* __restrict__ out) {
  const long e = blockIdx.x * (long)blockDim.x + threadIdx.x;
  const int g = blockIdx.y;
  if (e >= E) return;
  const int p0 = g * per, p1 = min(P, p0 + per);
  out[(long)g * E + e] = sum_slab_rows(in, E, e, p0, p1);
}

__global__ void k_project(const float* __restrict__ red_groups, int G, long E, const int32_t* __restrict__ theta_dst,
                          long n_theta, float* __restrict__ dtheta, float* __restrict__ dw_out, int Cb,
                          float* __restrict__ dbias) {
  const long t = blockIdx.x * (long)blockDim.x + threadIdx.x;
  const long ES = E + Cb;
  auto red_at = [&](long e) {
    float a[4] = {0.f, 0.f, 0.f, 0.f};
    int g = 0;
    for (; g + 3 < G; g += 4) {
#pragma unroll
      for (int q = 0; q < 4; ++q) a[q] += red_groups[(long)(g + q) * ES + e];
    }
    for (; g < G; ++g) a[0] += red_groups[(long)g * ES + e];
    return (a[0] + a[1]) + (a[2] + a[3]);
  };
  if (dtheta && t < n_theta) {
    float acc = 0.f;
#pragma unroll
    for (int q = 0; q < 2; ++q) {
      const int32_t v = theta_dst[2 * t + q];
      if (v >= 0) {
        const float d = red_at(v >> 1);
        acc += (v & 1) ? -d : d;
      }
    }
    dtheta[t] = acc;
  }
  if (dw_out && t < E) dw_out[t] = red_at(t);
  if (dbias && t < Cb) dbias[t] = red_at(E + t);
}

}

using namespace asr;

extern "C" {

const char* asr_last_error(void) { return g_err; }
int asr_abi_version(void) { return 11; }

int asr_device_cu_count(void) { return cu_count(); }

long asr_theta_count(int C, int kind, int antisymmetric) { return theta_count(C, kind, antisymmetric); }
long asr_theta_count_k(int C, int kernel_size, int kind, int antisymmetric) {
  return theta_count_k(C, kernel_size, kind, antisymmetric);
}
int asr_param_map_k(int C, int kernel_size, int kind, int antisymmetric, int32_t* w_src, int32_t* theta_dst) {
  return param_map_k(C, kernel_size, kind, antisymmetric, w_src, theta_dst);
}
int asr_param_map_transpose_k(int C, int kernel_size, const int32_t* w_src, int32_t* w_src_bwd) {
  return param_map_transpose_k(C, kernel_size, w_src, w_src_bwd);
}

int asr_param_map(int C, int kind, int antisymmetric, int32_t* w_src, int32_t* theta_dst) {
  return param_map(C, kind, antisymmetric, w_src, theta_dst);
}

int asr_param_is_antisymmetric(int kind, int antisymmetric) { return param_is_antisymmetric(kind, antisymmetric); }

int asr_param_map_transpose(int C, const int32_t* w_src, int32_t* w_src_bwd) {
  return param_map_transpose(C, w_src, w_src_bwd);
}

int asr_param_map_pair(int C, const int32_t* theta_dst, long n_theta, int32_t* theta_dst_pair) {
  if (C != 64 || !theta_dst || !theta_dst_pair || n_theta < 0)
    return fail(ASR_E_ARG, "asr_param_map_pair: C=64 and non-null maps required");
  return theta_dst_pair_host(theta_dst, n_theta, C, theta_dst_pair);
}

long asr_wpack_elems(int C) {
  if (C % 16 != 0) return -1;
  return (long)(C / 16) * ((9 * C + 31) / 32) * 64 * 8;
}

int asr_theta_to_w_k(const float* theta, long theta_stride, int L, int C, int kernel_size, const int32_t* w_src,
                     float gamma, float* w_out, long w_stride, asr_stream_t stream) {
  if (!theta || !w_src || !w_out || L < 1 || C < 1 || L > 65535 || kernel_size < 1)
    return fail(ASR_E_ARG, "asr_theta_to_w_k: bad arguments");
  const long E = (long)kernel_size * kernel_size * C * C;
  if (w_stride < E) return fail(ASR_E_ARG, "asr_theta_to_w_k: w_stride too small");
  dim3 grid((unsigned)std::min<long>((E + 255) / 256, 1024), L);
  hipLaunchKernelGGL(k_theta_to_w_hwio, grid, dim3(256), 0, (hipStream_t)stream, theta, theta_stride, E, w_src, gamma,
                     w_out, w_stride);
  ASR_LAUNCH_CHECK("k_theta_to_w_hwio");
  return ASR_OK;
}

long asr_wpack_elems_k(int C, int kernel_size) {
  if ((kernel_size != 5 && kernel_size != 7) || (C != 16 && C != 32 && C != 64)) return -1;
  return (long)(C / 16) * ((kernel_size * kernel_size * C + 31) / 32) * 64 * 8;
}

int asr_theta_to_w_k_bf16(const float* theta, long theta_stride, int L, int C, int kernel_size, const int32_t* w_src,
                          float gamma, void* w_pack, long w_stride, asr_stream_t stream) {
  if (!theta || !w_src || !w_pack || L < 1 || C < 1 || L > 65535 || kernel_size < 1 || kernel_size > 15 ||
      !(kernel_size & 1))
    return fail(ASR_E_ARG, "asr_theta_to_w_k_bf16: bad arguments");
  const long n = asr_wpack_elems_k(C, kernel_size);
  if (n < 0)
    return fail(ASR_E_UNSUPPORTED,
                "asr_theta_to_w_k_bf16: the bf16 k x k kernels take kernel_size in {5, 7}, C in {16, 32, 64}, "
                "W in {8, 16, 32} (kernel_size=%d C=%d)", kernel_size, C);
  if (w_stride < n) return fail(ASR_E_ARG, "asr_theta_to_w_k_bf16: w_stride too small");
  const int frags = (int)(n / 512);
  hipLaunchKernelGGL(k_theta_to_w_pack_k, dim3((frags + 3) / 4, L), dim3(256), 0, (hipStream_t)stream, theta,
                     theta_stride, C, kernel_size * kernel_size, w_src, gamma, (bf16*)w_pack, w_stride);
  ASR_LAUNCH_CHECK("k_theta_to_w_pack_k");
  return ASR_OK;
}

int asr_theta_to_w(const float* theta, long theta_stride, int L, int C, const int32_t* w_src, float gamma,
                   void* w_out, long w_stride, int dtype, asr_stream_t stream) {
  if (!theta || !w_src || !w_out || L < 1 || C < 1 || L > 65535)
    return fail(ASR_E_ARG, "asr_theta_to_w: bad arguments");
  hipStream_t s = (hipStream_t)stream;
  if (dtype == ASR_F32) {
    const long E = 9L * C * C;
    if (w_stride < E) return fail(ASR_E_ARG, "asr_theta_to_w: w_stride too small");
    dim3 grid((unsigned)std::min<long>((E + 255) / 256, 1024), L);
    hipLaunchKernelGGL(k_theta_to_w_hwio, grid, dim3(256), 0, s, theta, theta_stride, E, w_src, gamma,
                       (float*)w_out, w_stride);
    ASR_LAUNCH_CHECK("k_theta_to_w_hwio");
  } else if (dtype == ASR_BF16) {
    if (C % 16 != 0) return fail(ASR_E_UNSUPPORTED, "asr_theta_to_w: bf16 pack needs C %% 16 == 0 (C=%d)", C);
    if (w_stride < asr_wpack_elems(C)) return fail(ASR_E_ARG, "asr_theta_to_w: w_stride too small");
    return theta_to_w_bf16(theta, theta_stride, L, C, w_src, gamma, w_out, w_stride, true, s);
  } else {
    return fail(ASR_E_ARG, "asr_theta_to_w: bad dtype %d", dtype);
  }
  return ASR_OK;
}

}

namespace asr {

int theta_to_w_bf16(const float* theta, long theta_stride, int L, int C, const int32_t* w_src, float gamma, void* w,
                    long w_stride, bool balance, hipStream_t s, const int32_t* theta_dst, long n_theta) {
  const long n = asr_wpack_elems(C);
  if (!theta || !w_src || !w || L < 1 || L > 65535 || n < 0 || w_stride < n)
    return fail(ASR_E_ARG, "theta_to_w_bf16: bad arguments");
  if (balance && (C == 16 || C == 32 || C == 64)) {
    const PackJob job{theta, theta_stride, L, C, w_src, gamma, w, w_stride, theta_dst, n_theta};
    ASR_TRY(theta_to_w_bf16_jobs(&job, 1, s));
  } else {
    const int frags = (C / 16) * ((9 * C + 31) / 32);
    hipLaunchKernelGGL(k_theta_to_w_pack, dim3((frags + 3) / 4, L), dim3(256), 0, s, theta, theta_stride, C, w_src,
                       gamma, (bf16*)w, w_stride);
    ASR_LAUNCH_CHECK("k_theta_to_w_pack");
  }
  return ASR_OK;
}

int reduce_and_project(const float* slabs, int P, long E, int Cb, const int32_t* theta_dst, long n_theta,
                       float* dtheta, float* dbias, float* dw_out, float* ws, hipStream_t s) {
  const long ES = E + Cb;
  const int per = 32;
  const int G = (P + per - 1) / per;
  float* grp = ws;
  float* fin = ws + (long)G * ES;
  dim3 g1((unsigned)((ES + 255) / 256), G);
  hipLaunchKernelGGL(k_reduce_slabs, g1, dim3(256), 0, s, slabs, ES, P, per, grp);
  ASR_LAUNCH_CHECK("k_reduce_slabs");
  (void)fin;
  const long n = std::max(std::max(dtheta ? n_theta : 0L, dw_out ? E : 0L), (long)Cb);
  hipLaunchKernelGGL(k_project, dim3((unsigned)((n + 255) / 256)), dim3(256), 0, s, grp, G, E, theta_dst,
                     dtheta ? n_theta : 0L, dtheta, dw_out, Cb, dbias);
  ASR_LAUNCH_CHECK("k_project");
  return ASR_OK;
}

size_t reduce_ws_bytes(int P, long ES) { return (size_t)((P + 31) / 32 + 1) * ES * sizeof(float); }

int reduce_groups(int P) { return (P + 31) / 32; }

__global__ void k_reduce_slabs_layers(const float* __restrict__ in, long slab_stride, long E, int P, int per,
                                      float* __restrict__ out, long out_stride) {
  const long e = blockIdx.x * (long)blockDim.x + threadIdx.x;
  const int g = blockIdx.y;
  if (e >= E) return;
  const float* src = in + blockIdx.z * slab_stride;
  const int p0 = g * per, p1 = min(P, p0 + per);
  out[blockIdx.z * out_stride + (long)g * E + e] = sum_slab_rows(src, E, e, p0, p1);
}

int reduce_slab_layers(const float* slabs, long slab_stride, int P, long ES, float* grp, long grp_stride, int L,
                       hipStream_t s) {
  if (L < 1 || P < 1) return ASR_OK;
  dim3 g1((unsigned)((ES + 255) / 256), reduce_groups(P), L);
  hipLaunchKernelGGL(k_reduce_slabs_layers, g1, dim3(256), 0, s, slabs, slab_stride, ES, P, 32, grp, grp_stride);
  ASR_LAUNCH_CHECK("k_reduce_slabs_layers");
  return ASR_OK;
}

int reduce_slabs_to_groups(const float* slabs, int P, long ES, float* grp, hipStream_t s) {
  const int G = reduce_groups(P);
  dim3 g1((unsigned)((ES + 255) / 256), G);
  hipLaunchKernelGGL(k_reduce_slabs, g1, dim3(256), 0, s, slabs, ES, P, 32, grp);
  ASR_LAUNCH_CHECK("k_reduce_slabs");
  return ASR_OK;
}

__global__ void k_project_layers(const float* __restrict__ grp, long grp_stride, int G, long E, int Cb,
                                 const int32_t* __restrict__ theta_dst, long n_theta, float* __restrict__ out,
                                 long out_stride) {
  const int l = blockIdx.y;
  const float* rg = grp + (long)l * grp_stride;
  const long ES = E + Cb;
  const long t = blockIdx.x * (long)blockDim.x + threadIdx.x;
  auto red_at = [&](long e) {
    float a[4] = {0.f, 0.f, 0.f, 0.f};
    int g = 0;
    for (; g + 3 < G; g += 4) {
#pragma unroll
      for (int q = 0; q < 4; ++q) a[q] += rg[(long)(g + q) * ES + e];
    }
    for (; g < G; ++g) a[0] += rg[(long)g * ES + e];
    return (a[0] + a[1]) + (a[2] + a[3]);
  };
  float* o = out + (long)l * out_stride;
  if (t < n_theta) {
    const int32_t v0 = theta_dst[2 * t], v1 = theta_dst[2 * t + 1];
    float acc = 0.f;
    if (v0 >= 0) acc += (v0 & 1) ? -red_at(v0 >> 1) : red_at(v0 >> 1);
    if (v1 >= 0) acc += (v1 & 1) ? -red_at(v1 >> 1) : red_at(v1 >> 1);
    o[t] = acc;
  } else if (t < n_theta + Cb) {
    o[t] = red_at(E + (t - n_theta));
  }
}

__global__ void k_sum_groups(float* __restrict__ grp, long grp_stride, int G, long ES) {
  const long e = blockIdx.x * (long)blockDim.x + threadIdx.x;
  if (e >= ES) return;
  float* rg = grp + (long)blockIdx.y * grp_stride;
  float a[4] = {0.f, 0.f, 0.f, 0.f};
  int g = 0;
  for (; g + 3 < G; g += 4) {
#pragma unroll
    for (int q = 0; q < 4; ++q) a[q] += rg[(long)(g + q) * ES + e];
  }
  for (; g < G; ++g) a[0] += rg[(long)g * ES + e];
  rg[e] = (a[0] + a[1]) + (a[2] + a[3]);
}

__global__ void k_theta_dst_pair(const int32_t* __restrict__ in, long n_theta, int C, int32_t* __restrict__ out) {
  const long j = blockIdx.x * (long)blockDim.x + threadIdx.x;
  if (j >= n_theta) return;
  int32_t o[2] = {-1, -1};
  const int32_t v = in[2 * j];
  if (v >= 0) pair_encode(v >> 1, v & 1, C, o);
  out[2 * j] = o[0];
  out[2 * j + 1] = o[1];
}

int theta_dst_pair(const int32_t* in, long n_theta, int C, int32_t* out, hipStream_t s) {
  if (C != 64) return fail(ASR_E_UNSUPPORTED, "pair-local slabs: C=64 only");
  hipLaunchKernelGGL(k_theta_dst_pair, dim3((unsigned)((n_theta + 255) / 256)), dim3(256), 0, s, in, n_theta, C, out);
  ASR_LAUNCH_CHECK("k_theta_dst_pair");
  return ASR_OK;
}

int theta_dst_pair_host(const int32_t* in, long n_theta, int C, int32_t* out) {
  for (long j = 0; j < n_theta; ++j) {
    const int32_t v0 = in[2 * j], v1 = in[2 * j + 1];
    if (v0 < 0 || v1 < 0) return fail(ASR_E_ARG, "theta %ld: not an antisymmetric pair", j);
    const long e0 = v0 >> 1, e1 = v1 >> 1;
    const int t = (int)(e0 / ((long)C * C)), i = (int)((e0 / C) % C), o = (int)(e0 % C);
    const long mirror = ((long)(8 - t) * C + o) * C + i;
    if (e1 != mirror || ((v0 ^ v1) & 1) == 0) return fail(ASR_E_ARG, "theta %ld: not an antisymmetric pair", j);
    int32_t o2[2] = {-1, -1};
    if (pair_encode(e0, v0 & 1, C, o2) == 0) return fail(ASR_E_ARG, "theta %ld: no pair-local slab entry", j);
    out[2 * j] = o2[0];
    out[2 * j + 1] = o2[1];
  }
  return ASR_OK;
}

int project_layers(float* grp, long grp_stride, int G, long E, int Cb, const int32_t* theta_dst, long n_theta,
                   int L, float* out, long out_stride, hipStream_t s) {
  const long n = n_theta + Cb;
  if (G > 1) {
    hipLaunchKernelGGL(k_sum_groups, dim3((unsigned)((E + Cb + 255) / 256), L), dim3(256), 0, s, grp, grp_stride, G,
                       E + Cb);
    ASR_LAUNCH_CHECK("k_sum_groups");
  }
  hipLaunchKernelGGL(k_project_layers, dim3((unsigned)((n + 255) / 256), L), dim3(256), 0, s, grp, grp_stride, 1, E,
                     Cb, theta_dst, n_theta, out, out_stride);
  ASR_LAUNCH_CHECK("k_project_layers");
  return ASR_OK;
}

}
```

Before: 162,200 images/s.

## Fuse stack-backward slab reduction with theta projection and trim head/stem overheads

Replaces the separate flagged slab reduction and per-layer theta projection kernels with one tail kernel. It uses a precomputed owner map to reduce the slab groups and write the projected antisymmetric parameter gradients directly, skipping the intermediate grp write and re-read. It also clears the stack done-flags inside the head kernel instead of issuing a memset, and parallelises the head softmax/loss across threads. Smaller changes vectorise the stem image staging with 16-byte loads, unroll the head parameter-gradient loop, and cache the status buffer. The new tail kernel recomputes the partial sum for each paired theta entry, so some reduction work is done twice.

```diff
diff --git a/differential_equations_resnet_amd/csrc/asr_api.hip b/differential_equations_resnet_amd/csrc/asr_api.hip
--- a/differential_equations_resnet_amd/csrc/asr_api.hip
+++ b/differential_equations_resnet_amd/csrc/asr_api.hip
@@ -238,6 +238,7 @@
   int stack_grid;
   size_t theta_dst_tm, stack_slabs, stack_done;
   size_t theta_dst_pr;
+  size_t own_tm, own_pr;
   int f32_rows;
   size_t grow;
   BwdWs bw;
@@ -361,6 +362,8 @@
   L.deep_slabs = ws.take(L.deep && tr ? deep16_slab_bytes(c->N, c->L) : 0);
   L.theta_dst_tm = ws.take(L.stack_bwd ? (size_t)L.ntheta * 2 * 4 : 0);
   L.theta_dst_pr = ws.take(L.stack_pair ? (size_t)L.ntheta * 2 * 4 : 0);
+  L.own_tm = ws.take(L.stack_bwd ? (size_t)(L.E + C) * 4 : 0);
+  L.own_pr = ws.take(L.stack_pair ? (size_t)stack_slab_floats(C, 1) * 4 : 0);
   L.stack_slabs = ws.take(L.stack_bwd ? (size_t)c->L * L.stack_grid * (L.E + C) * 4 : 0);
   L.stack_done = ws.take(L.stack_bwd ? (size_t)stack_done_words(c->L) * 4 : 0);
   L.grow = ws.take(L.stack_bwd && !L.rk2 ? (size_t)c->N * C * 2 : 0);
@@ -659,7 +662,7 @@
 }
 
 struct StackWs {
-  size_t da, db, slabs, grp, blk, done, tdst, g, dys, total;
+  size_t da, db, slabs, grp, blk, done, tdst, own, g, dys, total;
   int fused;
   bool stack64;
   int grid;
@@ -689,6 +692,7 @@
     w.grp = c.take((size_t)L * reduce_groups(w.grid) * ES * 4);
     w.done = c.take((size_t)stack_done_words(L) * 4);
     w.tdst = c.take((size_t)2 * 9 * C * C * 4);
+    w.own = c.take((size_t)stack_slab_floats(C, 1) * 4);
     if (rk2) w.g = c.take(act);
   } else {
     w.blk = c.take(bwd_ws_layout(N, H, W, C, dtype).total);
@@ -715,10 +719,12 @@
   ASR_TRY(hip_check(hipMemcpyAsync(dx0, base + ((L & 1) ? Lw.db : Lw.da), act, hipMemcpyDeviceToDevice, s),
                     "hipMemcpyAsync"));
   if (!dparams) return ASR_OK;
-  ASR_TRY(stack_bwd_reduce_rest(slabs, sst, Lw.grid, ES, grp, gst, L, lfold, (const unsigned*)(base + Lw.done), s));
   int32_t* tm = (int32_t*)(base + Lw.tdst);
+  int32_t* own = (int32_t*)(base + Lw.own);
   ASR_TRY(theta_dst_pair(theta_dst, n_theta, C, tm, s));
-  return project_layers(grp, gst, reduce_groups(Lw.grid), ES - C, C, tm, n_theta, L, dparams, n_theta + C, s);
+  ASR_TRY(theta_owner(tm, n_theta, ES - C, C, own, s));
+  return stack_bwd_reduce_rest(slabs, sst, Lw.grid, ES, grp, gst, L, lfold, (const unsigned*)(base + Lw.done), C, tm,
+                               own, n_theta, dparams, n_theta + C, s);
 }
 
 size_t asr_block_stack_backward_workspace_bytes(int N, int H, int W, int C, int L, int dtype) {
@@ -1022,6 +1028,9 @@
     std::vector<int32_t> pr(theta_dst.size());
     ASR_TRY(theta_dst_pair_host(theta_dst.data(), L.ntheta, cfg->C, pr.data()));
     ASR_TRY(hip_check(hipMemcpy(b + L.theta_dst_pr, pr.data(), pr.size() * 4, hipMemcpyHostToDevice), "hipMemcpy"));
+    std::vector<int32_t> own((size_t)stack_slab_floats(cfg->C, 1));
+    ASR_TRY(theta_owner_host(pr.data(), L.ntheta, (long)own.size() - cfg->C, cfg->C, own.data()));
+    ASR_TRY(hip_check(hipMemcpy(b + L.own_pr, own.data(), own.size() * 4, hipMemcpyHostToDevice), "hipMemcpy"));
   }
   if (L.stack_bwd) {
     const int C = cfg->C;
@@ -1033,6 +1042,9 @@
       v = (int32_t)((et << 1) | (v & 1));
     }
     ASR_TRY(hip_check(hipMemcpy(b + L.theta_dst_tm, tm.data(), tm.size() * 4, hipMemcpyHostToDevice), "hipMemcpy"));
+    std::vector<int32_t> own((size_t)L.E + C);
+    ASR_TRY(theta_owner_host(tm.data(), L.ntheta, L.E, C, own.data()));
+    ASR_TRY(hip_check(hipMemcpy(b + L.own_tm, own.data(), own.size() * 4, hipMemcpyHostToDevice), "hipMemcpy"));
   }
   return ASR_OK;
 }
@@ -1102,7 +1114,8 @@
   const bool grow = stacked && !L.rk2 && !(cfg->variant & ASR_VARIANT_FULL_DXL);
   ASR_TRY(head(act(cfg->L), bf, params + L.off_fck, params + L.off_fcb, targets, N, H * W, C, K, probs_ws,
                (float*)(b + L.loss_per), (float*)(b + L.dlogits), (float*)(b + L.gap), grow ? nullptr : dcur, s,
-               grow ? b + L.grow : nullptr));
+               grow ? b + L.grow : nullptr, stacked ? (unsigned*)(b + L.stack_done) : nullptr,
+               stacked ? stack_done_words(cfg->L) : 0));
   ASR_TRY(head_param_grads((const float*)(b + L.gap), (const float*)(b + L.dlogits), N, C, K, grads + L.off_fck,
                            grads + L.off_fcb, (const float*)(b + L.loss_per), loss, s));
   const int32_t* theta_dst = (const int32_t*)(b + L.theta_dst);
@@ -1142,15 +1155,15 @@
                                  sst, grp, L.grp_stride, (unsigned*)(b + L.stack_done), &lfold, s,
                                  L.rk2 ? b + L.xmids : nullptr, L.rk2 ? m1 + (size_t)cfg->L * L.mask_bytes : nullptr,
                                  L.rk2 ? b + L.dxg : nullptr, grow ? b + L.grow : nullptr, fold_on ? 1 : 0,
-                                 pair ? 1 : 0));
+                                 pair ? 1 : 0, 1));
     ASR_TRY(timed_event(cfg, 3, s));
     ASR_TRY(stack_bwd_reduce_rest(slabs, sst, grid, ES, grp, L.grp_stride, cfg->L, lfold,
-                                  (const unsigned*)(b + L.stack_done), s));
+                                  (const unsigned*)(b + L.stack_done), C,
+                                  (const int32_t*)(b + (pair ? L.theta_dst_pr : L.theta_dst_tm)),
+                                  (const int32_t*)(b + (pair ? L.own_pr : L.own_tm)), L.ntheta, grads + L.off_blk,
+                                  L.blk_stride, s));
     if (cfg->L & 1) std::swap(dcur, dnext);
     dz1_fused = ro0;
-    ASR_TRY(project_layers(grp, L.grp_stride, reduce_groups(grid), ES - C, C,
-                           (const int32_t*)(b + (pair ? L.theta_dst_pr : L.theta_dst_tm)), L.ntheta, cfg->L,
-                           grads + L.off_blk, L.blk_stride, s));
     ASR_TRY(timed_event(cfg, 4, s));
   }
   if (L.kxk) {
diff --git a/differential_equations_resnet_amd/csrc/asr_blk_stem.h b/differential_equations_resnet_amd/csrc/asr_blk_stem.h
--- a/differential_equations_resnet_amd/csrc/asr_blk_stem.h
+++ b/differential_equations_resnet_amd/csrc/asr_blk_stem.h
@@ -7,6 +7,37 @@
 
 namespace asr {
 namespace blk {
+
+template <typename Tin>
+__device__ __forceinline__ void stem_stage_image(const Tin* __restrict__ src, float* __restrict__ ft, int H,
+                                                 float mean, int tid) {
+  constexpr int W = 32, CIN = 3, TW = W + 2;
+  constexpr int EPV = 16 / sizeof(Tin), KV = 4;
+  const int nel = H * W * CIN;
+  const int nvec = ((uintptr_t)src % 16 == 0) ? nel / EPV : 0;
+  auto put = [&](int o, float v) {
+    const int ci = o % CIN, p = o / CIN;
+    ft[((p / W + 1) * TW + p % W + 1) * CIN + ci] = v - mean;
+  };
+  for (int v0 = tid; v0 < nvec; v0 += KV * 256) {
+    uint4 r[KV];
+#pragma unroll
+    for (int k = 0; k < KV; ++k) {
+      const int vi = min(v0 + k * 256, nvec - 1);
+      r[k] = *(const uint4*)(src + (long)vi * EPV);
+    }
+#pragma unroll
+    for (int k = 0; k < KV; ++k) {
+      const int vi = v0 + k * 256;
+      if (vi < nvec) {
+        const Tin* e = (const Tin*)&r[k];
+#pragma unroll
+        for (int j = 0; j < EPV; ++j) put(vi * EPV + j, (float)e[j]);
+      }
+    }
+  }
+  for (int o = nvec * EPV + tid; o < nel; o += 256) put(o, (float)src[o]);
+}
 
 template <int C, typename Tin>
 __global__ __launch_bounds__(256) void k_stem_wgrad_mfma(const Tin* __restrict__ img, const bf16* __restrict__ dz1,
@@ -37,11 +68,7 @@
     if (b == 0) {
       const int n = band_n(it);
       __syncthreads();
-      const Tin* src = img + (long)n * H * W * CIN;
-      for (int i = tid; i < H * W * CIN; i += 256) {
-        const int ci = i % CIN, p = i / CIN;
-        ft[((p / W + 1) * TW + p % W + 1) * CIN + ci] = (float)src[i] - mean;
-      }
+      stem_stage_image(img + (long)n * H * W * CIN, ft, H, mean, tid);
       __syncthreads();
       for (int p = tid; p < H * W; p += 256) {
         const int y = p / W, x = p % W;
@@ -140,11 +167,7 @@
   }
   for (int n = blockIdx.x; n < N; n += gridDim.x) {
     __syncthreads();
-    const Tin* src = img + (long)n * H * W * CIN;
-    for (int i = tid; i < H * W * CIN; i += 256) {
-      const int ci = i % CIN, p = i / CIN;
-      ft[((p / W + 1) * TW + p % W + 1) * CIN + ci] = (float)src[i] - mean;
-    }
+    stem_stage_image(img + (long)n * H * W * CIN, ft, H, mean, tid);
     __syncthreads();
     for (int pt = wave; pt < H * W / 16; pt += 4) {
       const int y = pt / (W / 16), x0 = (pt % (W / 16)) * 16;
diff --git a/differential_equations_resnet_amd/csrc/asr_block_mfma.hip b/differential_equations_resnet_amd/csrc/asr_block_mfma.hip
--- a/differential_equations_resnet_amd/csrc/asr_block_mfma.hip
+++ b/differential_equations_resnet_amd/csrc/asr_block_mfma.hip
@@ -1,4 +1,7 @@
 #include <stdlib.h>
+
+#include <mutex>
+#include <vector>
 
 #include "asr_common.h"
 #include "asr_internal.h"
@@ -335,7 +338,7 @@
                          long mask_stride, const void* w, long w_stride, float h, float two_gamma, int N, int H, int W,
                          int C, int L, int ro0, float* slabs, long slab_stride, float* grp, long grp_stride,
                          unsigned* done, int* lfold_out, hipStream_t s, const void* xm, const uint8_t* masks2,
-                         void* gbuf, const void* gtop, int fold, int pair) {
+                         void* gbuf, const void* gtop, int fold, int pair, int done_cleared) {
   if (!block_stack_bwd_supported(N, H, W, C) || L < 1)
     return fail(ASR_E_UNSUPPORTED, "stack backward: needs C=64, W=32, >= 4 row bands per image (C=%d W=%d H=%d)", C, W, H);
   const int grid = block_stack_bwd_grid(N);
@@ -344,7 +347,8 @@
   const long fchunks = (long)((grid + 31) / 32) * (ES / 4);
   const int lfold = fold && (fchunks + grid - 1) / grid <= 512 ? 2 : L;
   if (lfold_out) *lfold_out = lfold;
-  ASR_TRY(hip_check(hipMemsetAsync(done, 0, (size_t)stack_done_words(L) * 4, s), "hipMemsetAsync"));
+  if (!done_cleared)
+    ASR_TRY(hip_check(hipMemsetAsync(done, 0, (size_t)stack_done_words(L) * 4, s), "hipMemsetAsync"));
   unsigned* skipf = done + L + 4;
   const size_t lds = stack_bwd_lds();
 #define ASR_STACK_BWD(RK, PR)                                                                                   \
@@ -363,38 +367,6 @@
   }
 #undef ASR_STACK_BWD
   ASR_LAUNCH_CHECK("k_bwd3_stack");
-  return ASR_OK;
-}
-
-__global__ __launch_bounds__(256) void k_reduce_slabs_flagged(const float* __restrict__ slabs, long slab_stride, long ES,
-                                                              int P, float* __restrict__ grp, long grp_stride, int L,
-                                                              int lfold, const unsigned* __restrict__ flags) {
-  const long e = blockIdx.x * (long)blockDim.x + threadIdx.x;
-  const int g = blockIdx.y;
-  const int p0 = 32 * g, p1 = min(P, p0 + 32);
-  for (int l = 0; l < L; ++l) {
-    if (l >= lfold && flags[l] == 0u) continue;
-    if (e >= ES) continue;
-    const float* in = slabs + (long)l * slab_stride;
-    float acc0 = 0.f, acc1 = 0.f, acc2 = 0.f, acc3 = 0.f;
-    int p = p0;
-    for (; p + 3 < p1; p += 4) {
-      acc0 += in[(long)p * ES + e];
-      acc1 += in[(long)(p + 1) * ES + e];
-      acc2 += in[(long)(p + 2) * ES + e];
-      acc3 += in[(long)(p + 3) * ES + e];
-    }
-    for (; p < p1; ++p) acc0 += in[(long)p * ES + e];
-    grp[(long)l * grp_stride + (long)g * ES + e] = (acc0 + acc1) + (acc2 + acc3);
-  }
-}
-
-int stack_bwd_reduce_rest(const float* slabs, long slab_stride, int grid, long ES, float* grp, long grp_stride, int L,
-                          int lfold, const unsigned* done, hipStream_t s) {
-  const int G = (grid + 31) / 32;
-  hipLaunchKernelGGL(k_reduce_slabs_flagged, dim3((unsigned)((ES + 255) / 256), G), dim3(256), 0, s, slabs,
-                     slab_stride, ES, grid, grp, grp_stride, L, lfold, done + L + 4);
-  ASR_LAUNCH_CHECK("k_reduce_slabs_flagged");
   return ASR_OK;
 }
 
@@ -445,14 +417,22 @@
 }
 
 extern "C" int asr_stack_status(int reset) {
-  unsigned* d = nullptr;
-  if (hipMalloc(&d, sizeof(unsigned)) != hipSuccess) return asr::fail(ASR_E_HIP, "asr_stack_status: hipMalloc failed");
+  static std::mutex mu;
+  static std::vector<unsigned*> words;
+  int dev = 0;
+  if (hipGetDevice(&dev) != hipSuccess || dev < 0) return asr::fail(ASR_E_HIP, "asr_stack_status: hipGetDevice failed");
+  std::lock_guard<std::mutex> lock(mu);
+  if ((size_t)dev >= words.size()) words.resize((size_t)dev + 1, nullptr);
+  if (!words[dev] && hipMalloc(&words[dev], sizeof(unsigned)) != hipSuccess) {
+    words[dev] = nullptr;
+    return asr::fail(ASR_E_HIP, "asr_stack_status: hipMalloc failed");
+  }
+  unsigned* d = words[dev];
   int rs = reset ? 1 : 0;
   void* args[] = {&rs, &d};
   hipError_t e = hipLaunchKernel((const void*)asr::blk::k_stack_status_take, dim3(1), dim3(1), args, 0, (hipStream_t)0);
   unsigned n = 0;
   if (e == hipSuccess) e = hipMemcpy(&n, d, sizeof(n), hipMemcpyDeviceToHost);
-  (void)hipFree(d);
   if (e != hipSuccess) return asr::fail(ASR_E_HIP, "asr_stack_status: %s", hipGetErrorString(e));
   return (int)std::min<unsigned>(n, 0x7fffffffu);
 }
diff --git a/differential_equations_resnet_amd/csrc/asr_internal.h b/differential_equations_resnet_amd/csrc/asr_internal.h
--- a/differential_equations_resnet_amd/csrc/asr_internal.h
+++ b/differential_equations_resnet_amd/csrc/asr_internal.h
@@ -34,6 +34,11 @@
                    int L, float* out, long out_stride, hipStream_t s);
 int theta_dst_pair(const int32_t* in, long n_theta, int C, int32_t* out, hipStream_t s);
 int theta_dst_pair_host(const int32_t* in, long n_theta, int C, int32_t* out);
+int stack_bwd_reduce_rest(const float* slabs, long slab_stride, int grid, long ES, const float* grp, long grp_stride,
+                          int L, int lfold, const unsigned* done, int Cb, const int32_t* theta_dst,
+                          const int32_t* owner, long n_theta, float* out, long out_stride, hipStream_t s);
+int theta_owner(const int32_t* theta_dst, long n_theta, long E, int Cb, int32_t* owner, hipStream_t s);
+int theta_owner_host(const int32_t* theta_dst, long n_theta, long E, int Cb, int32_t* owner);
 
 int block_fwd_mfma(int mode, const void* x, const void* resid, void* y, uint8_t* mask, const void* w,
                    const float* bias, float h, int N, int H, int W, int C, hipStream_t s);
@@ -69,9 +74,7 @@
                          int C, int L, int ro0, float* slabs, long slab_stride, float* grp, long grp_stride,
                          unsigned* done, int* lfold_out, hipStream_t s, const void* xm = nullptr,
                          const uint8_t* masks2 = nullptr, void* gbuf = nullptr, const void* gtop = nullptr,
-                         int fold = 1, int pair = 0);
-int stack_bwd_reduce_rest(const float* slabs, long slab_stride, int grid, long ES, float* grp, long grp_stride, int L,
-                          int lfold, const unsigned* done, hipStream_t s);
+                         int fold = 1, int pair = 0, int done_cleared = 0);
 
 int conv_f32(int fmode, const void* xin, void* out, uint8_t* mask, const float* w, const float* bias, float h,
              float two_gamma, const float* dy, int N, int H, int W, int Ci, int Co, int out_bf16, hipStream_t s,
@@ -129,7 +132,7 @@
                int Cin, int C, float mean, float inv_std, int use_norm, float* slabs, int* nslabs, hipStream_t s);
 int head(const void* xL, int act_bf16, const float* fck, const float* fcb, const float* targets, int N, int HW, int C,
          int K, float* probs, float* loss_per, float* dlogits, float* gap, void* dxL, hipStream_t s,
-         void* growL = nullptr);
+         void* growL = nullptr, unsigned* zero_words = nullptr, int nzero = 0);
 int head_param_grads(const float* gap, const float* dlogits, int N, int C, int K, float* dfck, float* dfcb,
                      const float* loss_per, float* loss_out, hipStream_t s);
 
diff --git a/differential_equations_resnet_amd/csrc/asr_stem_head.hip b/differential_equations_resnet_amd/csrc/asr_stem_head.hip
--- a/differential_equations_resnet_amd/csrc/asr_stem_head.hip
+++ b/differential_equations_resnet_amd/csrc/asr_stem_head.hip
@@ -206,12 +206,20 @@
                                               const float* __restrict__ fcb, const float* __restrict__ targets,
                                               int HW, int C, int K, float inv_n, float* __restrict__ probs,
                                               float* __restrict__ loss_per, float* __restrict__ dlogits,
-                                              float* __restrict__ gap, T* __restrict__ dxL, T* __restrict__ growL) {
+                                              float* __restrict__ gap, T* __restrict__ dxL, T* __restrict__ growL,
+                                              unsigned* __restrict__ zero_words, int nzero) {
   __shared__ float red[256 * VEC];
   __shared__ float gs[256];
   __shared__ float lg[256];
+  __shared__ float ex[256];
+  __shared__ float pr[256];
   __shared__ float dl[256];
+  __shared__ float tx[256];
+  __shared__ float lx[256];
+  __shared__ float dpv[256];
   const int n = blockIdx.x, tid = threadIdx.x;
+  if (n == 0)
+    for (int i = tid; i < nzero; i += 256) zero_words[i] = 0u;
   const int NQ = C / VEC;
   const int PL = max(1, 256 / NQ);
   const int q = tid % NQ, pl = tid / NQ;
@@ -220,7 +228,7 @@
   for (int v = 0; v < VEC; ++v) s[v] = 0.f;
   if (pl < PL && tid < PL * NQ) {
     const T* base = xL + (long)n * HW * C + q * VEC;
-#pragma unroll 8
+#pragma unroll 16
     for (int p = pl; p < HW; p += PL) {
       if constexpr (VEC == 8 && sizeof(T) == 2) {
         const bf16x8 v8 = *(const bf16x8*)(base + (long)p * C);
@@ -250,51 +258,62 @@
     if (gap) gap[(long)n * C + tid] = t;
   }
   __syncthreads();
-  if (tid < K) {
+  const bool mine = tid < K;
+  if (mine) {
     float a = fcb ? fcb[tid] : 0.f;
     for (int c = 0; c < C; ++c) a = fmaf(gs[c], fck[(long)c * K + tid], a);
     lg[tid] = a;
   }
   __syncthreads();
-  if (tid == 0) {
+  {
     float m = -INFINITY;
     for (int k = 0; k < K; ++k) m = fmaxf(m, lg[k]);
+    if (mine) ex[tid] = expf(lg[tid] - m);
+  }
+  __syncthreads();
+  float pk = 0.f;
+  {
     float S = 0.f;
+    for (int k = 0; k < K; ++k) S += ex[k];
+    if (mine) {
+      pk = ex[tid] / S;
+      pr[tid] = pk;
+      if (probs) probs[(long)n * K + tid] = pk;
+    }
+  }
+  __syncthreads();
+  if (targets) {
+    const float eps = 1e-7f;
+    float s2 = 0.f;
+    for (int k = 0; k < K; ++k) s2 += pr[k];
+    float dq = 0.f;
+    if (mine) {
+      const float qv = pk / s2;
+      const float qc = fminf(fmaxf(qv, eps), 1.f - eps);
+      tx[tid] = targets[(long)n * K + tid];
+      lx[tid] = qv > 1.f - eps ? -eps : logf(qc);
+      dq = (qv >= eps && qv <= 1.f - eps) ? -tx[tid] / qc * inv_n : 0.f;
+      dl[tid] = dq;
+    }
+    __syncthreads();
+    float loss = 0.f, sdq_p = 0.f;
     for (int k = 0; k < K; ++k) {
-      const float e = expf(lg[k] - m);
-      lg[k] = e;
-      S += e;
-    }
-    float s2 = 0.f;
-    for (int k = 0; k < K; ++k) {
-      lg[k] /= S;
-      s2 += lg[k];
-      if (probs) probs[(long)n * K + k] = lg[k];
-    }
-    if (targets) {
-      const float eps = 1e-7f;
-      float loss = 0.f, sdq_p = 0.f;
-      for (int k = 0; k < K; ++k) {
-        const float qv = lg[k] / s2;
-        const float qc = fminf(fmaxf(qv, eps), 1.f - eps);
-        const float t = targets[(long)n * K + k];
-        loss -= t * (qv > 1.f - eps ? -eps : logf(qc));
-        const float dq = (qv >= eps && qv <= 1.f - eps) ? -t / qc * inv_n : 0.f;
-        dl[k] = dq;
-        sdq_p += dq * lg[k];
-      }
-      if (loss_per) loss_per[n] = loss;
-      float sp_dp = 0.f;
-      for (int k = 0; k < K; ++k) {
-        const float dp = dl[k] / s2 - sdq_p / (s2 * s2);
-        dl[k] = dp;
-        sp_dp += lg[k] * dp;
-      }
-      for (int k = 0; k < K; ++k) {
-        const float d = lg[k] * (dl[k] - sp_dp);
-        dl[k] = d;
-        if (dlogits) dlogits[(long)n * K + k] = d;
-      }
+      loss -= tx[k] * lx[k];
+      sdq_p += dl[k] * pr[k];
+    }
+    if (tid == 0 && loss_per) loss_per[n] = loss;
+    float dp = 0.f;
+    if (mine) {
+      dp = dq / s2 - sdq_p / (s2 * s2);
+      dpv[tid] = dp;
+    }
+    __syncthreads();
+    float sp_dp = 0.f;
+    for (int k = 0; k < K; ++k) sp_dp += pr[k] * dpv[k];
+    if (mine) {
+      const float d = pk * (dp - sp_dp);
+      dl[tid] = d;
+      if (dlogits) dlogits[(long)n * K + tid] = d;
     }
   }
   __syncthreads();
@@ -339,9 +358,18 @@
   const int k = tid % K, nl = tid / K;
   float a = 0.f;
   if (nl < NL && tid < NL * K) {
-    for (int n = nl; n < N; n += NL) {
-      const float d = dlogits[(long)n * K + k];
-      a = (c < C) ? fmaf(gap[(long)n * C + c], d, a) : a + d;
+    constexpr int U = 8;
+    for (int n0 = nl; n0 < N; n0 += U * NL) {
+      float d[U], g[U];
+#pragma unroll
+      for (int u = 0; u < U; ++u) {
+        const int n = min(n0 + u * NL, N - 1);
+        d[u] = dlogits[(long)n * K + k];
+        g[u] = c < C ? gap[(long)n * C + c] : 0.f;
+      }
+#pragma unroll
+      for (int u = 0; u < U; ++u)
+        if (n0 + u * NL < N) a = (c < C) ? fmaf(g[u], d[u], a) : a + d[u];
     }
   }
   red[tid] = a;
@@ -426,23 +454,24 @@
 }
 
 int head(const void* xL, int act_bf16, const float* fck, const float* fcb, const float* targets, int N, int HW, int C,
-         int K, float* probs, float* loss_per, float* dlogits, float* gap, void* dxL, hipStream_t s, void* growL) {
+         int K, float* probs, float* loss_per, float* dlogits, float* gap, void* dxL, hipStream_t s, void* growL,
+         unsigned* zero_words, int nzero) {
   if (C > 256 || K > 256) return fail(ASR_E_UNSUPPORTED, "head: C and num_classes must be <= 256");
   const float inv_n = 1.f / (float)N;
   if (act_bf16) {
     if (C % 8 == 0)
       hipLaunchKernelGGL((k_head<bf16, 8>), dim3(N), dim3(256), 0, s, (const bf16*)xL, fck, fcb, targets, HW, C, K,
-                         inv_n, probs, loss_per, dlogits, gap, (bf16*)dxL, (bf16*)growL);
+                         inv_n, probs, loss_per, dlogits, gap, (bf16*)dxL, (bf16*)growL, zero_words, nzero);
     else
       hipLaunchKernelGGL((k_head<bf16, 1>), dim3(N), dim3(256), 0, s, (const bf16*)xL, fck, fcb, targets, HW, C, K,
-                         inv_n, probs, loss_per, dlogits, gap, (bf16*)dxL, (bf16*)growL);
+                         inv_n, probs, loss_per, dlogits, gap, (bf16*)dxL, (bf16*)growL, zero_words, nzero);
   } else {
     if (C % 4 == 0)
       hipLaunchKernelGGL((k_head<float, 4>), dim3(N), dim3(256), 0, s, (const float*)xL, fck, fcb, targets, HW, C,
-                         K, inv_n, probs, loss_per, dlogits, gap, (float*)dxL, (float*)growL);
+                         K, inv_n, probs, loss_per, dlogits, gap, (float*)dxL, (float*)growL, zero_words, nzero);
     else
       hipLaunchKernelGGL((k_head<float, 1>), dim3(N), dim3(256), 0, s, (const float*)xL, fck, fcb, targets, HW, C,
-                         K, inv_n, probs, loss_per, dlogits, gap, (float*)dxL, (float*)growL);
+                         K, inv_n, probs, loss_per, dlogits, gap, (float*)dxL, (float*)growL, zero_words, nzero);
   }
   ASR_LAUNCH_CHECK("k_head");
   return ASR_OK;
diff --git a/differential_equations_resnet_amd/csrc/asr_theta.hip b/differential_equations_resnet_amd/csrc/asr_theta.hip
--- a/differential_equations_resnet_amd/csrc/asr_theta.hip
+++ b/differential_equations_resnet_amd/csrc/asr_theta.hip
@@ -806,4 +806,87 @@
   return ASR_OK;
 }
 
-}
+__global__ __launch_bounds__(256) void k_stack_grad_tail(const float* __restrict__ slabs, long slab_stride, int P,
+                                                         const float* __restrict__ grp, long grp_stride, long E,
+                                                         int Cb, const int32_t* __restrict__ theta_dst,
+                                                         const int32_t* __restrict__ owner, long n_theta, int lfold,
+                                                         const unsigned* __restrict__ flags, float* __restrict__ out,
+                                                         long out_stride) {
+  __shared__ float part[2][4][64];
+  const int l = blockIdx.y, el = threadIdx.x & 63, q = threadIdx.x >> 6;
+  const long ES = E + Cb, e = blockIdx.x * 64L + el;
+  const int G = (P + 31) / 32, G4 = G & ~3;
+  const bool from_slabs = l < lfold || flags[l] != 0u;
+  const float* sl = slabs + (long)l * slab_stride;
+  const float* rg = grp + (long)l * grp_stride;
+  const long j = e < ES ? owner[e] : -1;
+  auto group_row = [&](long ee, int g) {
+    return from_slabs ? sum_slab_rows(sl, ES, ee, 32 * g, min(P, 32 * g + 32)) : rg[(long)g * ES + ee];
+  };
+  auto partial = [&](long ee) {
+    float a = 0.f;
+    if (ee < 0) return a;
+    for (int g = q; g < G4; g += 4) a += group_row(ee, g);
+    if (q == 0)
+      for (int g = G4; g < G; ++g) a += group_row(ee, g);
+    return a;
+  };
+  part[0][q][el] = partial(e < ES ? e : -1);
+  int32_t v0 = -1, v1 = -1;
+  if (j >= 0 && j < n_theta) {
+    v0 = theta_dst[2 * j];
+    v1 = theta_dst[2 * j + 1];
+  }
+  const bool own0 = !(v0 >= 0 && (v0 >> 1) != e);
+  const int32_t vo = own0 ? v1 : v0;
+  part[1][q][el] = partial(vo >= 0 ? (long)(vo >> 1) : -1L);
+  __syncthreads();
+  if (q == 0 && j >= 0) {
+    auto red = [&](int h) { return (part[h][0][el] + part[h][1][el]) + (part[h][2][el] + part[h][3][el]); };
+    float acc = 0.f;
+    if (v0 >= 0) acc += (v0 & 1) ? -red(own0 ? 0 : 1) : red(own0 ? 0 : 1);
+    if (v1 >= 0) acc += (v1 & 1) ? -red(own0 ? 1 : 0) : red(own0 ? 1 : 0);
+    out[(long)l * out_stride + j] = j >= n_theta ? red(0) : acc;
+  }
+}
+
+__global__ void k_theta_owner(const int32_t* __restrict__ theta_dst, long n_theta, long E, int Cb,
+                              int32_t* __restrict__ owner) {
+  const long j = blockIdx.x * (long)blockDim.x + threadIdx.x;
+  if (j < n_theta) {
+    const int32_t v0 = theta_dst[2 * j], v1 = theta_dst[2 * j + 1];
+    const int32_t v = v0 >= 0 ? v0 : v1;
+    if (v >= 0) owner[v >> 1] = (int32_t)j;
+  }
+  if (j < Cb) owner[E + j] = (int32_t)(n_theta + j);
+}
+
+int theta_owner(const int32_t* theta_dst, long n_theta, long E, int Cb, int32_t* owner, hipStream_t s) {
+  ASR_TRY(hip_check(hipMemsetAsync(owner, 0xFF, (size_t)(E + Cb) * 4, s), "hipMemsetAsync(owner)"));
+  const long n = std::max(n_theta, (long)Cb);
+  hipLaunchKernelGGL(k_theta_owner, dim3((unsigned)((n + 255) / 256)), dim3(256), 0, s, theta_dst, n_theta, E, Cb,
+                     owner);
+  ASR_LAUNCH_CHECK("k_theta_owner");
+  return ASR_OK;
+}
+
+int theta_owner_host(const int32_t* theta_dst, long n_theta, long E, int Cb, int32_t* owner) {
+  std::fill(owner, owner + E + Cb, -1);
+  for (long j = 0; j < n_theta; ++j) {
+    const int32_t v = theta_dst[2 * j] >= 0 ? theta_dst[2 * j] : theta_dst[2 * j + 1];
+    if (v >= 0) owner[v >> 1] = (int32_t)j;
+  }
+  for (int c = 0; c < Cb; ++c) owner[E + c] = (int32_t)(n_theta + c);
+  return ASR_OK;
+}
+
+int stack_bwd_reduce_rest(const float* slabs, long slab_stride, int grid, long ES, const float* grp, long grp_stride,
+                          int L, int lfold, const unsigned* done, int Cb, const int32_t* theta_dst,
+                          const int32_t* owner, long n_theta, float* out, long out_stride, hipStream_t s) {
+  hipLaunchKernelGGL(k_stack_grad_tail, dim3((unsigned)((ES + 63) / 64), L), dim3(256), 0, s, slabs, slab_stride, grid,
+                     grp, grp_stride, ES - Cb, Cb, theta_dst, owner, n_theta, lfold, done + L + 4, out, out_stride);
+  ASR_LAUNCH_CHECK("k_stack_grad_tail");
+  return ASR_OK;
+}
+
+}
```

Measured after the change: 161,600 images/s, median of 2. About the same (-0.4%).
